# netapp-rickhuang-ai/spark-rapids-ml-nai

Measured on AMD Instinct MI355X. Metric: fit-time speedup vs Spark-ML CPU (geomean over reference headline workloads, 1Mx3000 fp32), higher is better.
Workload: dtype fp32

## Files before the change

### spark_rapids_ml_nai_amd/models/logistic.py

```python
from __future__ import annotations

import os

from typing import Any, Dict, List, Optional, Tuple

import numpy as np
import torch

from .. import ops
from ..parallel.context import WorkerContext
from .qn import QNProblem, minimize


def _problem(n: int, m_total: int, stats: Dict[str, Any], reg: float, l1_ratio: float, fit_intercept: bool,
             standardization: bool, max_iter: int, tol: float, K: int) -> Tuple[QNProblem, np.ndarray, np.ndarray]:
    sigma = stats["sigma"]
    inv_sigma = np.where(sigma > 0, 1.0 / np.where(sigma > 0, sigma, 1.0), 0.0)
    q1 = sigma if standardization else np.ones(n)
    q2 = sigma * sigma if standardization else np.ones(n)
    pen_l2 = reg * (1.0 - l1_ratio) * np.where(sigma > 0, q2 / np.where(sigma > 0, sigma * sigma, 1.0), 0.0)
    pen_l1 = reg * l1_ratio * np.where(sigma > 0, q1 / np.where(sigma > 0, sigma, 1.0), 0.0)
    nb = K if fit_intercept else 0
    theta0 = np.zeros(K * n + nb)
    if fit_intercept:
        counts = stats["class_counts"]
        if K == 1:
            p1 = counts[1] / max(counts.sum(), 1.0) if len(counts) > 1 else 0.5
            p1 = min(max(p1, 1e-12), 1 - 1e-12)
            theta0[K * n] = np.log(p1 / (1 - p1))
        else:
            lc = np.log(np.maximum(counts[:K], 1.0))
            theta0[K * n:] = lc - lc.mean()
    P = QNProblem(n=n, K=K, fit_intercept=fit_intercept, m_total=float(m_total),
                  l2=np.concatenate([np.tile(pen_l2, K), np.zeros(nb)]),
                  l1=np.concatenate([np.tile(pen_l1 if l1_ratio > 0 and reg > 0 else np.zeros(n), K), np.zeros(nb)]),
                  inv_sigma=inv_sigma, max_iter=max(0, int(max_iter)), tol=float(tol), M=10)
    return P, theta0, inv_sigma


def _result(res: Dict[str, Any], base: Dict[str, Any], ctx: WorkerContext, n: int, K: int, fit_intercept: bool,
            inv_sigma: np.ndarray, path: str) -> Dict[str, Any]:
    theta = res["theta"]
    if ctx.world_size > 1:
        th = torch.from_numpy(theta).to(ctx.device)
        ctx.comm.broadcast(th, 0)
        theta = th.cpu().numpy()
    W = theta[: K * n].reshape(K, n) * inv_sigma
    b = theta[K * n:] if fit_intercept else np.zeros(K)
    if fit_intercept and K > 1:
        b = b - b.mean()
    out = dict(base)
    out.update(coef_=W.tolist(), intercept_=[float(v) for v in b], num_iters=int(res["iter"]),
               objective=float(res["f"]))
    out["_solver"] = {"n_evals": int(res["n_evals"]), "status": res["status"], "path": path}
    if res.get("n_margin_only"):
        out["_solver"]["n_margin_only"] = int(res["n_margin_only"])
    return out


def _one_class(classes: list, base: Dict[str, Any], n: int) -> Dict[str, Any]:
    cv = classes[0]
    if cv not in (0.0, 1.0):
        raise RuntimeError("class value must be either 1. or 0. when dataset has one label")
    out = dict(base)
    out.update(coef_=[[0.0] * n], intercept_=[float("inf") if cv == 1.0 else float("-inf")], num_iters=0,
               objective=0.0)
    return out


def logistic_fit(X: Any, y: torch.Tensor, m_total: int, ctx: WorkerContext, reg: float, l1_ratio: float,
                 fit_intercept: bool, standardization: bool, max_iter: int, tol: float,
                 n_classes: Optional[int] = None, sparse: bool = False,
                 stats: Optional[Dict[str, Any]] = None) -> Dict[str, Any]:
    n = X.shape[1]
    if stats is None:
        stats = logistic_stats(X, y, m_total, ctx, sparse)
    classes = stats["classes"]
    C = n_classes if n_classes is not None else stats["num_classes"]
    K = 1 if C <= 2 else C
    dtype = "float32" if (X.dtype if not sparse else X.data.dtype) == torch.float32 else "float64"
    base = {"classes_": [float(c) for c in classes], "n_cols": int(n), "dtype": dtype}
    if len(classes) == 1 and fit_intercept:
        return _one_class(classes, base, n)
    P, theta0, inv_sigma = _problem(n, m_total, stats, reg, l1_ratio, fit_intercept, standardization, max_iter, tol, K)
    y32 = y if y.dtype == torch.float32 else y.to(torch.float32)
    y32 = y32.contiguous()

    ws = ops.logreg_workspace(X) if not sparse and K == 1 else None

    def evaluate(w: torch.Tensor, b: torch.Tensor, flag: Optional[torch.Tensor], out: torch.Tensor,
                 zc: Optional[tuple] = None) -> None:
        ops.logistic_loss_grad(X, y32, w, b, K, out, flag, ws=ws, zcache=zc)

    allreduce = ctx.comm.allreduce if ctx.distributed else None
    path = ops.logistic_path(X, K)
    fold = evaluate_partials = None
    if ws is not None and allreduce is None and path == "fused_binary_f32":
        parts, wst = ops.logreg_fold_layout(X)
        fold = (ws, parts, wst)
        _scratch = ops.zeros(K * n + 2, dtype=torch.float64, device=X.device)

        def evaluate_partials(w: torch.Tensor, b: torch.Tensor, flag: Optional[torch.Tensor],
                              zc: Optional[tuple] = None) -> None:
            ops.logistic_loss_grad(X, y32, w, b, K, _scratch, flag, ws=ws, leave_partials=True, zcache=zc)
    graph_safe = (path in ("fused_binary_f32", "fused_multinomial_f32", "csr_binary", "two_pass_multinomial_f32",
                           "two_pass_binary_f32") or path.startswith("lds_binary")) and _eval_bytes(X) <= GRAPH_MAX_BYTES
    zok = ((path == "fused_binary_f32" and (X.shape[0] == 0 or ops.logreg_zcache_ok(X)))
           or (path == "two_pass_multinomial_f32" and ops.XW_MFMA_MIN_K <= K <= 16))
    if allreduce is not None:
        flag_t = torch.tensor([1.0 if zok else 0.0], dtype=torch.float64, device=X.device)
        ctx.comm.allreduce(flag_t, op="min")
        zok = bool(flag_t.item() > 0)
    zbuf = ops.zeros(2 * X.shape[0] * K, dtype=torch.float64, device=X.device) if zok else None
    res = minimize(P, theta0, evaluate, allreduce, y.device, batch=8 if not path.startswith("torch") else 2,
                   graph_safe=graph_safe, fold=fold, evaluate_partials=evaluate_partials, zcache=zbuf)
    return _result(res, base, ctx, n, K, fit_intercept, inv_sigma, path)


GRAPH_MAX_BYTES = int(os.environ.get("SRML_QN_GRAPH_MAX_MB", "64")) << 20


def _eval_bytes(X: Any) -> int:
    if hasattr(X, "data") and hasattr(X, "indices") and not isinstance(X, torch.Tensor):
        return int(X.data.numel() * X.data.element_size() + X.indices.numel() * X.indices.element_size())
    return int(X.numel() * X.element_size())


MAX_BATCH = 12


def logistic_fit_multi(X: Any, y: torch.Tensor, m_total: int, ctx: WorkerContext, settings: List[Dict[str, Any]],
                       sparse: bool = False, stats: Optional[Dict[str, Any]] = None) -> List[Dict[str, Any]]:
    n = X.shape[1]
    if stats is None:
        stats = logistic_stats(X, y, m_total, ctx, sparse)
    K = 1 if stats["num_classes"] <= 2 else stats["num_classes"]
    if sparse or K != 1 or len(settings) < 2 or not ops.mbin_supported(X, min(len(settings), MAX_BATCH)):
        return [logistic_fit(X, y, m_total, ctx, s["reg"], s["l1_ratio"], s["fit_intercept"], s["standardization"],
                             s["max_iter"], s["tol"], sparse=sparse, stats=stats) for s in settings]
    from .qn import minimize_batch

    classes = stats["classes"]
    base = {"classes_": [float(c) for c in classes], "n_cols": int(n), "dtype": "float32"}
    y32 = (y if y.dtype == torch.float32 else y.to(torch.float32)).contiguous()
    allreduce = ctx.comm.allreduce if ctx.distributed else None
    out: List[Optional[Dict[str, Any]]] = [None] * len(settings)
    todo = []
    for i, s in enumerate(settings):
        if len(classes) == 1 and s["fit_intercept"]:
            out[i] = _one_class(classes, base, n)
        else:
            todo.append(i)
    for g0 in range(0, len(todo), MAX_BATCH):
        grp = todo[g0: g0 + MAX_BATCH]
        probs = [_problem(n, m_total, stats, settings[i]["reg"], settings[i]["l1_ratio"], settings[i]["fit_intercept"],
                          settings[i]["standardization"], settings[i]["max_iter"], settings[i]["tol"], 1) for i in grp]

        def evaluate(WB: torch.Tensor, OUT: torch.Tensor) -> None:
            ops.logistic_loss_grad_multi(X, y32, WB, OUT)

        res = minimize_batch([p[0] for p in probs], [p[1] for p in probs], evaluate, allreduce, y.device)
        for i, (P, _, inv_sigma), r in zip(grp, probs, res):
            out[i] = _result(r, base, ctx, n, 1, P.fit_intercept, inv_sigma, "batched_binary_f32")
    return [o for o in out if o is not None]


def logistic_stats(X: Any, y: torch.Tensor, m_total: int, ctx: WorkerContext, sparse: bool) -> Dict[str, Any]:
    n = X.shape[1]
    if sparse:
        s, q = ops.csr_col_moments(X)
    else:
        s, q = ops.col_moments(X)
    yl = y.long()
    if torch.any(y < 0) or torch.any(y != torch.floor(y)):
        bad = y[(y < 0) | (y != torch.floor(y))][0].item()
        if bad < 0:
            raise RuntimeError(f"Labels MUST be in [0, 2147483647), but got {bad}")
        raise RuntimeError(f"Labels MUST be Integers, but got {bad}")
    mx = torch.tensor([float(yl.max().item()) if yl.numel() else 0.0], dtype=torch.float64, device=y.device)
    ctx.comm.allreduce(mx, op="max")
    ncls = int(mx.item()) + 1
    hist = ops.label_counts(yl, ncls).double()
    buf = torch.cat([s, q, hist])
    ctx.comm.allreduce(buf)
    s, q, hist = buf[:n], buf[n: 2 * n], buf[2 * n:]
    mean = (s / m_total).cpu().numpy()
    var = np.maximum((q / m_total).cpu().numpy() - mean * mean, 0.0)
    var = var * m_total / max(m_total - 1, 1)
    counts = hist.cpu().numpy()
    classes = [float(c) for c in np.nonzero(counts > 0)[0]]
    return {"sigma": np.sqrt(var), "mean": mean, "class_counts": counts, "classes": classes,
            "num_classes": max(2, ncls)}


def logistic_scores(X: torch.Tensor, coef: torch.Tensor, intercept: torch.Tensor) -> torch.Tensor:
    return ops.xw(X, coef.T.contiguous(), intercept)
```

### spark_rapids_ml_nai_amd/models/qn.py

```python
from __future__ import annotations

import ctypes
import os
from dataclasses import dataclass
from typing import Callable, List, Optional

import numpy as np
import torch

from .. import ops

QN_GRAPH = os.environ.get("SRML_QN_GRAPH", "1") != "0"
QN_GRAPH_COMM = os.environ.get("SRML_QN_GRAPH_COMM", "1") != "0"
QN_STEP = os.environ.get("SRML_QN_STEP", "mb")
if QN_STEP not in ("mb", "single"):
    raise ValueError("SRML_QN_STEP must be 'mb' or 'single', not %r" % QN_STEP)
QN_MB = QN_STEP == "mb"
GRAPH_STATS = {"captures": 0, "replays": 0}
STATUS = {0: "running", 1: "converged (gradient)", 2: "converged (objective change)", 3: "max iterations",
          4: "line search failed"}
F_DONE, F_STATUS, F_ITER, F_NEVAL, F_LS, F_COUNT, F_HEAD, F_STARTED, F_BRACKET, F_ZMODE, F_ZSEL, F_NCHEAP, F_ZC = \
    range(13)
SC_F, SC_ALPHA, SC_DGINIT, SC_GAMMA, SC_GINF, SC_ALPHA1, SC_BETA = range(7)
QN_ZCACHE = os.environ.get("SRML_QN_ZCACHE", "1") != "0"


@dataclass
class QNProblem:
    n: int
    K: int
    fit_intercept: bool
    m_total: float
    l2: np.ndarray
    l1: np.ndarray
    inv_sigma: np.ndarray
    max_iter: int
    tol: float
    M: int = 10
    max_ls: int = 20
    past: int = 10
    c1: float = 1e-4
    c2: float = 0.9
    wolfe: bool = False
    delta: Optional[float] = None

    @property
    def Kn(self) -> int:
        return self.K * self.n

    @property
    def N(self) -> int:
        return self.Kn + (self.K if self.fit_intercept else 0)

    @property
    def use_l1(self) -> bool:
        return bool(np.any(self.l1 > 0))

    @property
    def delta_(self) -> float:
        return 0.01 * self.tol if self.delta is None else float(self.delta)

    @property
    def out_len(self) -> int:
        return self.Kn + self.K + 1


def _interp_width(f0: float, ft: float, dgtest: float) -> float:
    den = 2.0 * (ft - f0 - dgtest)
    w = -dgtest / den if den > 0 else 0.5
    if not np.isfinite(w):
        return 0.5
    return float(min(0.5, max(0.1, w)))


class HostQN:

    def __init__(self, P: QNProblem, theta0: np.ndarray) -> None:
        self.P = P
        N = P.N
        self.x = np.zeros(N)
        self.g = np.zeros(N)
        self.pg = np.zeros(N)
        self.d = np.zeros(N)
        self.xt = np.asarray(theta0, dtype=np.float64).copy()
        self.S: list = []
        self.Y: list = []
        self.f = 0.0
        self.alpha = 0.0
        self.dginit = 0.0
        self.gamma = 1.0
        self.iter = 0
        self.n_evals = 0
        self.ls = 0
        self.bracket = False
        self.started = False
        self.done = False
        self.status = 0
        self.fh = np.zeros(max(P.past, 1))
        self._isg_full = np.tile(P.inv_sigma, P.K)

    def wb(self) -> np.ndarray:
        P = self.P
        out = np.zeros(P.Kn + P.K)
        out[: P.Kn] = self.xt[: P.Kn] * self._isg_full
        if P.fit_intercept:
            out[P.Kn:] = self.xt[P.Kn:]
        return out

    @staticmethod
    def _pseudo(x: np.ndarray, g: np.ndarray, c: np.ndarray) -> np.ndarray:
        pg = g.copy()
        pos, neg, zero = x > 0, x < 0, x == 0
        pg[pos] += c[pos]
        pg[neg] -= c[neg]
        gp, gm = g + c, g - c
        z = zero & (c > 0)
        pz = np.where(gp < 0, gp, np.where(gm > 0, gm, 0.0))
        pg[z] = pz[z]
        return pg

    def _set_trial(self) -> None:
        P = self.P
        t = self.x + self.alpha * self.d
        if P.use_l1:
            orth = np.where(self.x != 0, np.sign(self.x), -np.sign(self.pg))
            mask = (P.l1 > 0) & (t * orth <= 0)
            t[mask] = 0.0
        self.xt = t

    def step(self, out: np.ndarray) -> None:
        P = self.P
        if self.done:
            return
        out = np.asarray(out, dtype=np.float64)
        Kn, N = P.Kn, P.N
        xt = self.xt
        gt = np.empty(N)
        gt[:Kn] = out[:Kn] / P.m_total * self._isg_full + P.l2[:Kn] * xt[:Kn]
        gt[Kn:] = out[Kn:N] / P.m_total
        ft = out[Kn + P.K] / P.m_total + 0.5 * float(np.sum(P.l2 * xt * xt)) + float(np.sum(P.l1 * np.abs(xt)))
        self.n_evals += 1
        if self.started:
            accept, width = True, 1.0
            if not np.isfinite(ft):
                accept, width = False, 0.5
            else:
                dgtest = float(self.pg @ (xt - self.x)) if P.use_l1 else self.alpha * self.dginit
                if ft > self.f + P.c1 * dgtest:
                    accept, width = False, _interp_width(self.f, ft, dgtest)
                elif P.wolfe and not P.use_l1 and not self.bracket and float(gt @ self.d) < P.c2 * self.dginit:
                    accept, width = False, 2.1
            if not accept:
                self.ls += 1
                if self.ls >= P.max_ls:
                    self.status, self.done = 4, True
                    return
                if width < 1.0:
                    self.bracket = True
                self.alpha *= width
                self._set_trial()
                return
        pg = self._pseudo(xt, gt, P.l1 if P.use_l1 else np.zeros(N))
        if self.started:
            s, y = xt - self.x, gt - self.g
            ys, yy = float(s @ y), float(y @ y)
            if yy > 0 and ys > 1e-10 * yy:
                self.S.append(s)
                self.Y.append(y)
                if len(self.S) > P.M:
                    self.S.pop(0)
                    self.Y.pop(0)
                self.gamma = ys / yy
            self.iter += 1
        self.x, self.g, self.f, self.pg = xt.copy(), gt, ft, pg
        self.ls, self.bracket = 0, False
        status = 0
        fmag = max(abs(ft), P.tol)
        if np.max(np.abs(pg)) <= P.tol * fmag if N else True:
            status = 1
        if P.past > 0:
            k = self.iter
            if status == 0 and self.started and k >= P.past and abs(self.fh[k % P.past] - ft) <= P.delta_ * fmag:
                status = 2
            self.fh[k % P.past] = ft
        if status == 0 and self.iter >= P.max_iter:
            status = 3
        self.started = True
        if status:
            self.status, self.done = status, True
            return
        d = -self._h_times(pg)
        if P.use_l1:
            d[(P.l1 > 0) & (d * pg >= 0)] = 0.0
        dg = float(pg @ d)
        if not dg < 0:
            d = -pg
            dg = -float(pg @ pg)
            self.S, self.Y, self.gamma = [], [], 1.0
        self.d = d
        self.dginit = dg
        self.alpha = 1.0 / max(np.sqrt(float(d @ d)), 1e-300) if not self.S else 1.0
        self._set_trial()

    def _h_times(self, v: np.ndarray) -> np.ndarray:
        if not self.S:
            return v.copy()
        S = np.stack(self.S)
        Y = np.stack(self.Y)
        g = self.gamma
        SY = S @ Y.T
        R = np.triu(SY)
        Dg = np.diag(np.diag(SY))
        p1, p2 = S @ v, Y @ v
        from scipy.linalg import solve_triangular

        t = solve_triangular(R, p1, lower=False)
        a = solve_triangular(R.T, (Dg + g * (Y @ Y.T)) @ t - g * p2, lower=True)
        return g * v + S.T @ a - g * (Y.T @ t)

    def theta(self) -> np.ndarray:
        return self.x.copy()


class _QnArgs(ctypes.Structure):
    _fields_ = [("N", ctypes.c_long), ("Kn", ctypes.c_long), ("n", ctypes.c_int), ("K", ctypes.c_int),
                ("M", ctypes.c_int), ("past", ctypes.c_int), ("max_iter", ctypes.c_int), ("max_ls", ctypes.c_int),
                ("l1", ctypes.c_int), ("wolfe", ctypes.c_int), ("tol", ctypes.c_double), ("delta", ctypes.c_double),
                ("inv_m", ctypes.c_double), ("c1", ctypes.c_double), ("c2", ctypes.c_double)] + \
               [(nm, ctypes.c_void_p) for nm in ("x", "g", "pg", "d", "xt", "gt", "S", "Y", "SY", "YY", "fh", "sc",
                                                 "l2", "l1c", "isg", "fl", "wb", "out", "probe")]


class DeviceQN:

    def __init__(self, P: QNProblem, theta0: np.ndarray, device: torch.device, wb: Optional[torch.Tensor] = None,
                 out: Optional[torch.Tensor] = None, flags: Optional[torch.Tensor] = None) -> None:
        from ..ops import native

        self.P = P
        self.device = device
        N, M = P.N, P.M
        if M > int(native.lib().srml_qn_max_history()):
            raise ValueError("L-BFGS memory %d exceeds the kernel's capacity" % M)
        f64 = dict(dtype=torch.float64, device=device)
        self.vec = ops.zeros((6 + 2 * M) * N, **f64)
        v = self.vec
        self.x, self.g, self.pg, self.d, self.xt, self.gt = (v[i * N:(i + 1) * N] for i in range(6))
        self.S = v[6 * N: (6 + M) * N]
        self.Y = v[(6 + M) * N:]
        self.small = ops.zeros(2 * M * M + max(P.past, 1) + 8, **f64)
        self.coef = torch.from_numpy(np.concatenate([P.l2, P.l1, P.inv_sigma]).astype(np.float64)).to(device)
        self.flags = flags if flags is not None else ops.zeros(16, dtype=torch.int32, device=device)
        self.wb = wb if wb is not None else ops.zeros(P.Kn + P.K, **f64)
        self.out = out if out is not None else ops.zeros(P.out_len, **f64)
        assert self.wb.numel() == P.Kn + P.K and self.out.numel() == P.out_len and self.flags.numel() == 16
        th = torch.from_numpy(np.asarray(theta0, dtype=np.float64)).to(device)
        self.xt.copy_(th)
        isg = torch.from_numpy(np.tile(P.inv_sigma, P.K)).to(device)
        self.wb[: P.Kn] = th[: P.Kn] * isg
        if P.fit_intercept:
            self.wb[P.Kn:] = th[P.Kn:]
        a = _QnArgs()
        a.N, a.Kn, a.n, a.K, a.M, a.past = N, P.Kn, P.n, P.K, M, P.past
        a.max_iter, a.max_ls, a.l1, a.wolfe = int(P.max_iter), int(P.max_ls), int(P.use_l1), int(P.wolfe)
        a.tol, a.delta, a.inv_m, a.c1, a.c2 = float(P.tol), P.delta_, 1.0 / float(P.m_total), P.c1, P.c2
        sm = self.small
        MM = M * M
        ptrs = dict(x=self.x, g=self.g, pg=self.pg, d=self.d, xt=self.xt, gt=self.gt, S=self.S, Y=self.Y,
                    SY=sm[:MM], YY=sm[MM: 2 * MM], fh=sm[2 * MM: 2 * MM + max(P.past, 1)],
                    sc=sm[2 * MM + max(P.past, 1):], l2=self.coef[:N], l1c=self.coef[N: 2 * N],
                    isg=self.coef[2 * N:], fl=self.flags, wb=self.wb, out=self.out)
        for k, t in ptrs.items():
            setattr(a, k, t.data_ptr())

        if os.environ.get("SRML_QN_PROBE") == "1":
            self.probe = ops.zeros(16, dtype=torch.int64, device=device)
            a.probe = self.probe.data_ptr()
        self._args = a
        self._keep = ptrs
        self._mb = None
        self.fold: Optional[tuple] = None
        if QN_MB and N <= 16384 and os.environ.get("SRML_QN_PROBE") != "1":
            self._mb = ops.zeros(int(native.lib().srml_qn_mb_scratch()), **f64)
        assert ctypes.sizeof(_QnArgs) == int(native.lib().srml_qn_args_size()), "QnArgs layout mismatch"

    @property
    def w_dev(self) -> torch.Tensor:
        return self.wb[: self.P.Kn]

    @property
    def b_dev(self) -> torch.Tensor:
        return self.wb[self.P.Kn:]

    def step(self) -> None:
        from ..ops import native

        if self._mb is not None and self.fold is not None:
            ws, parts, wst = self.fold
            native.call("srml_qn_step_mbf", ctypes.addressof(self._args), self._mb.data_ptr(), ws.data_ptr(),
                        int(parts), int(wst), native.stream(self.device))
        elif self._mb is not None:
            native.call("srml_qn_step_mb", ctypes.addressof(self._args), self._mb.data_ptr(), native.stream(self.device))
        else:
            native.call("srml_qn_step", ctypes.addressof(self._args), native.stream(self.device))

    def theta(self) -> np.ndarray:
        return self.x.cpu().numpy().copy()

    def zcache_supported(self) -> bool:
        return not self.P.use_l1 and not self.P.wolfe

    def enable_zcache(self, zbuf: torch.Tensor) -> tuple:
        self.flags[F_ZC] = 1
        return (self.flags, zbuf, self._keep["sc"])

    def info(self) -> dict:
        fl = self.flags.cpu().numpy()
        sc = self._keep["sc"].cpu().numpy()
        return {"iter": int(fl[F_ITER]), "n_evals": int(fl[F_NEVAL]), "status": STATUS.get(int(fl[F_STATUS]), "?"),
                "f": float(sc[SC_F]), "done": bool(fl[F_DONE]), "n_margin_only": int(fl[F_NCHEAP])}


def _graph_capturable(allreduce: Callable) -> bool:
    comm = getattr(allreduce, "__self__", None)
    if comm is None or getattr(comm, "backend", "none") != "nccl":
        return False
    from ..parallel import oneshot

    return oneshot.comm_mode() == "rccl"


def _comm_poll(allreduce: Optional[Callable]) -> Optional[Callable[[], None]]:
    return getattr(getattr(allreduce, "__self__", None), "poll", None)


def minimize(P: QNProblem, theta0: np.ndarray, evaluate: Callable[[torch.Tensor, torch.Tensor, Optional[torch.Tensor],
                                                                   torch.Tensor], None],
             allreduce: Optional[Callable[[torch.Tensor], None]], device: torch.device,
             batch: int = 8, graph_safe: bool = False, fold: Optional[tuple] = None,
             evaluate_partials: Optional[Callable] = None, zcache: Optional[torch.Tensor] = None) -> dict:
    if device.type != "cuda":
        st = HostQN(P, theta0)
        out = ops.zeros(P.out_len, dtype=torch.float64, device=device)
        cap = max(1, P.max_iter) * (P.max_ls + 1) + 2
        while not st.done and st.n_evals < cap:
            wb = torch.from_numpy(st.wb()).to(device)
            out.zero_()
            evaluate(wb[: P.Kn], wb[P.Kn:], None, out)
            if allreduce is not None:
                allreduce(out)
            st.step(out.cpu().numpy())
        return {"theta": st.theta(), "f": st.f, "iter": st.iter, "n_evals": st.n_evals,
                "status": STATUS[st.status if st.done else 3]}
    q = DeviceQN(P, theta0, device)
    zc = None
    if zcache is not None and QN_ZCACHE and q.zcache_supported():
        zc = q.enable_zcache(zcache)
    if fold is not None and evaluate_partials is not None and allreduce is None and q._mb is not None:
        q.fold = fold
        evaluate = lambda w, b, flag, out, **kw: evaluate_partials(w, b, flag, **kw)
    zkw = {"zc": zc} if zc is not None else {}
    poll = _comm_poll(allreduce)
    flag = q.flags[F_DONE: F_DONE + 1]
    host_flag = ops.zeros(2, dtype=torch.int32, pin_memory=True)
    events: list = []
    cap = max(1, P.max_iter) * (P.max_ls + (2 if zc is not None else 1)) + 2
    evals = 0
    stream = torch.cuda.current_stream(device)
    j = 0

    def run_batch() -> None:
        for _ in range(batch):
            evaluate(q.w_dev, q.b_dev, flag, q.out, **zkw)
            if allreduce is not None:
                allreduce(q.out)
            q.step()

    graph = None
    use_graph = graph_safe and QN_GRAPH and (allreduce is None or (QN_GRAPH_COMM and _graph_capturable(allreduce)))
    while evals < cap:
        if graph is not None:
            graph.replay()
            GRAPH_STATS["replays"] += 1
        else:
            run_batch()
            if use_graph and evals + batch < cap:
                graph = torch.cuda.CUDAGraph()
                side = torch.cuda.Stream(device)
                side.wait_stream(stream)
                try:
                    with torch.cuda.stream(side):
                        graph.capture_begin()
                        try:
                            run_batch()
                        finally:
                            graph.capture_end()
                    GRAPH_STATS["captures"] += 1
                except RuntimeError:
                    if allreduce is None:
                        raise
                    graph, use_graph = None, False
                    GRAPH_STATS["comm_capture_failed"] = GRAPH_STATS.get("comm_capture_failed", 0) + 1
                stream.wait_stream(side)
        evals += batch
        slot = host_flag[j % 2: j % 2 + 1]
        slot.copy_(flag, non_blocking=True)
        ev = torch.cuda.Event()
        ev.record(stream)
        events.append((ev, slot))
        j += 1
        if poll is not None:
            poll()
        if len(events) >= 2:
            ev0, s0 = events.pop(0)
            ev0.synchronize()
            if int(s0.item()):
                break
    torch.cuda.synchronize(device)
    res = q.info()
    res["theta"] = q.theta()
    if not res["done"]:
        res["status"] = "evaluation cap"
    return res


def minimize_batch(Ps: List[QNProblem], theta0s: List[np.ndarray],
                   evaluate: Callable[[torch.Tensor, torch.Tensor], None],
                   allreduce: Optional[Callable[[torch.Tensor], None]], device: torch.device,
                   batch: int = 8) -> List[dict]:
    from ..ops import native

    B = len(Ps)
    n = Ps[0].n
    assert all(P.K == 1 and P.n == n for P in Ps), "batched QN needs binary problems of one width"
    f64 = dict(dtype=torch.float64, device=device)
    WB = ops.zeros((B, n + 1), **f64)
    OUT = ops.zeros((B, n + 2), **f64)
    FL = ops.zeros((B, 16), dtype=torch.int32, device=device)
    qs = [DeviceQN(P, th, device, wb=WB[j], out=OUT[j], flags=FL[j]) for j, (P, th) in enumerate(zip(Ps, theta0s))]
    raw = b"".join(bytes(q._args) for q in qs)
    args_dev = torch.frombuffer(bytearray(raw), dtype=torch.uint8).to(device)
    st = native.stream(device)
    host = ops.zeros(2, dtype=torch.int32, pin_memory=True)
    cap = max(max(1, P.max_iter) * (P.max_ls + 1) + 2 for P in Ps)
    evals, j = 0, 0
    events: list = []
    stream = torch.cuda.current_stream(device)
    poll = _comm_poll(allreduce)
    while evals < cap:
        for _ in range(batch):
            evaluate(WB, OUT)
            if allreduce is not None:
                allreduce(OUT)
            native.call("srml_qn_step_batch", args_dev.data_ptr(), B, st)
        evals += batch
        slot = host[j % 2: j % 2 + 1]
        slot.copy_(FL[:, F_DONE].min().view(1), non_blocking=True)
        ev = torch.cuda.Event()
        ev.record(stream)
        events.append((ev, slot))
        j += 1
        if poll is not None:
            poll()
        if len(events) >= 2:
            ev0, s0 = events.pop(0)
            ev0.synchronize()
            if int(s0.item()):
                break
    torch.cuda.synchronize(device)
    out = []
    for q in qs:
        r = q.info()
        r["theta"] = q.theta()
        if not r["done"]:
            r["status"] = "evaluation cap"
        out.append(r)
    return out
```

### spark_rapids_ml_nai_amd/ops/__init__.py

```python
from __future__ import annotations

import math
import os
from typing import Any, Callable, Dict, Iterator, Optional, Tuple

import numpy as np
import torch

from . import native
from ..utils.determinism import deterministic

__all__ = ["col_moments", "gram", "xw", "dgemm", "sign_flip", "is_native", "xtv", "row_sqnorm",
           "logreg_binary_loss_grad", "nearest_centroid", "cluster_sums", "csr_logreg_binary_loss_grad",
           "csr_spmm", "csr_spmtm", "csr_col_moments", "logistic_loss_grad", "svc_path", "svc_loss_grad"]


def is_native(t: torch.Tensor) -> bool:
    return t.is_cuda


def _c(t: torch.Tensor) -> torch.Tensor:
    return t if t.is_contiguous() else t.contiguous()


# ... 138 lines not shown
        a = A.double().T if ta else A.double()
        b = B.double().T if tb else B.double()
        res = alpha * (a @ b)
        if beta != 0.0:
            res = res + beta * out
        out.copy_(res)
        return out
    A = _c(A.double())
    B = _c(B.double())
    if out.stride(1) != 1:
        raise ValueError("dgemm: out must have unit column stride")
    st = native.stream(A.device)
    tiles = ((M + 63) // 64) * ((N + 63) // 64)
    splits = _dgemm_splits(M, N, K, tiles)
    if splits > 1:
        ws = torch.empty(splits * M * N, dtype=torch.float64, device=A.device)
        native.call("srml_dgemm_splitk", int(ta), int(tb), M, N, K, float(alpha), A.data_ptr(), A.stride(0),
                    B.data_ptr(), B.stride(0), float(beta), out.data_ptr(), out.stride(0), splits, ws.data_ptr(), st)
        return out
    native.call("srml_dgemm", int(ta), int(tb), M, N, K, float(alpha), A.data_ptr(), A.stride(0), B.data_ptr(),
                B.stride(0), float(beta), out.data_ptr(), out.stride(0), st)
    return out


def _dgemm_splits(M: int, N: int, K: int, tiles: int) -> int:
    if tiles >= 512 or K < 128:
        return 1
    want = (1024 + tiles - 1) // tiles
    by_k = K // 64
    by_mem = max(1, (256 << 20) // max(1, 8 * M * N))
    return max(1, min(want, by_k, by_mem))


def sign_flip(U: torch.Tensor) -> torch.Tensor:
    rows, cols = U.shape
    if not U.is_cuda or U.dtype != torch.float64 or not U.is_contiguous():
        idx = U.abs().argmax(0)
        s = torch.sign(U[idx, torch.arange(cols, device=U.device)])
        s[s == 0] = 1
        U.mul_(s)
        return U
    native.call("srml_sign_flip_f64", U.data_ptr(), rows, cols, U.stride(0), native.stream(U.device))
    return U


def xtv(X: torch.Tensor, V: torch.Tensor, out: Optional[torch.Tensor] = None) -> torch.Tensor:
    m, n = X.shape
    V2 = V.reshape(m, -1)
    k = V2.shape[1]
    if out is None:
        out = zeros((n, k), dtype=torch.float64, device=X.device)
    if not X.is_cuda:
        out += X.double().T @ V2.double()
        return out
    if X.dtype == torch.float64:
        dgemm(_c(X), _c(V2.to(torch.float64)), ta=True, beta=1.0, out=out)
        return out
    if X.dtype != torch.float32:
        raise TypeError("xtv supports fp32/fp64 inputs, got %s" % X.dtype)
    X = _c(X)
    if k >= XTV_MFMA_MIN_K:
        for c0 in range(0, k, 16):
            kk = min(16, k - c0)
            Vc = _c(V2[:, c0: c0 + kk].to(torch.float32))
            oc = out[:, c0: c0 + kk]
            native.call("srml_xtv_mfma_f32", X.data_ptr(), m, n, X.stride(0), Vc.data_ptr(), kk, Vc.stride(0),
                        oc.data_ptr(), oc.stride(0), oc.stride(1), None, native.stream(X.device))
        return out
    if k <= 4 and out.is_contiguous() and out.dtype == torch.float64:
        Vc = _c(V2.to(torch.float32))
        native.call("srml_xtv_f32", X.data_ptr(), m, n, X.stride(0), Vc.data_ptr(), k, Vc.stride(0), out.data_ptr(),
                    native.stream(X.device))
        return out
    for c0 in range(0, k, 4):
        kk = min(4, k - c0)
        Vc = _c(V2[:, c0: c0 + kk].to(torch.float32))
        tmp = zeros((n, kk), dtype=torch.float64, device=X.device)
        native.call("srml_xtv_f32", X.data_ptr(), m, n, X.stride(0), Vc.data_ptr(), kk, Vc.stride(0), tmp.data_ptr(),
                    native.stream(X.device))
        out[:, c0: c0 + kk] += tmp
    return out


def row_sqnorm(X: torch.Tensor, mu: Optional[torch.Tensor] = None) -> torch.Tensor:
    m, n = X.shape
    if mu is not None:
        muf = _c(mu.float().view(-1))
        if not X.is_cuda or X.dtype != torch.float32:
            return ((X.float() - muf) ** 2).sum(1)
        X = _c(X)
        out = torch.empty(m, dtype=torch.float32, device=X.device)
        native.call("srml_row_sqnorm_centered_f32", X.data_ptr(), m, n, X.stride(0), muf.data_ptr(), out.data_ptr(),
                    native.stream(X.device))
        return out
    if X.is_cuda and X.dtype == torch.float64:
        X = _c(X)
        out = torch.empty(m, dtype=torch.float64, device=X.device)
        native.call("srml_row_sqnorm_f64", X.data_ptr(), m, n, X.stride(0), out.data_ptr(), native.stream(X.device))
        return out
    if not X.is_cuda or X.dtype != torch.float32:
        return (X.float() * X.float()).sum(1)
    X = _c(X)
    out = torch.empty(m, dtype=torch.float32, device=X.device)
    native.call("srml_row_sqnorm_f32", X.data_ptr(), m, n, X.stride(0), out.data_ptr(), native.stream(X.device))
    return out


def _softplus(z: torch.Tensor) -> torch.Tensor:
    return torch.clamp(z, min=0) + torch.log1p(torch.exp(-z.abs()))


def logreg_binary_loss_grad(X: torch.Tensor, y: torch.Tensor, w: torch.Tensor, b: float,
                            out: Optional[torch.Tensor] = None) -> torch.Tensor:
    m, n = X.shape
    if not X.is_cuda or X.dtype != torch.float32 or n > 4096:
        Xd = X.double()
        z = Xd @ w.double().to(X.device) + b
        yd = y.double()
        p = torch.sigmoid(z)
        r = p - yd
        loss = _softplus(z).sum() - (yd * z).sum()
        return torch.cat([Xd.T @ r, r.sum().view(1), loss.view(1)])
    X = _c(X)
    out = zeros(n + 2, dtype=torch.float64, device=X.device) if out is None else zero_(out)
    wf = _c(w.to(device=X.device, dtype=torch.float64))
    yf = _c(y.to(torch.float32))
    ws = logreg_workspace(X)
    native.call("srml_logreg_binary_f32", X.data_ptr(), m, n, X.stride(0), yf.data_ptr(), wf.data_ptr(), float(b),
                None, None, out.data_ptr(), ws.data_ptr() if ws is not None else None, 0, None, None, None,
                native.stream(X.device))
    return out


def logreg_fold_layout(X: Any) -> Tuple[int, int]:
    m, n = X.shape
    return int(native.lib().srml_logreg_fold_parts(m)), ((n + 3) & ~3) + 4


def logreg_workspace(X: Any) -> Optional[torch.Tensor]:
    if _is_csr(X) or not X.is_cuda or X.dtype != torch.float32:
        return None
    m, n = X.shape
    ptr, ld = (X.data_ptr(), X.stride(0)) if X.is_contiguous() else (0, n)
    nf = int(native.lib().srml_logreg_fold_ws(m, n, ld, ptr))
    return torch.empty(nf, dtype=torch.float32, device=X.device) if nf > 0 else None


def logreg_zcache_ok(X: Any) -> bool:
    if _is_csr(X) or not X.is_cuda or X.dtype != torch.float32 or deterministic():
        return False
    m, n = X.shape
    ptr, ld = (X.data_ptr(), X.stride(0)) if X.is_contiguous() else (0, n)
    return bool(int(native.lib().srml_logreg_zcache_ok(m, n, ld, ptr)))


def nearest_centroid(X: torch.Tensor, C: torch.Tensor, xnorm: Optional[torch.Tensor] = None,
                     cnorm: Optional[torch.Tensor] = None) -> Tuple[torch.Tensor, torch.Tensor]:
    m, n = X.shape
    k = C.shape[0]
    if X.is_cuda and X.dtype == torch.float64:
        X = _c(X)
        Cd = _c(C.to(device=X.device, dtype=torch.float64))
        cn = (Cd * Cd).sum(1) if cnorm is None or cnorm.dtype != torch.float64 else _c(cnorm)
        xn = xnorm if xnorm is not None and xnorm.dtype == torch.float64 else row_sqnorm(X)
        labels = torch.empty(m, dtype=torch.int32, device=X.device)
        dist = torch.empty(m, dtype=torch.float32, device=X.device)
        native.call("srml_nearest_centroid_f64", X.data_ptr(), m, n, X.stride(0), Cd.data_ptr(), k, Cd.stride(0),
                    cn.data_ptr(), _c(xn).data_ptr(), labels.data_ptr(), dist.data_ptr(), None,
                    native.stream(X.device))
        return labels, dist
    if cnorm is None:
        cnorm = (C.float() * C.float()).sum(1)
    if not X.is_cuda or X.dtype != torch.float32:
        labels = torch.empty(m, dtype=torch.int32, device=X.device)
        dist = torch.empty(m, dtype=torch.float32, device=X.device)
        bs = max(1, (1 << 24) // max(k, 1))
        for s in range(0, m, bs):
            xb = X[s: s + bs].float()
            d = cnorm.view(1, -1) - 2.0 * (xb @ C.float().T)
            v, i = d.min(1)
            xn = (xb * xb).sum(1) if xnorm is None else xnorm[s: s + bs]
            labels[s: s + bs] = i.int()
            dist[s: s + bs] = (v + xn).clamp_min(0)
        return labels, dist
    X = _c(X)
    C = _c(C.to(torch.float32))
    cn = _c(cnorm.to(torch.float32))
    if lloyd_small_ok(X, k, search_only=True):
        return kmeans_lloyd_small(X, C, cn, with_sums=False)[:2]
    best = torch.full((m,), -1, dtype=torch.int64, device=X.device)
    st = native.stream(X.device)
    native.call("srml_nearest_centroid_f32", X.data_ptr(), m, n, X.stride(0), C.data_ptr(), k, C.stride(0),
                cn.data_ptr(), best.data_ptr(), st)
    if xnorm is None:
        xnorm = row_sqnorm(X)
    labels = torch.empty(m, dtype=torch.int32, device=X.device)
    dist = torch.empty(m, dtype=torch.float32, device=X.device)
    native.call("srml_nn_finalize", best.data_ptr(), m, xnorm.data_ptr(), labels.data_ptr(), dist.data_ptr(), st)
    return labels, dist


def split_bf16x3(X: torch.Tensor, row_multiple: int = 128, tiled: bool = False,
                 mu: Optional[torch.Tensor] = None) -> torch.Tensor:
    m, n = X.shape
    kp = (n + 15) // 16 * 16
    if tiled and X.is_cuda and X.dtype == torch.float32:
        rows_pad = max(256, (m + 255) // 256 * 256)
        X = X if X.stride(1) == 1 else X.contiguous()
        P = torch.empty((3, rows_pad // 256, kp // 16, 256, 16), dtype=torch.bfloat16, device=X.device)
        if mu is not None:
            muf = _c(mu.float().view(-1))
            native.call("srml_split_bf16x3_tiled_centered", X.data_ptr(), m, n, X.stride(0), muf.data_ptr(), kp,
                        rows_pad, P.data_ptr(), native.stream(X.device))
        else:
            native.call("srml_split_bf16x3_tiled", X.data_ptr(), m, n, X.stride(0), kp, rows_pad, P.data_ptr(),
                        native.stream(X.device))
        return P
    if mu is not None:
        X = X.float() - mu.float().view(1, -1)
    rows_pad = max(row_multiple, (m + row_multiple - 1) // row_multiple * row_multiple)
    if not X.is_cuda or X.dtype != torch.float32:
        P = zeros((3, rows_pad, kp), dtype=torch.bfloat16, device=X.device)
        r = X.float()
        for p in range(3):
            P[p, :m, :n] = r.to(torch.bfloat16)
            r = r - P[p, :m, :n].float()
        return P
    X = X if X.stride(1) == 1 else X.contiguous()
    P = torch.empty((3, rows_pad, kp), dtype=torch.bfloat16, device=X.device)
    native.call("srml_split_bf16x3", X.data_ptr(), m, n, X.stride(0), kp, rows_pad, P.data_ptr(),
                native.stream(X.device))
    return P


CERTIFY_TAU = 2.0 ** -13


def split_bf16x3_rows(X: torch.Tensor, rows: torch.Tensor, mu: Optional[torch.Tensor]) -> torch.Tensor:
    m, n = int(rows.shape[0]), X.shape[1]
    if not X.is_cuda or X.dtype != torch.float32 or X.stride(1) != 1:
        return split_bf16x3(X.index_select(0, rows.long()), tiled=True, mu=mu)
    kp = (n + 15) // 16 * 16
    rows_pad = max(256, (m + 255) // 256 * 256)
    P = torch.empty((3, rows_pad // 256, kp // 16, 256, 16), dtype=torch.bfloat16, device=X.device)
    muf = _c(mu.float().view(-1)) if mu is not None else None
    ri = _c(rows.to(torch.int32))
    native.call("srml_split_bf16x3_tiled_centered_rows", X.data_ptr(), X.stride(0), ri.data_ptr(), m, n,
                muf.data_ptr() if muf is not None else None, kp, rows_pad, P.data_ptr(), native.stream(X.device))
    return P


def certify_tau(n: int) -> float:
    return CERTIFY_TAU + 2.0 * float(n) * 2.0 ** -24


def _nearest_centroid_certified(XP: torch.Tensor, X: torch.Tensor, m: int, k: int, CP: torch.Tensor,
                                cn: torch.Tensor, xnorm: torch.Tensor, st: int, mu: Optional[torch.Tensor]
                                ) -> Tuple[torch.Tensor, torch.Tensor]:
    dev = XP.device
    nslot = int(native.lib().srml_nearest_centroid_split_top2_nslot(k))
    keys = torch.empty(m * nslot, dtype=torch.int64, device=dev)
    lob = torch.empty(m * nslot, dtype=torch.float32, device=dev)
    xrows, kp, crows = XP.shape[1] * 256, XP.shape[2] * 16, CP.shape[1] * 256
    xn = _c(xnorm.float())
    tau = certify_tau(int(X.shape[1]) if X is not None else kp)
    cg = (2.0 * tau) * cn.clamp_min(0).sqrt()
    native.call("srml_nearest_centroid_split_top2", XP.data_ptr(), m, xrows, kp, CP.data_ptr(), k, crows,
                cn.data_ptr(), cg.data_ptr(), xn.data_ptr(), keys.data_ptr(), lob.data_ptr(), st)
    labels = torch.empty(m, dtype=torch.int32, device=dev)
    dist = torch.empty(m, dtype=torch.float32, device=dev)
    flagged = torch.empty(m, dtype=torch.int32, device=dev)
    cnt = zeros(1, dtype=torch.int32, device=dev)
    native.call("srml_split_top2_select", keys.data_ptr(), lob.data_ptr(), m, nslot, xn.data_ptr(), cg.data_ptr(),
                labels.data_ptr(), dist.data_ptr(), flagged.data_ptr(), cnt.data_ptr(), st)
    del keys, lob
    nf = int(cnt.item())
    _CERTIFY_STATS["rows"] += m
    _CERTIFY_STATS["refined"] += nf
    if nf:
        rows = flagged[:nf]
        XPr = split_bf16x3_rows(X, rows, mu)
        best = torch.full((nf,), -1, dtype=torch.int64, device=dev)
        native.call("srml_nearest_centroid_split_tiled_np", XPr.data_ptr(), nf, XPr.shape[1] * 256, kp,
                    CP.data_ptr(), k, crows, cn.data_ptr(), best.data_ptr(), 6, st)
        native.call("srml_split_scatter_refined", best.data_ptr(), rows.data_ptr(), nf, xn.data_ptr(),
                    labels.data_ptr(), dist.data_ptr(), st)
    return labels, dist


_CERTIFY_STATS = {"rows": 0, "refined": 0}


F16_U = 2.0 ** -11
F16_A = 2.0 ** -14


def certify_tau16(n: int) -> float:
    return 1.01 * (2.0 * F16_U + F16_U * F16_U + 1.01 * float(n) * 2.0 ** -24)


def f16_radius_terms(n: int, scale: float, tau: float) -> Tuple[float, float, float]:
    a = F16_A / scale
    z = 2.02 * a * math.sqrt(n) * (1.0 + F16_U)
    z2 = 2.02 * float(n) * a * a
    wmax = math.sqrt(n) * 32768.0 / scale
    return (z + 2.0 ** -24 * wmax) / (2.0 * tau), z, z2
# ... 2912 lines not shown
    n = X.shape[1]
    f32 = X.dtype == torch.float32
    if deterministic() and f32:
        return det
    if f32 and n <= 4096:
        return "fused_%s_f32" % tag
    if X.dtype in (torch.float32, torch.float64) and n <= 16384:
        return "lds_%s_%s" % (tag, "f32" if f32 else "f64")
    return "two_pass_%s_%s" % (tag, "f32" if f32 else "f64")


def logistic_path(X, K: int) -> str:
    if K == 1:
        return _binary_path(X, "binary", "two_pass_deterministic_f32")
    if _is_csr(X):
        if not X.data.is_cuda:
            return "torch-cpu"
        return "csr_spmm" if K <= 16 else "csr_wide"
    if not X.is_cuda:
        return "torch-cpu"
    n = X.shape[1]
    if deterministic() and X.dtype == torch.float32 and K <= 16:
        return "two_pass_deterministic_f32"
    if X.dtype == torch.float32 and K <= 16:
        fused = os.environ.get("SRML_LOGREG_FUSED", "0") == "1" and int(native.lib().srml_mlogit_supported(n, K))
        return "fused_multinomial_f32" if fused else "two_pass_multinomial_f32"
    if X.dtype == torch.float32:
        return "two_pass_wide_f32"
    return "two_pass_multinomial_f64"


def _glm_wide(X, y32: torch.Tensor, W: torch.Tensor, b: torch.Tensor, out: torch.Tensor,
              flag: Optional[torch.Tensor]) -> None:
    csr = _is_csr(X)
    m, n = X.shape
    K = W.shape[0]
    dev = X.data.device if csr else X.device
    st = native.stream(dev)
    fp = flag.data_ptr() if flag is not None else None
    Wf = W.to(torch.float32)
    if csr:
        Z = csr_spmm(X, Wf.t())
    else:
        Z = torch.empty((m, K), dtype=torch.float32, device=dev)
        for c0 in range(0, K, 32):
            xw_t(X, _c(Wf[c0: c0 + 32]), out=Z[:, c0: c0 + 32])
    R = zeros((m, K), dtype=torch.float32, device=dev)
    Kn = K * n
    native.call("srml_logit_residual_wide_f32", Z.data_ptr(), m, K, K, _c(y32).data_ptr(), _c(b).data_ptr(), 1,
                R.data_ptr(), K, out[Kn + K:].data_ptr(), fp, st)
    del Z
    gb, _ = col_moments(R, need_sq=False)
    out[Kn: Kn + K] += gb
    if csr:
        out[: K * n] += csr_spmtm(X, R).t().reshape(-1)
        return
    for c0 in range(0, K, 16):
        kk = min(16, K - c0)
        native.call("srml_xtv_mfma_f32", X.data_ptr(), m, n, X.stride(0), R[:, c0:].data_ptr(), kk, K,
                    out[c0 * n:].data_ptr(), 1, n, fp, st)


def mbin_supported(X, M: int) -> bool:
    return (not _is_csr(X)) and X.is_cuda and X.dtype == torch.float32 and M >= 1


def _glm_two_pass(X: torch.Tensor, y32: torch.Tensor, W: torch.Tensor, b: torch.Tensor, sb: int, mode: int,
                  grad: torch.Tensor, so_c: int, so_k: int, gb: torch.Tensor, sgb: int, loss: torch.Tensor, sl: int,
                  flag: Optional[torch.Tensor], zc: Optional[tuple] = None, family: str = "logit",
                  kind: Tuple[int, ...] = ()) -> None:
    m, n = X.shape
    K = W.shape[0]
    st = native.stream(X.device)
    fp = flag.data_ptr() if flag is not None else None
    yp = _c(y32).data_ptr()
    if zc is not None:
        zfl, zb, zsc = zc
        skip = zfl[13:14]
        Wt = W.to(torch.float32).contiguous()
        Z = torch.empty((m, K), dtype=torch.float32, device=X.device)
        X = _c(X)
        native.call("srml_xw_t_f32_skip", X.data_ptr(), m, n, X.stride(0), Wt.data_ptr(), K, Wt.stride(0), None,
                    Z.data_ptr(), Z.stride(0), skip.data_ptr(), st)
        R = torch.empty((m, K), dtype=torch.float32, device=X.device)
        native.call("srml_logit_residual_zc_f32", Z.data_ptr(), m, K, Z.stride(0), yp, b.data_ptr(), sb, mode,
                    R.data_ptr(), K, gb.data_ptr(), sgb, loss.data_ptr(), sl, fp, zfl.data_ptr(), zb.data_ptr(),
                    zsc.data_ptr(), st)
        fn = "srml_xtv_mfma_f32" if K >= XTV_MFMA_MIN_K else "srml_xtv2_f32"
        native.call(fn, X.data_ptr(), m, n, X.stride(0), R.data_ptr(), K, K, grad.data_ptr(), so_c, so_k,
                    skip.data_ptr(), st)
        return
    Z = xw_t(X, W.to(torch.float32).contiguous()) if K >= XW_MFMA_MIN_K else xw(X, W.t().float().contiguous())
    R = torch.empty((m, K), dtype=torch.float32, device=X.device)
    if deterministic():
        L = native.lib()
        ws = torch.empty(max(int(L.srml_logit_residual_ws(m, K)), int(L.srml_xtv_mfma_ws(m, n, K)), 1),
                         dtype=torch.float64, device=X.device)
        native.call("srml_%s_residual_det_f32" % family, Z.data_ptr(), m, K, Z.stride(0), yp, b.data_ptr(), sb, mode,
                    R.data_ptr(), K, gb.data_ptr(), sgb, loss.data_ptr(), sl, fp, ws.data_ptr(), *kind, st)
        native.call("srml_xtv_mfma_det_f32", X.data_ptr(), m, n, X.stride(0), R.data_ptr(), K, K, grad.data_ptr(),
                    so_c, so_k, fp, ws.data_ptr(), st)
        return
    native.call("srml_%s_residual_f32" % family, Z.data_ptr(), m, K, Z.stride(0), yp, b.data_ptr(), sb,
                mode, R.data_ptr(), K, gb.data_ptr(), sgb, loss.data_ptr(), sl, fp, *kind, st)
    fn = "srml_xtv_mfma_f32" if K >= XTV_MFMA_MIN_K else "srml_xtv2_f32"
    native.call(fn, X.data_ptr(), m, n, X.stride(0), R.data_ptr(), K, K, grad.data_ptr(), so_c, so_k, fp, st)


def _binary_two_pass(X: torch.Tensor, y32: torch.Tensor, w: torch.Tensor, b: torch.Tensor, out: torch.Tensor,
                     flag: Optional[torch.Tensor], family: str = "logit", kind: Tuple[int, ...] = ()) -> None:
    m, n = X.shape
    if X.dtype == torch.float32:
        _glm_two_pass(X, y32, w.view(1, n), b, 1, 1, out, 1, n, out[n:], 1, out[n + 1:], 1, flag, family=family,
                      kind=kind)
        return
    z = dgemm(X, w.view(n, 1))
    r = zeros((m, 1), dtype=torch.float64, device=X.device)
    native.call("srml_%s_residual_f64" % family, z.data_ptr(), m, 1, 1, _c(y32).data_ptr(), b.data_ptr(), 1, 1,
                r.data_ptr(), 1, out[n:].data_ptr(), 1, out[n + 1:].data_ptr(), 1,
                flag.data_ptr() if flag is not None else None, *kind, native.stream(X.device))
    dgemm(X, r, ta=True, beta=1.0, out=out[:n].view(n, 1))


def logistic_loss_grad_multi(X: torch.Tensor, y32: torch.Tensor, WB: torch.Tensor, out: torch.Tensor) -> torch.Tensor:
    m, n = X.shape
    M = WB.shape[0]
    if mbin_supported(X, M) and WB.stride(1) == 1 and out.stride(1) == 1 and M > 16:
        for j0 in range(0, M, 16):
            logistic_loss_grad_multi(X, y32, WB[j0: j0 + 16], out[j0: j0 + 16])
        return out
    if mbin_supported(X, M) and WB.stride(1) == 1 and out.stride(1) == 1:
        X = _c(X)
        if (os.environ.get("SRML_LOGREG_FUSED", "0") == "1" and not deterministic()
                and int(native.lib().srml_mlogit_supported(n, max(2, M)))):
            native.call("srml_mbin_f32", X.data_ptr(), m, n, X.stride(0), _c(y32).data_ptr(), WB.data_ptr(),
                        WB.stride(0), M, out.data_ptr(), out.stride(0), native.stream(X.device))
            return out
        ld = out.stride(0)
        _glm_two_pass(X, y32, WB[:, :n], WB[:, n:], WB.stride(0), 1, out, 1, ld, out[:, n:], ld, out[:, n + 1:], ld,
                      None)
        return out
    Xd = X.double()
    yd = y32.double()
    Z = Xd @ WB[:, :n].double().t() + WB[:, n].double().view(1, M)
    R = torch.sigmoid(Z) - yd.view(-1, 1)
    out[:, :n] += (R.t() @ Xd)
    out[:, n] += R.sum(0)
    out[:, n + 1] += (_softplus(Z) - yd.view(-1, 1) * Z).sum(0)
    return out


def logistic_loss_grad(X, y32: torch.Tensor, w: torch.Tensor, b: torch.Tensor, K: int, out: torch.Tensor,
                       flag: Optional[torch.Tensor] = None, ws: Optional[torch.Tensor] = None,
                       leave_partials: bool = False, zcache: Optional[tuple] = None) -> torch.Tensor:
    path = logistic_path(X, K)
    if _is_csr(X):
        m, n = X.shape
        dev = X.data.device
    else:
        X = _c(X)
        m, n = X.shape
        dev = X.device
    if path.startswith("torch"):
        if _is_csr(X):
            Xs = _csr_torch(X)
            Xs = Xs.to(torch.float64) if Xs.dtype != torch.float64 else Xs
            W = w.double().view(K, n)
            Z = (Xs @ W.t()) + b.double().view(1, K)
        else:
            Xd = X.double()
            W = w.double().view(K, n)
            Z = Xd @ W.t() + b.double().view(1, K)
        yd = y32.double()
        if K == 1:
            z = Z.view(-1)
            r = (torch.sigmoid(z) - yd).view(-1, 1)
            loss = (_softplus(z) - yd * z).sum()
        else:
            lse = torch.logsumexp(Z, 1)
            Y = torch.nn.functional.one_hot(yd.long(), K).double()
            r = torch.exp(Z - lse.view(-1, 1)) - Y
            loss = (lse - (Z * Y).sum(1)).sum()
        if _is_csr(X):
            G = (Xs.t() @ r).t()
        else:
            G = r.t() @ Xd
        out[: K * n] += G.reshape(-1)
        out[K * n: K * n + K] += r.sum(0)
        out[K * n + K] += loss
        return out
    st = native.stream(dev)
    fp = flag.data_ptr() if flag is not None else None
    assert w.dtype == torch.float64 and b.dtype == torch.float64 and out.dtype == torch.float64
    assert w.numel() == K * n and b.numel() == K and out.numel() == K * n + K + 1
    if path == "csr_binary":
        _csr_check(X)
        native.call("srml_csr_logreg_binary_" + _sfx(X), X.indptr.data_ptr(), X.indices.data_ptr(), X.data.data_ptr(),
                    m, n, X.data.numel(), y32.data_ptr(), w.data_ptr(), 0.0, b.data_ptr(), fp, out.data_ptr(), st)
    elif path == "csr_spmm":
        Z = csr_spmm(X, w.view(K, n).t())
        R = zeros((m, K), dtype=torch.float32, device=dev)
        native.call("srml_logit_residual_f32", Z.data_ptr(), m, K, K, _c(y32).data_ptr(), b.data_ptr(), 1, 0,
                    R.data_ptr(), K, out[K * n:].data_ptr(), 1, out[K * n + K:].data_ptr(), 0, fp, st)
        out[: K * n] += csr_spmtm(X, R).t().reshape(-1)
    elif path in ("csr_wide", "two_pass_wide_f32"):
        _glm_wide(X, y32, w.view(K, n), b, out, flag)
    elif path in ("two_pass_binary_f32", "two_pass_binary_f64") or (path == "two_pass_deterministic_f32" and K == 1):
        _binary_two_pass(X, y32, w, b, out, flag)
    elif path == "two_pass_multinomial_f64":
        Z = dgemm(X, w.view(K, n), tb=True)
        R = zeros((m, K), dtype=torch.float64, device=dev)
        if K <= 16:
            native.call("srml_logit_residual_f64", Z.data_ptr(), m, K, K, _c(y32).data_ptr(), b.data_ptr(), 1, 0,
                        R.data_ptr(), K, out[K * n:].data_ptr(), 1, out[K * n + K:].data_ptr(), 0, fp, st)
        else:
            native.call("srml_logit_residual_wide_f64", Z.data_ptr(), m, K, K, _c(y32).data_ptr(), b.data_ptr(), 1,
                        R.data_ptr(), K, out[K * n + K:].data_ptr(), fp, st)
            del Z
            out[K * n: K * n + K] += col_moments(R, need_sq=False)[0]
        dgemm(R, X, ta=True, beta=1.0, out=out[: K * n].view(K, n))
    elif path == "fused_binary_f32":
        zc = [t.data_ptr() for t in zcache] if zcache is not None else [None, None, None]
        native.call("srml_logreg_binary_f32", X.data_ptr(), m, n, X.stride(0), y32.data_ptr(), w.data_ptr(), 0.0,
                    b.data_ptr(), fp, out.data_ptr(), ws.data_ptr() if ws is not None else None,
                    int(bool(leave_partials and ws is not None)), *zc, st)
    elif path.startswith("lds_binary"):
        native.call("srml_logreg_binary_lds_" + path[-3:], X.data_ptr(), m, n, X.stride(0), y32.data_ptr(),
                    w.data_ptr(), 0.0, b.data_ptr(), fp, out.data_ptr(), st)
    elif path == "fused_multinomial_f32":
        native.call("srml_mlogit_f32", X.data_ptr(), m, n, X.stride(0), y32.data_ptr(), w.data_ptr(), b.data_ptr(),
                    fp, K, out.data_ptr(), st)
    elif path in ("two_pass_multinomial_f32", "two_pass_deterministic_f32"):
        _glm_two_pass(X, y32, w.view(K, n), b, 1, 0, out, 1, n, out[K * n:], 1, out[K * n + K:], 0, flag,
                      zc=zcache if path == "two_pass_multinomial_f32" else None)
    else:
        raise AssertionError(path)
    return out


SVC_LOSSES = {"hinge": 0, "squared_hinge": 1}


def svc_path(X) -> str:
    return _binary_path(X, "svc", "two_pass_deterministic_svc_f32")


def exact_sum(T: torch.Tensor, bound: Any, dim: int = 0) -> torch.Tensor:
    bound = torch.as_tensor(bound, dtype=torch.float64, device=T.device).clamp_min(2.0 ** -900)
    grid = torch.ldexp(torch.ones_like(bound), torch.frexp(bound).exponent - 52)
    return (torch.round(T / grid) * grid).sum(dim)


def _svc_exact_cpu(Xd: torch.Tensor, y32: torch.Tensor, w: torch.Tensor, b: torch.Tensor, out: torch.Tensor, kind: int,
                   xmax: torch.Tensor, m_total: float) -> torch.Tensor:
    n = Xd.shape[1]
    wd, b0 = w.double().view(-1), float(b.double().view(-1)[0])
    bz = math.fsum((xmax * wd.abs()).tolist())
    z = exact_sum(Xd * wd.view(1, n), bz, 1) + b0
    s = 2.0 * y32.double() - 1.0
    h = 1.0 - s * z
    act = (h > 0).double()
    hb = 2.0 + bz + abs(b0)
    r = -2.0 * s * h * act if kind else -s * act
    rb = 2.0 * hb if kind else 1.0
    out[:n] += exact_sum(Xd * r.view(-1, 1), m_total * rb * xmax)
    out[n] += exact_sum(r, m_total * rb)
    out[n + 1] += exact_sum(h * h * act if kind else h * act, m_total * (hb * hb if kind else hb))
    return out


def svc_loss_grad(X, y32: torch.Tensor, w: torch.Tensor, b: torch.Tensor, out: torch.Tensor,
                  flag: Optional[torch.Tensor] = None, loss: str = "hinge", ws: Optional[torch.Tensor] = None,
                  leave_partials: bool = False, exact: Optional[tuple] = None) -> torch.Tensor:
    if loss not in SVC_LOSSES:
        raise ValueError(f"loss must be 'hinge' or 'squared_hinge', got {loss!r}")
    kind = SVC_LOSSES[loss]
    path = svc_path(X)
    csr = _is_csr(X)
    if csr:
        m, n = X.shape
        dev = X.data.device
    else:
        if not (X.dim() == 2 and X.stride(1) == 1 and X.stride(0) >= X.shape[1] and ws is None
                and (path == "fused_svc_f32" or path.startswith("lds_svc"))):
            X = _c(X)
        m, n = X.shape
        dev = X.device
    if path == "torch-cpu":
        wd = w.double().view(n, 1)
        if csr:
            Xd = _csr_torch(X)
            Xd = Xd.to(torch.float64) if Xd.dtype != torch.float64 else Xd
        else:
            Xd = X.double()
        if exact is not None:
            return _svc_exact_cpu(Xd.to_dense() if csr else Xd, y32, w, b, out, kind, exact[0], float(exact[1]))
        z = (Xd @ wd).view(-1) + b.double().view(-1)[0]
        s = 2.0 * y32.double() - 1.0
        h = 1.0 - s * z
        act = (h > 0).double()
        r = -2.0 * s * h * act if kind else -s * act
        lsum = (h * h * act).sum() if kind else (h * act).sum()
        out[:n] += (Xd.t() @ r.view(-1, 1)).view(-1)
        out[n] += r.sum()
        out[n + 1] += lsum
        return out
    st = native.stream(dev)
    fp = flag.data_ptr() if flag is not None else None
    assert w.dtype == torch.float64 and b.dtype == torch.float64 and out.dtype == torch.float64
    assert w.numel() == n and b.numel() == 1 and out.numel() == n + 2 and y32.dtype == torch.float32
    if path == "csr_svc":
        _csr_check(X)
        native.call("srml_csr_svc_loss_grad_" + _sfx(X), X.indptr.data_ptr(), X.indices.data_ptr(), X.data.data_ptr(),
                    m, n, X.data.numel(), y32.data_ptr(), w.data_ptr(), 0.0, b.data_ptr(), fp, out.data_ptr(), kind, st)
    elif path == "fused_svc_f32":
        native.call("srml_svc_loss_grad_f32", X.data_ptr(), m, n, X.stride(0), y32.data_ptr(), w.data_ptr(), 0.0,
                    b.data_ptr(), fp, out.data_ptr(), ws.data_ptr() if ws is not None else None,
                    int(bool(leave_partials and ws is not None)), kind, st)
    elif path.startswith("lds_svc"):
        native.call("srml_svc_loss_grad_lds_" + path[-3:], X.data_ptr(), m, n, X.stride(0), y32.data_ptr(),
                    w.data_ptr(), 0.0, b.data_ptr(), fp, out.data_ptr(), kind, st)
    elif path in ("two_pass_svc_f32", "two_pass_svc_f64", "two_pass_deterministic_svc_f32"):
        _binary_two_pass(X, y32, w, b, out, flag, family="svc", kind=(kind,))
    else:
        raise AssertionError(path)
    return out


def h2d_async(dst: torch.Tensor, src: torch.Tensor) -> None:
    if not dst.is_cuda:
        dst.copy_(src)
        return
    assert src.is_pinned() and dst.is_contiguous() and src.is_contiguous() and dst.nbytes == src.nbytes
    native.call("srml_memcpy_h2d_async", dst.data_ptr(), src.data_ptr(), dst.nbytes, native.stream(dst.device))


def d2h_sync(dst: torch.Tensor, src: torch.Tensor) -> None:
    if not src.is_cuda:
        dst.copy_(src)
        return
    assert dst.is_pinned() and dst.is_contiguous() and src.is_contiguous() and dst.nbytes == src.nbytes
    native.call("srml_memcpy_d2h_sync", dst.data_ptr(), src.data_ptr(), src.nbytes, native.stream(src.device))


def zero_(t: torch.Tensor) -> torch.Tensor:
    if not t.is_cuda:
        return t.zero_()
    assert t.is_contiguous()
    if t.numel():
        native.call("srml_memset_async", t.data_ptr(), 0, t.nbytes, native.stream(t.device))
    return t


def zeros(*size: Any, **kw: Any) -> torch.Tensor:
    return zero_(torch.empty(*size, **kw))


_KIND = {torch.float64: 0, torch.float32: 1, torch.int64: 2, torch.int32: 3}


def _kind(t: torch.Tensor) -> Tuple[torch.Tensor, int]:
    t = _c(t)
    if t.dtype not in _KIND:
        t = t.double()
    return t, _KIND[t.dtype]


CONFUSION_MAX_CLASSES = 4096


def confusion_counts(y: torch.Tensor, pred: torch.Tensor, C: int) -> Optional[np.ndarray]:
    if C > CONFUSION_MAX_CLASSES:
        return None
    m = int(y.shape[0])
    if not y.is_cuda:
        yy, pp = y.double().cpu().numpy(), pred.double().cpu().numpy()
        ok = (yy >= 0) & (yy < C) & (yy == np.floor(yy)) & (pp >= 0) & (pp < C) & (pp == np.floor(pp))
        if not ok.all():
# ... 42 lines not shown
```

### spark_rapids_ml_nai_amd/ops/csrc/glm.hip

```cpp
#include "common.h"
#include <stdlib.h>

template <int K>
__global__ __launch_bounds__(256) void xtv_kernel(const float* __restrict__ X, long m, int n, long ld,
                                                  const float* __restrict__ V, long ldv, double* __restrict__ out,
                                                  long rows_per_block) {
  const int c0 = (blockIdx.x * 256 + threadIdx.x) * 4;
  const long r0 = (long)blockIdx.y * rows_per_block;
  const long r1 = min(m, r0 + rows_per_block);
  if (c0 >= n) return;
  double acc[K][4];
  float facc[K][4];
#pragma unroll
  for (int k = 0; k < K; ++k)
#pragma unroll
    for (int j = 0; j < 4; ++j) { acc[k][j] = 0.0; facc[k][j] = 0.f; }
  const bool full = (c0 + 3 < n) && ((ld & 3) == 0);
  int cnt = 0;
  for (long r = r0; r < r1; ++r) {
    floatx4 x;
    if (full) {
      x = *reinterpret_cast<const floatx4*>(X + r * ld + c0);
    } else {
#pragma unroll
      for (int j = 0; j < 4; ++j) x[j] = (c0 + j < n) ? X[r * ld + c0 + j] : 0.f;
    }
#pragma unroll
    for (int k = 0; k < K; ++k) {
      const float v = V[r * ldv + k];
#pragma unroll
      for (int j = 0; j < 4; ++j) facc[k][j] = fmaf(x[j], v, facc[k][j]);
    }
    if (++cnt == 256) {
#pragma unroll
      for (int k = 0; k < K; ++k)
#pragma unroll
        for (int j = 0; j < 4; ++j) { acc[k][j] += facc[k][j]; facc[k][j] = 0.f; }
      cnt = 0;
    }
  }
#pragma unroll
  for (int k = 0; k < K; ++k)
#pragma unroll
    for (int j = 0; j < 4; ++j) {
      acc[k][j] += facc[k][j];
      if (c0 + j < n) atomicAdd(&out[(long)(c0 + j) * K + k], acc[k][j]);
    }
}

SRML_API int srml_xtv_f32(const float* X, long m, int n, long ld, const float* V, int k, long ldv, double* out,
                          hipStream_t stream) {
  if (m <= 0 || n <= 0) return 0;
  unsigned gx = ceil_div(n, 1024);
  long gy = (2048 + gx - 1) / gx;
  long rpb = (m + gy - 1) / gy;
  if (rpb < 64) rpb = 64;
  gy = (m + rpb - 1) / rpb;
  dim3 grid(gx, (unsigned)gy);
  switch (k) {
    case 1: hipLaunchKernelGGL(xtv_kernel<1>, grid, dim3(256), 0, stream, X, m, n, ld, V, ldv, out, rpb); break;
    case 2: hipLaunchKernelGGL(xtv_kernel<2>, grid, dim3(256), 0, stream, X, m, n, ld, V, ldv, out, rpb); break;
    case 3: hipLaunchKernelGGL(xtv_kernel<3>, grid, dim3(256), 0, stream, X, m, n, ld, V, ldv, out, rpb); break;
    case 4: hipLaunchKernelGGL(xtv_kernel<4>, grid, dim3(256), 0, stream, X, m, n, ld, V, ldv, out, rpb); break;
    default: return -1;
  }
  return srml_status();
}

template <int K>
__global__ __launch_bounds__(256) void xtv2_kernel(const float* __restrict__ X, long m, int n, long ld,
                                                   const float* __restrict__ V, long ldv, double* __restrict__ out,
                                                   long so_c, long so_k, long rows_per_block, int kk,
                                                   const int* __restrict__ flag) {
  if (flag && *flag) return;
  const int c0 = (blockIdx.x * 256 + threadIdx.x) * 4;
  const long r0 = (long)blockIdx.y * rows_per_block;
  const long r1 = min(m, r0 + rows_per_block);
  if (c0 >= n) return;
  double acc[K][4];
  float facc[K][4];
#pragma unroll
  for (int k = 0; k < K; ++k)
#pragma unroll
    for (int j = 0; j < 4; ++j) { acc[k][j] = 0.0; facc[k][j] = 0.f; }
  const bool full = (c0 + 3 < n) && ((ld & 3) == 0);
  int cnt = 0;
  for (long r = r0; r < r1; ++r) {
    floatx4 x;
    if (full) {
      x = __builtin_nontemporal_load(reinterpret_cast<const floatx4*>(X + r * ld + c0));
    } else {
#pragma unroll
      for (int j = 0; j < 4; ++j) x[j] = (c0 + j < n) ? X[r * ld + c0 + j] : 0.f;
    }
#pragma unroll
    for (int k = 0; k < K; ++k) {
      const float v = k < kk ? V[r * ldv + k] : 0.f;
#pragma unroll
      for (int j = 0; j < 4; ++j) facc[k][j] = fmaf(x[j], v, facc[k][j]);
    }
    if (++cnt == 256) {
#pragma unroll
      for (int k = 0; k < K; ++k)
#pragma unroll
        for (int j = 0; j < 4; ++j) { acc[k][j] += facc[k][j]; facc[k][j] = 0.f; }
      cnt = 0;
    }
  }
#pragma unroll
  for (int k = 0; k < K; ++k)
#pragma unroll
    for (int j = 0; j < 4; ++j) {
      acc[k][j] += facc[k][j];
      if (k < kk && c0 + j < n) atomicAdd(&out[(long)(c0 + j) * so_c + (long)k * so_k], acc[k][j]);
    }
}

SRML_API int srml_xtv2_f32(const float* X, long m, int n, long ld, const float* V, int k, long ldv, double* out,
                           long so_c, long so_k, const int* flag, hipStream_t stream) {
  if (m <= 0 || n <= 0) return 0;
  unsigned gx = ceil_div(n, 1024);
  long gy = (2048 + gx - 1) / gx;
  long rpb = (m + gy - 1) / gy;
  if (rpb < 64) rpb = 64;
  gy = (m + rpb - 1) / rpb;
  dim3 grid(gx, (unsigned)gy);
#define SRML_XTV2(KK)                                                                                            \
  hipLaunchKernelGGL(xtv2_kernel<KK>, grid, dim3(256), 0, stream, X, m, n, ld, V, ldv, out, so_c, so_k, rpb, k, flag)
  if (k <= 1) SRML_XTV2(1);
  else if (k <= 2) SRML_XTV2(2);
  else if (k <= 4) SRML_XTV2(4);
  else if (k <= 8) SRML_XTV2(8);
  else if (k <= 12) SRML_XTV2(12);
  else if (k <= 16) SRML_XTV2(16);
  else return -1;
#undef SRML_XTV2
  return srml_status();
}

template <int WPB>
__global__ __launch_bounds__(64 * WPB) void xtv_mfma_kernel(const float* __restrict__ X, long m, int n, long ld,
                                                       const float* __restrict__ V, int K, long ldv,
                                                       double* __restrict__ out, long so_c, long so_k,
                                                       long rows_per_block, int vec, const int* __restrict__ flag,
                                                       double* __restrict__ ws) {
  if (flag && *flag) return;
  const int lane = threadIdx.x & 63, g = lane >> 4, li = lane & 15;
  const int c0 = (blockIdx.x * WPB + (threadIdx.x >> 6)) * 64;
  if (c0 >= n) return;
  const long r0 = (long)blockIdx.y * rows_per_block;
  const long r1 = min(m, r0 + rows_per_block);
  const int cl = c0 + 4 * li;
  const bool cfull = vec && (c0 + 63 < n);
// ... 156 lines not shown
SRML_API int srml_fold_partials_f64(const double* ws, long parts, long pstride, long width, long inner, double* out,
                                    long so_outer, long so_inner, const int* flag, hipStream_t stream) {
  if (width <= 0 || parts <= 0) return 0;
  if (inner < 1) return -2;
  hipLaunchKernelGGL(fold_partials_kernel, dim3(ceil_div(width, 256)), dim3(256), 0, stream, ws, parts, pstride, width,
                     inner, out, so_outer, so_inner, flag);
  return srml_status();
}

__global__ __launch_bounds__(256) void row_sqnorm_kernel(const float* __restrict__ X, long m, int n, long ld,
                                                         float* __restrict__ out, const float* __restrict__ mu,
                                                         unsigned* __restrict__ amax = nullptr) {
  const int lane = threadIdx.x & 63;
  const long wave = (long)blockIdx.x * 4 + (threadIdx.x >> 6);
  const long nw = (long)gridDim.x * 4;
  const bool vec = ((ld & 3) == 0) && ((n & 3) == 0);
  float mx = 0.f;
  for (long r = wave; r < m; r += nw) {
    const float* row = X + r * ld;
    float s = 0.f;
    if (vec) {
      for (int d = lane * 4; d < n; d += 256) {
        floatx4 v = *reinterpret_cast<const floatx4*>(row + d);
        if (mu) {
          const floatx4 c = *reinterpret_cast<const floatx4*>(mu + d);
          v[0] -= c[0]; v[1] -= c[1]; v[2] -= c[2]; v[3] -= c[3];
        }
        s = fmaf(v[0], v[0], fmaf(v[1], v[1], fmaf(v[2], v[2], fmaf(v[3], v[3], s))));
        if (amax) mx = fmaxf(mx, fmaxf(fmaxf(fabsf(v[0]), fabsf(v[1])), fmaxf(fabsf(v[2]), fabsf(v[3]))));
      }
    } else {
      for (int d = lane; d < n; d += 64) {
        const float v = mu ? row[d] - mu[d] : row[d];
        s = fmaf(v, v, s);
        mx = fmaxf(mx, fabsf(v));
      }
    }
    s = wave_sum(s);
    if (lane == 0) out[r] = s;
  }
  if (amax) {
    mx = wave_max(mx);
    if (lane == 0) atomicMax(amax, __float_as_uint(mx));
  }
}

SRML_API int srml_row_sqnorm_f32(const float* X, long m, int n, long ld, float* out, hipStream_t stream) {
  if (m <= 0) return 0;
  long blocks = (m + 3) / 4;
  if (blocks > 8192) blocks = 8192;
  hipLaunchKernelGGL(row_sqnorm_kernel, dim3((unsigned)blocks), dim3(256), 0, stream, X, m, n, ld, out,
                     (const float*)nullptr);
  return srml_status();
}

SRML_API int srml_row_sqnorm_centered_f32(const float* X, long m, int n, long ld, const float* mu, float* out,
                                          hipStream_t stream) {
  if (m <= 0) return 0;
  if (reinterpret_cast<uintptr_t>(mu) & 15) return -5;
  long blocks = (m + 3) / 4;
  if (blocks > 8192) blocks = 8192;
  hipLaunchKernelGGL(row_sqnorm_kernel, dim3((unsigned)blocks), dim3(256), 0, stream, X, m, n, ld, out, mu);
  return srml_status();
}

SRML_API int srml_row_sqnorm_centered_amax_f32(const float* X, long m, int n, long ld, const float* mu, float* out,
                                               unsigned* amax, hipStream_t stream) {
  if (m <= 0) return 0;
  if (reinterpret_cast<uintptr_t>(mu) & 15) return -5;
  long blocks = (m + 3) / 4;
  if (blocks > 8192) blocks = 8192;
  hipLaunchKernelGGL(row_sqnorm_kernel, dim3((unsigned)blocks), dim3(256), 0, stream, X, m, n, ld, out, mu, amax);
  return srml_status();
}

__device__ __forceinline__ float softplus_f(float z) {
  return z > 0.f ? z + log1pf(__expf(-z)) : log1pf(__expf(z));
}

template <int V, int LOSS = GLM_LOGISTIC>
__global__ __launch_bounds__(256) void logreg_binary_kernel(const float* __restrict__ X, long m, int n, long ld,
                                                            const float* __restrict__ y, const double* __restrict__ w,
                                                            double b_in, const double* __restrict__ bptr,
                                                            const int* __restrict__ flag, double* __restrict__ out,
                                                            long rows_per_block) {
  if (flag && *flag) return;
  const double b = bptr ? *bptr : b_in;
  extern __shared__ __attribute__((aligned(16))) double ldsd[];
  double* ws = ldsd;
  float* gs = reinterpret_cast<float*>(ldsd + 256 * V);
  const int NV = 256 * V;
  for (int i = threadIdx.x; i < NV; i += 256) {
    ws[i] = (i < n) ? w[i] : 0.0;
    gs[i] = 0.f;
  }
  __syncthreads();
  const int lane = threadIdx.x & 63;
  const int wid = threadIdx.x >> 6;
  const long r0 = (long)blockIdx.x * rows_per_block;
  const long r1 = min(m, r0 + rows_per_block);

  floatx4 g[V];
#pragma unroll
  for (int v = 0; v < V; ++v) g[v] = floatx4{0.f, 0.f, 0.f, 0.f};
  double gb = 0.0, loss = 0.0;
  const bool vec = ((ld & 3) == 0);
  for (long r = r0 + wid; r < r1; r += 4) {
    const float* row = X + r * ld;
    floatx4 x[V];
    double dot = 0.0;
#pragma unroll
    for (int v = 0; v < V; ++v) {
      const int c = (v * 64 + lane) * 4;
      floatx4& xv = x[v];
      if (vec && c + 3 < n) {
        xv = *reinterpret_cast<const floatx4*>(row + c);
      } else {
#pragma unroll
        for (int q = 0; q < 4; ++q) xv[q] = (c + q < n) ? row[c + q] : 0.f;
      }
      const double2 w01 = *reinterpret_cast<const double2*>(&ws[c]);
      const double2 w23 = *reinterpret_cast<const double2*>(&ws[c + 2]);
      dot = fma((double)xv[0], w01.x, fma((double)xv[1], w01.y, fma((double)xv[2], w23.x,
                fma((double)xv[3], w23.y, dot))));
    }
    dot = wave_sum(dot);
    const double z = dot + b;
    const double yr = (double)y[r];
    double res, lt;
    binary_terms<LOSS>(z, yr, res, lt);
    if (lane == 0) {
      loss += lt;
      gb += res;
    }
    const float rf = (float)res;
#pragma unroll
    for (int v = 0; v < V; ++v)
#pragma unroll
      for (int q = 0; q < 4; ++q) g[v][q] = fmaf(rf, x[v][q], g[v][q]);
  }
#pragma unroll
  for (int v = 0; v < V; ++v)
#pragma unroll
    for (int q = 0; q < 4; ++q) atomicAdd(&gs[(v * 64 + lane) * 4 + q], g[v][q]);
  __syncthreads();
  for (int i = threadIdx.x; i < n; i += 256) atomicAdd(&out[i], (double)gs[i]);
  if (lane == 0) {
    atomicAdd(&out[n], gb);
    atomicAdd(&out[n + 1], loss);
  }
}


constexpr int LR_F_ZMODE = 9, LR_F_ZSEL = 10, LR_SC_BETA = 6;

__device__ __forceinline__ void lr_margin_only(long m, int n, const float* __restrict__ y, double* __restrict__ out,
                                               float* __restrict__ ws, const double* __restrict__ zb,
                                               const double* __restrict__ zsc, int zsel, long q0, long rows) {
  __shared__ double mred[2][4];
  const int lane = threadIdx.x & 63, wid = threadIdx.x >> 6;
  const double beta = zsc[LR_SC_BETA];
  const double* z0 = zb + (long)zsel * m;
  const double* z1 = zb + (long)(1 - zsel) * m;
  const long q1 = min(m, q0 + rows);
  double gbc = 0.0, lossc = 0.0;
  for (long r = q0 + threadIdx.x; r < q1; r += blockDim.x) {
    const double a = z0[r];
    double res, lt;
    logistic_terms(a + beta * (z1[r] - a), (double)y[r], res, lt);
    gbc += res;
    lossc += lt;
  }
  gbc = wave_sum(gbc);
  lossc = wave_sum(lossc);
  if (lane == 0) {
    mred[0][wid] = gbc;
    mred[1][wid] = lossc;
  }
  __syncthreads();
  gbc = (mred[0][0] + mred[0][1]) + (mred[0][2] + mred[0][3]);
  lossc = (mred[1][0] + mred[1][1]) + (mred[1][2] + mred[1][3]);
  if (ws == nullptr) {
    if (threadIdx.x == 0) {
      if (gbc != 0.0) atomicAdd(&out[n], gbc);
      if (lossc != 0.0) atomicAdd(&out[n + 1], lossc);
    }
    return;
  }
  const long wsc = (long)((n + 3) & ~3) + 4;
  float* mine = ws + (long)blockIdx.x * wsc;
  for (int c = 4 * threadIdx.x; c < n; c += 4 * blockDim.x)
    *reinterpret_cast<floatx4*>(mine + c) = floatx4{0.f, 0.f, 0.f, 0.f};
  if (threadIdx.x == 0) {
    double* md = reinterpret_cast<double*>(mine + wsc - 4);
    md[0] = gbc;
    md[1] = lossc;
  }
}

constexpr int LR_PF_R = 1;
constexpr int LR_PF_D = 3;
constexpr bool LR_PF_NT = true;

template <int V, int LOSS = GLM_LOGISTIC>
__global__ __launch_bounds__(256, 2) void logreg_binary_pf_kernel(const float* __restrict__ X, long m, int n, long ld,
                                                                  const float* __restrict__ y,
                                                                  const double* __restrict__ w, double b_in,
                                                                  const double* __restrict__ bptr,
                                                                  const int* __restrict__ flag,
                                                                  double* __restrict__ out, long rows_per_block,
                                                                  float* __restrict__ ws, const int* __restrict__ zfl,
                                                                  double* __restrict__ zb,
                                                                  const double* __restrict__ zsc) {
  constexpr int R = LR_PF_R, D = LR_PF_D;
  if (flag && *flag) return;
  const double b = bptr ? *bptr : b_in;
  __shared__ double part[2][R][4];
  const int lane = threadIdx.x & 63;
  const int wid = threadIdx.x >> 6;
  const int zmode = (LOSS == GLM_LOGISTIC && zfl) ? zfl[LR_F_ZMODE] : 0;
  const int zsel = (LOSS == GLM_LOGISTIC && zfl) ? zfl[LR_F_ZSEL] : 0;
  if (zmode == 1) {
    lr_margin_only(m, n, y, out, ws, zb, zsc, zsel, (long)blockIdx.x * rows_per_block, rows_per_block);
    return;
  }
  double* zw = (LOSS == GLM_LOGISTIC && zfl) ? zb + (long)(1 - zsel) * m : nullptr;
  const int cbase = wid * 256 * V;
  double wreg[V][4];
  int coff[V];
#pragma unroll
  for (int v = 0; v < V; ++v) {
    const int c = cbase + (v * 64 + lane) * 4;
    coff[v] = (c + 3 < n) ? c : 0;
#pragma unroll
    for (int q = 0; q < 4; ++q) wreg[v][q] = (c + 3 < n) ? w[c + q] : 0.0;
  }
  floatx4 g[V];
#pragma unroll
  for (int v = 0; v < V; ++v) g[v] = floatx4{0.f, 0.f, 0.f, 0.f};
  double gb = 0.0, loss = 0.0;
  const long r0 = (long)blockIdx.x * rows_per_block;
  const long r1 = min(m, r0 + rows_per_block);
  if (r0 >= r1 && ws == nullptr) return;

  auto load = [&](long rb, floatx4 (&x)[R][V]) {
#pragma unroll
    for (int i = 0; i < R; ++i) {
      const long r = rb + i < r1 ? rb + i : r1 - 1;
      const float* row = X + r * ld;
#pragma unroll
      for (int v = 0; v < V; ++v)
        x[i][v] = LR_PF_NT ? __builtin_nontemporal_load(reinterpret_cast<const floatx4*>(row + coff[v]))
                           : *reinterpret_cast<const floatx4*>(row + coff[v]);
    }
  };
  int buf = 0;
  auto process = [&](long rb, const floatx4 (&x)[R][V]) {
#pragma unroll
    for (int i = 0; i < R; ++i) {
      double dot = 0.0;
#pragma unroll
      for (int v = 0; v < V; ++v)
        dot = fma((double)x[i][v][0], wreg[v][0], fma((double)x[i][v][1], wreg[v][1],
              fma((double)x[i][v][2], wreg[v][2], fma((double)x[i][v][3], wreg[v][3], dot))));
      dot = wave_sum(dot);
      if (lane == 0) part[buf][i][wid] = dot;
    }
    __syncthreads();
#pragma unroll
    for (int i = 0; i < R; ++i) {
      const long r = rb + i;
      if (r < r1) {
        const double z = part[buf][i][0] + part[buf][i][1] + part[buf][i][2] + part[buf][i][3] + b;
        double res, lt;
        binary_terms<LOSS>(z, (double)y[r], res, lt);
        if (wid == 0 && lane == 0) {
          loss += lt;
          gb += res;
          if (zw) zw[r] = z;
        }
        const float rf = (float)res;
#pragma unroll
        for (int v = 0; v < V; ++v)
#pragma unroll
          for (int q = 0; q < 4; ++q) g[v][q] = fmaf(rf, x[i][v][q], g[v][q]);
      }
    }
    buf ^= 1;
  };
  floatx4 x[D + 1][R][V];
#pragma unroll
  for (int d = 0; d < D; ++d)
    if (r0 + d * R < r1) load(r0 + d * R, x[d]);
  for (long rb = r0; rb < r1; rb += (D + 1) * R) {
#pragma unroll
    for (int ph = 0; ph <= D; ++ph) {
      const long cur = rb + ph * R;
      if (cur < r1) {
        const long nxt = cur + D * R;
        if (nxt < r1) load(nxt, x[(ph + D) % (D + 1)]);
        process(cur, x[ph]);
      }
    }
  }
  if (ws == nullptr) {
#pragma unroll
    for (int v = 0; v < V; ++v)
#pragma unroll
      for (int q = 0; q < 4; ++q) {
        const int c = cbase + (v * 64 + lane) * 4 + q;
        if (cbase + (v * 64 + lane) * 4 + 3 < n) atomicAdd(&out[c], (double)g[v][q]);
      }
    if (wid == 0 && lane == 0) {
      atomicAdd(&out[n], gb);
      atomicAdd(&out[n + 1], loss);
    }
    return;
  }
  const long wst = (long)((n + 3) & ~3) + 4;
  float* mine = ws + (long)blockIdx.x * wst;
#pragma unroll
  for (int v = 0; v < V; ++v) {
    const int c = cbase + (v * 64 + lane) * 4;
    if (c + 3 < n) *reinterpret_cast<floatx4*>(mine + c) = g[v];
  }
  if (wid == 0 && lane == 0) {
    double* md = reinterpret_cast<double*>(mine + wst - 4);
    md[0] = gb;
    md[1] = loss;
  }
}

template <int G, int D, int LOSS = GLM_LOGISTIC, int WPE = 1>
__global__ __launch_bounds__(256, WPE) void logreg_binary_narrow_kernel(const float* __restrict__ X, long m, int n, long ld,
                                                                   const float* __restrict__ y,
                                                                   const double* __restrict__ w, double b_in,
                                                                   const double* __restrict__ bptr,
                                                                   const int* __restrict__ flag,
                                                                   double* __restrict__ out, long rows_per_block,
                                                                   const int* __restrict__ zfl,
                                                                   double* __restrict__ zb,
                                                                   const double* __restrict__ zsc) {
  if (flag && *flag) return;
  const int zmode = (LOSS == GLM_LOGISTIC && zfl) ? zfl[LR_F_ZMODE] : 0;
  const int zsel = (LOSS == GLM_LOGISTIC && zfl) ? zfl[LR_F_ZSEL] : 0;
  if (zmode == 1) {
    lr_margin_only(m, n, y, out, nullptr, zb, zsc, zsel, (long)blockIdx.x * rows_per_block, rows_per_block);
    return;
  }
  double* zw = (LOSS == GLM_LOGISTIC && zfl) ? zb + (long)(1 - zsel) * m : nullptr;
  __shared__ float gsum[4][64 * G];
  __shared__ double red[2][4];
  const double b = bptr ? *bptr : b_in;
  const int lane = threadIdx.x & 63, wid = threadIdx.x >> 6;
  const int sub = lane & 15, grp = lane >> 4;
  double wr[G][4];
  bool cok[G];
#pragma unroll
  for (int k = 0; k < G; ++k) {
    const int c = (k * 16 + sub) * 4;
    cok[k] = c + 3 < n;
#pragma unroll
    for (int q = 0; q < 4; ++q) wr[k][q] = cok[k] ? w[c + q] : 0.0;
  }
  floatx4 g[G];
#pragma unroll
  for (int k = 0; k < G; ++k) g[k] = floatx4{0.f, 0.f, 0.f, 0.f};
  double gb = 0.0, loss = 0.0;
  const long r0 = (long)blockIdx.x * rows_per_block;
  const long r1 = min(m, r0 + rows_per_block);
  const int roff = wid * 4 + grp;
  auto load = [&](long base, floatx4 (&x)[G]) {
    long r = base + roff;
    if (r >= r1) r = r1 - 1;
    const float* row = X + r * ld;
#pragma unroll
    for (int k = 0; k < G; ++k)
      x[k] = cok[k] ? __builtin_nontemporal_load(reinterpret_cast<const floatx4*>(row + (k * 16 + sub) * 4))
                    : floatx4{0.f, 0.f, 0.f, 0.f};
  };
  auto process = [&](long base, const floatx4 (&x)[G]) {
    const long r = base + roff;
    double dot = 0.0;
#pragma unroll
    for (int k = 0; k < G; ++k)
      dot = fma((double)x[k][0], wr[k][0], fma((double)x[k][1], wr[k][1],
            fma((double)x[k][2], wr[k][2], fma((double)x[k][3], wr[k][3], dot))));
    dot += dpp_d<0xb1>(dot);
    dot += dpp_d<0x4e>(dot);
    dot += dpp_d<0x141>(dot);
    dot += dpp_d<0x140>(dot);
    if (r < r1) {
      double res, lt;
      binary_terms<LOSS>(dot + b, (double)y[r], res, lt);
      if (sub == 0) {
        loss += lt;
        gb += res;
        if (zw) zw[r] = dot + b;
      }
      const float rf = (float)res;
#pragma unroll
      for (int k = 0; k < G; ++k)
#pragma unroll
        for (int q = 0; q < 4; ++q) g[k][q] = fmaf(rf, x[k][q], g[k][q]);
    }
  };
  floatx4 xs[D + 1][G];
#pragma unroll
  for (int d = 0; d < D; ++d)
    if (r0 + d * 16 < r1) load(r0 + d * 16, xs[d]);
  for (long rb = r0; rb < r1; rb += (D + 1) * 16) {
#pragma unroll
    for (int ph = 0; ph <= D; ++ph) {
      const long cur = rb + ph * 16;
      if (cur < r1) {
        const long nxt = cur + D * 16;
        if (nxt < r1) load(nxt, xs[(ph + D) % (D + 1)]);
        process(cur, xs[ph]);
      }
    }
  }
#pragma unroll
  for (int k = 0; k < G; ++k)
#pragma unroll
    for (int q = 0; q < 4; ++q) {
      float v = g[k][q];
      v += __shfl_xor(v, 16, 64);
      v += __shfl_xor(v, 32, 64);
      if (grp == 0) gsum[wid][(k * 16 + sub) * 4 + q] = v;
    }
  loss = wave_sum(loss);
  gb = wave_sum(gb);
  if (lane == 0) {
    red[0][wid] = gb;
    red[1][wid] = loss;
  }
  __syncthreads();
  for (int c = threadIdx.x; c < n; c += 256) {
    const float v = (gsum[0][c] + gsum[1][c]) + (gsum[2][c] + gsum[3][c]);
    if (v != 0.f) atomicAdd(&out[c], (double)v);
  }
  if (threadIdx.x == 0) {
    atomicAdd(&out[n], (red[0][0] + red[0][1]) + (red[0][2] + red[0][3]));
    atomicAdd(&out[n + 1], (red[1][0] + red[1][1]) + (red[1][2] + red[1][3]));
  }
}

__global__ __launch_bounds__(256) void fold_rows_kernel(const float* __restrict__ ws, int parts, long wst, int n,
                                                        double* __restrict__ out, const int* __restrict__ flag) {
  if (flag && *flag) return;
  __shared__ double red[16][65];
  const int t = threadIdx.x;
  const int q = t & 15, rg = t >> 4;
  const int ncb = (n + 63) / 64;
  if ((int)blockIdx.x < ncb) {
    const int c = (int)blockIdx.x * 64 + 4 * q;
    double a0 = 0.0, a1 = 0.0, a2 = 0.0, a3 = 0.0;
    if (c < n) {
      int p = rg;
      for (; p + 48 < parts; p += 64) {
        floatx4 v[4];
#pragma unroll
        for (int j = 0; j < 4; ++j)
          v[j] = __builtin_nontemporal_load(reinterpret_cast<const floatx4*>(ws + (long)(p + 16 * j) * wst + c));
#pragma unroll
        for (int j = 0; j < 4; ++j) { a0 += v[j][0]; a1 += v[j][1]; a2 += v[j][2]; a3 += v[j][3]; }
      }
      for (; p < parts; p += 16) {
        const floatx4 v = __builtin_nontemporal_load(reinterpret_cast<const floatx4*>(ws + (long)p * wst + c));
        a0 += v[0]; a1 += v[1]; a2 += v[2]; a3 += v[3];
      }
    }
    red[rg][4 * q] = a0;
    red[rg][4 * q + 1] = a1;
    red[rg][4 * q + 2] = a2;
    red[rg][4 * q + 3] = a3;
    __syncthreads();
    if (t < 64) {
      const int cc = (int)blockIdx.x * 64 + t;
      double sum = 0.0;
#pragma unroll
      for (int g = 0; g < 16; ++g) sum += red[g][t];
      if (cc < n) out[cc] += sum;
    }
    return;
  }
  double gb = 0.0, loss = 0.0;
  for (int p = t; p < parts; p += 256) {
    const double* pd = reinterpret_cast<const double*>(ws + (long)p * wst + wst - 4);
    gb += pd[0];
    loss += pd[1];
  }
  gb = wave_sum(gb);
  loss = wave_sum(loss);
  if ((t & 63) == 0) {
    red[0][t >> 6] = gb;
    red[1][t >> 6] = loss;
  }
  __syncthreads();
  if (t == 0) {
    out[n] += (red[0][0] + red[0][1]) + (red[0][2] + red[0][3]);
    out[n + 1] += (red[1][0] + red[1][1]) + (red[1][2] + red[1][3]);
  }
}

static long logreg_grid(long m) {
  static const long blocks_env = getenv("SRML_LOGREG_BLOCKS") ? atol(getenv("SRML_LOGREG_BLOCKS")) : 0;
  long blocks = blocks_env;
  if (blocks <= 0) {
    blocks = m / 163;
    if (blocks > 2048) blocks = 2048;
    if (blocks < 512) blocks = 512;
  }
  long rpb = (m + blocks - 1) / blocks;
  if (rpb < 16) rpb = 16;
  return (m + rpb - 1) / rpb;
}

static bool logreg_pf_eligible(int n, long ld, const void* X) {
  return n > 1024 && n <= 4096 && (n & 3) == 0 && (ld & 3) == 0 && (reinterpret_cast<uintptr_t>(X) & 15) == 0;
}

static bool logreg_narrow_eligible(int n, long ld, const void* X) {
  static const int narrow = getenv("SRML_LOGREG_NARROW") ? atoi(getenv("SRML_LOGREG_NARROW")) : 1;
  return narrow && n <= 512 && (n & 3) == 0 && (ld & 3) == 0 && (reinterpret_cast<uintptr_t>(X) & 15) == 0;
}

static bool logreg_fold_enabled() {
  static const int fold = getenv("SRML_LOGREG_FOLD") ? atoi(getenv("SRML_LOGREG_FOLD")) : 1;
  return fold != 0;
}

SRML_API long srml_logreg_fold_ws(long m, int n, long ld, const void* X) {
  if (m <= 0 || !logreg_fold_enabled() || !logreg_pf_eligible(n, ld, X)) return 0;
  return logreg_grid(m) * (((n + 3) & ~3) + 4);
}

SRML_API long srml_logreg_fold_parts(long m) { return m <= 0 ? 0 : logreg_grid(m); }

SRML_API int srml_logreg_zcache_ok(long m, int n, long ld, const void* X) {
  return m > 0 && (logreg_narrow_eligible(n, ld, X) || logreg_pf_eligible(n, ld, X)) ? 1 : 0;
}

template <int LOSS>
static int logreg_binary_launch(const float* X, long m, int n, long ld, const float* y, const double* w, double b,
                                const double* bptr, const int* flag, double* out, float* fold_ws, int leave,
                                const int* zfl, double* zb, const double* zsc, hipStream_t stream) {
  if (m <= 0) return 0;
  if (LOSS != GLM_LOGISTIC && zfl) return -2;
  if (zfl && !logreg_pf_eligible(n, ld, X) && !logreg_narrow_eligible(n, ld, X)) return -2;
  if (logreg_narrow_eligible(n, ld, X)) {
    long nb = m / 256;
    if (nb > 4096) nb = 4096;
    if (nb < 1) nb = 1;
    long rpb = (m + nb - 1) / nb;
    rpb = (rpb + 15) / 16 * 16;
    const long blocks = (m + rpb - 1) / rpb;
    const int G = (n + 63) / 64;
#define SRML_LR_NARROW(GG, DD)                                                                                       \
  hipLaunchKernelGGL((logreg_binary_narrow_kernel<GG, DD, LOSS>), dim3((unsigned)blocks), dim3(256), 0, stream, X, m, n, ld, \
                     y, w, b, bptr, flag, out, rpb, zfl, zb, zsc)
    if constexpr (LOSS != GLM_LOGISTIC) {
      if (G > 2 && G <= 4) {
        hipLaunchKernelGGL((logreg_binary_narrow_kernel<4, 1, LOSS, 4>), dim3((unsigned)blocks), dim3(256), 0, stream,
                           X, m, n, ld, y, w, b, bptr, flag, out, rpb, zfl, zb, zsc);
        return srml_status();
      }
    }
    if (G <= 1) SRML_LR_NARROW(1, 3);
    else if (G <= 2) SRML_LR_NARROW(2, 3);
    else if (G <= 4) SRML_LR_NARROW(4, 3);
    else SRML_LR_NARROW(8, 2);
#undef SRML_LR_NARROW
    return srml_status();
  }
  const long blocks = logreg_grid(m);
  long rpb = (m + blocks - 1) / blocks;
  if (rpb < 16) rpb = 16;
  dim3 grid((unsigned)blocks), blk(256);
  if (logreg_pf_eligible(n, ld, X)) {
    const int VS = (n + 1023) / 1024;
    const long wst = ((n + 3) & ~3) + 4;
    float* fws = logreg_fold_enabled() ? fold_ws : nullptr;
#define SRML_LR_PF(VV)                                                                                       \
  hipLaunchKernelGGL((logreg_binary_pf_kernel<VV, LOSS>), grid, blk, 0, stream, X, m, n, ld, y, w, b, bptr, flag, out, \
                     rpb, fws, zfl, zb, zsc)
    if (VS == 2) SRML_LR_PF(2);
    else if (VS == 3) SRML_LR_PF(3);
    else SRML_LR_PF(4);
#undef SRML_LR_PF
    if (fws && !leave)
      hipLaunchKernelGGL(fold_rows_kernel, dim3(ceil_div(n, 64) + 1), dim3(256), 0, stream, fws, (int)blocks, wst, n,
                         out, flag);
    return srml_status();
  }
  const int V = (n + 255) / 256;
  const size_t vpad = V <= 1 ? 1 : V <= 2 ? 2 : V <= 4 ? 4 : V <= 8 ? 8 : V <= 12 ? 12 : 16;
  const size_t lds = 256 * vpad * (sizeof(double) + sizeof(float));
#define SRML_LR_LAUNCH(VV)                                                                                        \
  hipLaunchKernelGGL((logreg_binary_kernel<VV, LOSS>), grid, blk, lds, stream, X, m, n, ld, y, w, b, bptr, flag, out, rpb)
  if (V <= 1) SRML_LR_LAUNCH(1);
  else if (V <= 2) SRML_LR_LAUNCH(2);
  else if (V <= 4) SRML_LR_LAUNCH(4);
  else if (V <= 8) SRML_LR_LAUNCH(8);
  else if (V <= 12) SRML_LR_LAUNCH(12);
  else if (V <= 16) SRML_LR_LAUNCH(16);
  else return -2;
#undef SRML_LR_LAUNCH
  return srml_status();
}

SRML_API int srml_logreg_binary_f32(const float* X, long m, int n, long ld, const float* y, const double* w, double b,
                                    const double* bptr, const int* flag, double* out, float* fold_ws, int leave,
                                    const int* zfl, double* zb, const double* zsc, hipStream_t stream) {
  return logreg_binary_launch<GLM_LOGISTIC>(X, m, n, ld, y, w, b, bptr, flag, out, fold_ws, leave, zfl, zb, zsc, stream);
}

SRML_API int srml_svc_loss_grad_f32(const float* X, long m, int n, long ld, const float* y, const double* w, double b,
                                    const double* bptr, const int* flag, double* out, float* fold_ws, int leave,
                                    int loss, hipStream_t stream) {
  if (loss == 0)
    return logreg_binary_launch<GLM_HINGE>(X, m, n, ld, y, w, b, bptr, flag, out, fold_ws, leave, nullptr, nullptr,
                                           nullptr, stream);
  if (loss == 1)
    return logreg_binary_launch<GLM_SQ_HINGE>(X, m, n, ld, y, w, b, bptr, flag, out, fold_ws, leave, nullptr, nullptr,
                                              nullptr, stream);
  return -2;
}
```

### spark_rapids_ml_nai_amd/ops/csrc/qn.hip

```cpp
#include "common.h"

namespace {

constexpr int QN_T = 512;
constexpr int QN_NW = QN_T / 64;
constexpr int QN_MMAX = 12;
constexpr int QN_NV = 6 + 5 * QN_MMAX;

enum { F_DONE = 0, F_STATUS, F_ITER, F_NEVAL, F_LS, F_COUNT, F_HEAD, F_STARTED, F_BRACKET, F_ZMODE, F_ZSEL,
       F_NCHEAP, F_ZC, F_SKIPX };
enum { ST_RUNNING = 0, ST_CONV_GRAD = 1, ST_CONV_F = 2, ST_MAXITER = 3, ST_LS_FAIL = 4 };
enum { SC_F = 0, SC_ALPHA, SC_DGINIT, SC_GAMMA, SC_GINF, SC_ALPHA1, SC_BETA };

}

struct QnArgs {
  long N;
  long Kn;
  int n, K, M, past, max_iter, max_ls, l1, wolfe;
  double tol, delta, inv_m, c1, c2;
  double *x, *g, *pg, *d, *xt, *gt;
  double *S, *Y;
  double *SY, *YY;
  double *fh;
  double *sc;
  const double *l2, *l1c;
  const double *isg;
  int *fl;
  double *wb;
  double *out;
  long long *probe;
};


template <int NW, int NV>
__device__ __forceinline__ void qn_block_sum(const double (&v)[NV], double* red, double* tot) {
  const int lane = threadIdx.x & 63, wid = threadIdx.x >> 6;
#pragma unroll
  for (int i = 0; i < NV; ++i) {
    const double t = wave_sum(v[i]);
    if (lane == 0) red[i * NW + wid] = t;
    __builtin_amdgcn_sched_barrier(0);
  }
  __syncthreads();
  if (threadIdx.x < NV) {
    double s = 0.0;
#pragma unroll
    for (int w = 0; w < NW; ++w) s += red[threadIdx.x * NW + w];
    tot[threadIdx.x] = s;
  }
  __syncthreads();
}

__device__ __forceinline__ double pseudo_grad(double x, double g, double c) {
  if (c <= 0.0) return g;
  if (x > 0.0) return g + c;
  if (x < 0.0) return g - c;
  if (g + c < 0.0) return g + c;
  if (g - c > 0.0) return g - c;
  return 0.0;
}

__device__ __forceinline__ double qn_trial_value(double xv, double dv, double pv, double cv, double alpha) {
  double t = xv + alpha * dv;
  if (cv > 0.0) {
    const double orth = xv != 0.0 ? (xv > 0.0 ? 1.0 : -1.0) : (pv < 0.0 ? 1.0 : (pv > 0.0 ? -1.0 : 0.0));
    if (t * orth <= 0.0) t = 0.0;
  }
  return t;
}

__device__ __forceinline__ double qn_p0_terms(const QnArgs& A, double ov, double isg, double l2v, double l1v,
                                              double xv, double dv, double pv, double xo, double (&t)[4]) {
  const double gi = ov * A.inv_m * isg + l2v * xv;
  t[0] = l2v * xv * xv;
  t[1] = l1v * fabs(xv);
  t[2] = gi * dv;
  t[3] = pv * (xv - xo);
  return gi;
}

struct QnPair {
  double sx, yx, pgi;
};

__device__ __forceinline__ QnPair qn_p1_terms(bool started, double xv, double gv, double xo, double go, double cv,
                                              double (&t)[6]) {
  const double sx = started ? xv - xo : 0.0;
  const double yx = started ? gv - go : 0.0;
  const double pgi = pseudo_grad(xv, gv, cv);
  t[0] = sx * yx;
  t[1] = yx * yx;
  t[2] = sx * pgi;
  t[3] = yx * pgi;
  t[4] = pgi * pgi;
  t[5] = fabs(pgi);
  return {sx, yx, pgi};
}

__device__ __forceinline__ void qn_p1_slot_terms(double sx, double yx, double pgi, double Sj, double Yj,
                                                 double (&t)[5]) {
  t[0] = sx * Yj;
  t[1] = Sj * yx;
  t[2] = yx * Yj;
  t[3] = Sj * pgi;
  t[4] = Yj * pgi;
}

struct QnLs {
  bool accept;
  double width;
};

__device__ __forceinline__ QnLs qn_ls_decide(const QnArgs& A, double ft, double f, double alpha, double dginit,
                                             double p02, double p03, bool bracket, bool zc, int zmode) {
  bool accept = true;
  double width = 1.0;
  if (zc && zmode == 2 && isfinite(ft)) {
  } else if (!isfinite(ft)) {
    accept = false;
    width = 0.5;
  } else {
    const double dgtest = A.l1 ? p03 : alpha * dginit;
    if (ft > f + A.c1 * dgtest) {
      accept = false;
      const double den = 2.0 * (ft - f - dgtest);
      width = den > 0.0 ? -dgtest / den : 0.5;
      width = isfinite(width) ? fmin(0.5, fmax(0.1, width)) : 0.5;
    } else if (A.wolfe && !A.l1 && !bracket && p02 < A.c2 * dginit) {
      accept = false;
      width = 2.1;
    }
  }
  return {accept, width};
}

__device__ __forceinline__ void qn_commit_done(int* fl, int status) {
  fl[F_STATUS] = status;
  fl[F_DONE] = 1;
  fl[F_SKIPX] = 1;
}

__device__ __forceinline__ void qn_commit_zmode(int* fl, int zmode) {
  fl[F_ZMODE] = zmode;
  fl[F_SKIPX] = zmode == 1 ? 1 : 0;
}

__device__ __forceinline__ void qn_commit_reject(const QnArgs& A, int ls, int neval, double width, double alpha_tried,
                                                 double alpha, double ft, bool zc, int zmode, double alpha1) {
  int* fl = A.fl;
  fl[F_LS] = ls;
  fl[F_NEVAL] = neval;
  if (ls >= A.max_ls) {
    qn_commit_done(fl, ST_LS_FAIL);
    return;
  }
  if (width < 1.0) fl[F_BRACKET] = 1;
  A.sc[SC_ALPHA] = alpha;
  if (zc && isfinite(ft)) {
    const double a1 = zmode == 0 ? alpha_tried : alpha1;
    A.sc[SC_ALPHA1] = a1;
    A.sc[SC_BETA] = alpha / a1;
    qn_commit_zmode(fl, 1);
  } else if (zc) {
    qn_commit_zmode(fl, 0);
  }
}

__device__ __forceinline__ void qn_commit_margins_accept(int* fl, int neval) {
  fl[F_NEVAL] = neval;
  qn_commit_zmode(fl, 2);
}

__device__ __forceinline__ void qn_commit_margins_point(int* fl) {
  fl[F_ZSEL] ^= 1;
  qn_commit_zmode(fl, 0);
}

struct QnHist {
  double sy[QN_MMAX * QN_MMAX], yy[QN_MMAX * QN_MMAX];
  double p1[QN_MMAX], p2[QN_MMAX];
  double cf_a[QN_MMAX], cf_t[QN_MMAX];
  int sl[QN_MMAX];
};

struct QnUpd {
  int status, newp, cnt, hd, iter;
  double gamma;
};

__device__ __forceinline__ QnUpd qn_history_update(const QnArgs& A, QnHist& H, const double* tot, double ginf,
                                                   double fn, bool started, int count, int head, int pre_iter,
                                                   double pre_gamma, double fh_next) {
  const int M = A.M;
  int cnt = count, hd = head, status = ST_RUNNING;
  double gamma = started ? pre_gamma : 1.0;
  for (int j = 0; j < M; ++j) {
    H.p1[j] = tot[6 + 3 * QN_MMAX + j];
    H.p2[j] = tot[6 + 4 * QN_MMAX + j];
  }
  const double ys = tot[0], yy = tot[1];
  const bool newp = started && yy > 0.0 && ys > 1e-10 * yy;
  if (newp) {
    const int h = hd;
    for (int j = 0; j < M; ++j) {
      if (j == h) continue;
      H.sy[h * M + j] = tot[6 + j];
      H.sy[j * M + h] = tot[6 + QN_MMAX + j];
      H.yy[h * M + j] = tot[6 + 2 * QN_MMAX + j];
      H.yy[j * M + h] = tot[6 + 2 * QN_MMAX + j];
    }
    H.sy[h * M + h] = ys;
    H.yy[h * M + h] = yy;
    H.p1[h] = tot[2];
    H.p2[h] = tot[3];
    hd = (h + 1) % M;
    cnt = cnt < M ? cnt + 1 : M;
    gamma = ys / yy;
  }
  const int iter = pre_iter + (started ? 1 : 0);
  const double fmag = fmax(fabs(fn), A.tol);
  if (ginf <= A.tol * fmag) status = ST_CONV_GRAD;
  if (A.past > 0 && status == ST_RUNNING && started && iter >= A.past && fabs(fh_next - fn) <= A.delta * fmag)
    status = ST_CONV_F;
  if (status == ST_RUNNING && iter >= A.max_iter) status = ST_MAXITER;
  for (int c = 0; c < cnt; ++c) H.sl[c] = (hd - cnt + c + 2 * M) % M;
  return {status, newp ? 1 : 0, cnt, hd, iter, gamma};
}

__device__ __forceinline__ void qn_compact_solve(QnHist& H, int M, int cnt, double gamma) {
  const int c = threadIdx.x;
  const bool act = c < cnt;
  const int slc = act ? H.sl[c] : 0;
  double Rrow[QN_MMAX], Rcol[QN_MMAX], Yrow[QN_MMAX], tv[QN_MMAX];
#pragma unroll
  for (int e = 0; e < QN_MMAX; ++e) {
    const bool ok = act && e < cnt;
    const int sle = ok ? H.sl[e] : 0;
    Rrow[e] = ok ? H.sy[slc * M + sle] : 0.0;
    Rcol[e] = ok ? H.sy[sle * M + slc] : 0.0;
    Yrow[e] = ok ? H.yy[slc * M + sle] : 0.0;
    tv[e] = 0.0;
  }
  const double diag = act ? H.sy[slc * M + slc] : 1.0;
  double acc = act ? H.p1[slc] : 0.0;
  double tmine = 0.0;
#pragma unroll
  for (int e = QN_MMAX - 1; e >= 0; --e) {
    if (e < cnt) {
      const double te = __shfl(acc / diag, e, 64);
      tv[e] = te;
      if (c == e) tmine = te;
      if (c < e) acc -= Rrow[e] * te;
    }
  }
  acc = diag * tmine - gamma * (act ? H.p2[slc] : 0.0);
#pragma unroll
  for (int e = 0; e < QN_MMAX; ++e) acc += gamma * Yrow[e] * tv[e];
  double amine = 0.0;
#pragma unroll
  for (int e = 0; e < QN_MMAX; ++e) {
    if (e < cnt) {
      const double ae = __shfl(acc / diag, e, 64);
      if (c == e) amine = ae;
      if (c > e) acc -= Rcol[e] * ae;
    }
  }
  if (c < QN_MMAX) {
    H.cf_a[c] = 0.0;
    H.cf_t[c] = 0.0;
  }
  __builtin_amdgcn_wave_barrier();
  if (act) {
    H.cf_a[slc] = amine;
    H.cf_t[slc] = gamma * tmine;
  }
}


template <int NV>
__device__ __forceinline__ void qn_sum_all(double (&v)[NV], double* red) {
  qn_block_sum<QN_NW>(v, red, red + NV * QN_NW);
#pragma unroll
  for (int i = 0; i < NV; ++i) v[i] = red[NV * QN_NW + i];
}

__device__ __forceinline__ double qn_max_all(double v, double* red) {
  v = wave_max(v);
  const int lane = threadIdx.x & 63, wid = threadIdx.x >> 6;
  if (lane == 0) red[wid] = v;
  __syncthreads();
  double r = red[0];
#pragma unroll
  for (int w = 1; w < QN_NW; ++w) r = fmax(r, red[w]);
  __syncthreads();
  return r;
}

constexpr int QN_U = 4;
#define QN_BATCH(i0) for (long i0 = threadIdx.x; i0 < A.N; i0 += (long)QN_T * QN_U)
#define QN_LANE(u, i0) const long i_##u = (i0) + (long)(u) * QN_T

__device__ void qn_set_trial(const QnArgs& A, double alpha) {
  QN_BATCH(i0) {
    double xv[QN_U], dv[QN_U], pv[QN_U], cv[QN_U], sv[QN_U];
#pragma unroll
    for (int u = 0; u < QN_U; ++u) {
      const long i = i0 + (long)u * QN_T;
      const bool ok = i < A.N;
      xv[u] = ok ? A.x[i] : 0.0;
      dv[u] = ok ? A.d[i] : 0.0;
      pv[u] = (ok && A.l1) ? A.pg[i] : 0.0;
      cv[u] = (ok && A.l1) ? A.l1c[i] : 0.0;
      sv[u] = (ok && i < A.Kn) ? A.isg[i % A.n] : 1.0;
    }
#pragma unroll
    for (int u = 0; u < QN_U; ++u) {
      const long i = i0 + (long)u * QN_T;
      if (i < A.N) {
        const double t = qn_trial_value(xv[u], dv[u], pv[u], cv[u], alpha);
        A.xt[i] = t;
        A.wb[i] = t * sv[u];
      }
    }
  }
}

#define QN_PROBE(k) \
  do { if (A.probe && threadIdx.x == 0) A.probe[k] = wall_clock64(); } while (0)
// ... 163 lines not shown
        }
      }
    }
  }

  QN_PROBE(3);
  if (tid == 0) {
    const QnUpd u = qn_history_update(A, H, s_v, ginf, ft, started, count, head, pre_iter, pre_gamma, pre_fh_next);
    s_u = u;
    if (A.past > 0) A.fh[u.iter % A.past] = ft;
    fl[F_ITER] = u.iter;
    fl[F_HEAD] = u.hd;
    fl[F_COUNT] = u.cnt;
    fl[F_NEVAL] = pre_neval + 1;
    fl[F_LS] = 0;
    fl[F_BRACKET] = 0;
    fl[F_STARTED] = 1;
    A.sc[SC_F] = ft;
    A.sc[SC_GAMMA] = u.gamma;
    A.sc[SC_GINF] = ginf;
  }
  __syncthreads();
  if (tid < 64) qn_compact_solve(H, M, s_u.cnt, s_u.gamma);
  __syncthreads();
  if (s_u.newp) {
    for (int i = tid; i < M * M; i += QN_T) {
      A.SY[i] = H.sy[i];
      A.YY[i] = H.yy[i];
    }
  }
  __syncthreads();
  const int status = s_u.status;
  const bool newp = s_u.newp != 0;
  const int cnt = s_u.cnt;
  const double gamma = s_u.gamma;
  QN_PROBE(4);

  double p2v[2] = {0.0, 0.0};
  QN_BATCH(i0) {
    double xv[QN_U], gv[QN_U], sv[QN_U], yv[QN_U], pv[QN_U], cv[QN_U];
#pragma unroll
    for (int u = 0; u < QN_U; ++u) {
      const long i = i0 + (long)u * QN_T;
      const bool ok = i < N;
      xv[u] = ok ? A.xt[i] : 0.0;
      gv[u] = ok ? A.gt[i] : 0.0;
      sv[u] = ok ? A.d[i] : 0.0;
      yv[u] = ok ? A.wb[i] : 0.0;
      pv[u] = ok ? A.pg[i] : 0.0;
      cv[u] = (ok && A.l1) ? A.l1c[i] : 0.0;
    }
#pragma unroll
    for (int u = 0; u < QN_U; ++u) {
      const long i = i0 + (long)u * QN_T;
      if (i < N) {
        if (newp) {
          A.S[(long)head * N + i] = sv[u];
          A.Y[(long)head * N + i] = yv[u];
        }
        A.x[i] = xv[u];
        A.g[i] = gv[u];
      }
    }
    if (status == ST_RUNNING) {
      double hg[QN_U];
#pragma unroll
      for (int u = 0; u < QN_U; ++u) hg[u] = gamma * pv[u];
      constexpr int QN_G = 4;
      for (int c0 = 0; c0 < cnt; c0 += QN_G) {
        double Sv[QN_G][QN_U], Yv[QN_G][QN_U], ca[QN_G], ct[QN_G];
#pragma unroll
        for (int q = 0; q < QN_G; ++q) {
          const bool okq = c0 + q < cnt;
          const int j = okq ? H.sl[c0 + q] : 0;
          ca[q] = okq ? H.cf_a[j] : 0.0;
          ct[q] = okq ? H.cf_t[j] : 0.0;
#pragma unroll
          for (int u = 0; u < QN_U; ++u) {
            const long i = i0 + (long)u * QN_T;
            const bool ok = okq && i < N;
            Sv[q][u] = ok ? A.S[(long)j * N + i] : 0.0;
            Yv[q][u] = ok ? A.Y[(long)j * N + i] : 0.0;
          }
        }
#pragma unroll
        for (int q = 0; q < QN_G; ++q)
#pragma unroll
          for (int u = 0; u < QN_U; ++u) hg[u] += ca[q] * Sv[q][u] - ct[q] * Yv[q][u];
      }
#pragma unroll
      for (int u = 0; u < QN_U; ++u) {
        const long i = i0 + (long)u * QN_T;
        if (i < N) {
          double di = -hg[u];
          if (cv[u] > 0.0 && di * pv[u] >= 0.0) di = 0.0;
          A.d[i] = di;
          p2v[0] += pv[u] * di;
          p2v[1] += di * di;
        }
      }
    }
  }
  if (status != ST_RUNNING) {
    if (tid == 0) qn_commit_done(fl, status);
    return;
  }
  QN_PROBE(5);
  qn_sum_all(p2v, red);
  double dg = p2v[0], dd = p2v[1];
  int cnt2 = cnt;
  if (!(dg < 0.0)) {
    for (long i = tid; i < N; i += QN_T) A.d[i] = -A.pg[i];
    dg = -s_v[4];
    dd = s_v[4];
    cnt2 = 0;
    __syncthreads();
  }
  alpha = cnt2 == 0 ? 1.0 / fmax(sqrt(dd), 1e-300) : 1.0;
  QN_PROBE(6);
  qn_set_trial(A, alpha);
  QN_PROBE(7);
  if (tid == 0) {
    if (cnt2 == 0) {
      fl[F_COUNT] = 0;
      A.sc[SC_GAMMA] = 1.0;
    }
    A.sc[SC_ALPHA] = alpha;
    A.sc[SC_DGINIT] = dg;
  }
}

__global__ __launch_bounds__(QN_T) void qn_step_kernel(QnArgs A) { qn_step_body(A); }

__global__ __launch_bounds__(QN_T) void qn_step_batch_kernel(const QnArgs* __restrict__ args) {
  const QnArgs A = args[blockIdx.x];
  qn_step_body(A);
}

SRML_API int srml_qn_step_batch(const QnArgs* args_dev, int count, hipStream_t stream) {
  if (count <= 0) return 0;
  hipLaunchKernelGGL(qn_step_batch_kernel, dim3((unsigned)count), dim3(QN_T), 0, stream, args_dev);
  return srml_status();
}

SRML_API int srml_qn_step(const QnArgs* a, hipStream_t stream) {
  if (a->M < 1 || a->M > QN_MMAX || a->N <= 0) return (int)hipErrorInvalidValue;
  hipLaunchKernelGGL(qn_step_kernel, dim3(1), dim3(QN_T), 0, stream, *a);
  return srml_status();
}

SRML_API int srml_qn_max_history() { return QN_MMAX; }
SRML_API long srml_qn_args_size() { return (long)sizeof(QnArgs); }

namespace {

constexpr int MB_T = 256;
constexpr int MB_NW = MB_T / 64;
constexpr int MB_GMAX = 64;
constexpr int MBF_E = 32;
constexpr int MB_GAMAX = 512;
constexpr int MB_PW = 6 + 5 * QN_MMAX + 1;
enum {
  S_STARTED = 0, S_ITER, S_COUNT, S_HEAD, S_LS, S_NEVAL, S_BRACKET, S_F, S_ALPHA, S_DGINIT, S_GAMMA, S_FHN, S_LOSS,
  S_ZMODE, S_ZC, S_ALPHA1,
  S_PHASE = 16, S_STATUS, S_NEWP, S_CNT, S_HD, S_GAM, S_FT, S_GINF, S_ITERN, S_FN,
  S_CF = 32,
  S_SL = S_CF + 2 * QN_MMAX,
  S_SY = S_SL + QN_MMAX,
  S_PA = S_SY + 2 * QN_MMAX * QN_MMAX,
  S_PB = S_PA + 4 * MB_GAMAX,
  S_PC = S_PB + MB_PW * MB_GMAX,
  S_END = S_PC + 2 * MB_GMAX
};

__device__ __forceinline__ void mb_grid_sum(const double* part, int G, int width, double* tot, bool max_last) {
  __shared__ double gs[MB_T];
  const int t = threadIdx.x, S = MB_T / width;
  const int j = t % width, sl = t / width;
  const bool mx = max_last && j == width - 1;
  double a[8] = {0.0, 0.0, 0.0, 0.0, 0.0, 0.0, 0.0, 0.0};
  if (sl < S) {
    int b = sl;
    for (; b + 7 * S < G; b += 8 * S) {
      double v[8];
#pragma unroll
      for (int k = 0; k < 8; ++k) v[k] = part[(long)(b + k * S) * width + j];
#pragma unroll
      for (int k = 0; k < 8; ++k) a[k] = mx ? fmax(a[k], v[k]) : a[k] + v[k];
    }
    for (; b < G; b += S) {
      const double v = part[(long)b * width + j];
      a[0] = mx ? fmax(a[0], v) : a[0] + v;
    }
  }
  gs[t] = mx ? fmax(fmax(fmax(a[0], a[1]), fmax(a[2], a[3])), fmax(fmax(a[4], a[5]), fmax(a[6], a[7])))
             : ((a[0] + a[1]) + (a[2] + a[3])) + ((a[4] + a[5]) + (a[6] + a[7]));
  __syncthreads();
  if (t < width) {
    double x = gs[t];
    for (int q = 1; q < S; ++q) x = mx ? fmax(x, gs[q * width + t]) : x + gs[q * width + t];
    tot[t] = x;
  }
  __syncthreads();
}

}


struct MbSnap {
  int started, iter, count, head, ls, neval, bracket, zmode, zc;
  double f, alpha, dginit, gamma, alpha1;
};

__device__ __forceinline__ MbSnap mb_snap_load(const QnArgs& A) {
  const int* fl = A.fl;
  MbSnap q;
  q.started = fl[F_STARTED];
  q.iter = fl[F_ITER];
  q.count = fl[F_COUNT];
  q.head = fl[F_HEAD];
  q.ls = fl[F_LS];
  q.neval = fl[F_NEVAL];
  q.bracket = fl[F_BRACKET];
  q.f = A.sc[SC_F];
  q.alpha = A.sc[SC_ALPHA];
  q.dginit = A.sc[SC_DGINIT];
  q.gamma = A.sc[SC_GAMMA];
  q.zc = fl[F_ZC];
  q.zmode = q.zc ? fl[F_ZMODE] : 0;
  q.alpha1 = A.sc[SC_ALPHA1];
  return q;
}

__device__ __forceinline__ void mb_snap_store(const QnArgs& A, const MbSnap& q, double* scr) {
  scr[S_STARTED] = q.started ? 1.0 : 0.0;
  scr[S_ITER] = q.iter;
  scr[S_COUNT] = q.count;
  scr[S_HEAD] = q.head;
  scr[S_LS] = q.ls;
  scr[S_NEVAL] = q.neval;
  scr[S_BRACKET] = q.bracket;
  scr[S_F] = q.f;
  scr[S_ALPHA] = q.alpha;
  scr[S_DGINIT] = q.dginit;
  scr[S_GAMMA] = q.gamma;
  scr[S_FHN] = (A.past > 0 && q.started) ? A.fh[(q.iter + 1) % A.past] : 0.0;
  scr[S_ZMODE] = q.zmode;
  scr[S_ZC] = q.zc;
  scr[S_ALPHA1] = q.alpha1;
  scr[S_PHASE] = 0.0;
}

struct MbP0In {
  double xv, l2v, l1v, dv, pgv, xo, isg;
};

__device__ __forceinline__ MbP0In mb_p0_load(const QnArgs& A, long i, bool own) {
  MbP0In e{0.0, 0.0, 0.0, 0.0, 0.0, 0.0, 1.0};
  if (own) {
    e.xv = A.xt[i];
    e.l2v = A.l2[i];
    e.l1v = A.l1c[i];
    e.dv = A.d[i];
    e.pgv = A.pg[i];
    e.xo = A.x[i];
    if (i < A.Kn) e.isg = A.isg[i % A.n];
  }
  return e;
}

__device__ __forceinline__ void mb_p0(const QnArgs& A, long i, bool own, const MbP0In& e, double ov, double (&p0)[4]) {
  if (own) A.gt[i] = qn_p0_terms(A, ov, e.isg, e.l2v, e.l1v, e.xv, e.dv, e.pgv, e.xo, p0);
}

__global__ __launch_bounds__(MB_T) void qn_mb1_kernel(QnArgs A, double* __restrict__ scr) {
  __shared__ double red[4 * MB_NW], tot[4];
  const bool first = blockIdx.x == 0 && threadIdx.x == 0;
  const long i = (long)blockIdx.x * MB_T + threadIdx.x;
  const bool own = i < A.N;
  const int done = A.fl[F_DONE];
  MbSnap q{};
  double loss = 0.0;
  if (first) {
    q = mb_snap_load(A);
    loss = A.out[A.Kn + A.K];
  }
  const MbP0In e = mb_p0_load(A, i, own);
  const double ov = own ? A.out[i] : 0.0;
  if (done) {
    if (first) scr[S_PHASE] = 0.0;
    return;
  }
  if (first) {
    mb_snap_store(A, q, scr);
    scr[S_LOSS] = loss;
  }
  double p0[4] = {0.0, 0.0, 0.0, 0.0};
  mb_p0(A, i, own, e, ov, p0);
  if (own && i < A.Kn + A.K) A.out[i] = 0.0;
  qn_block_sum<MB_NW>(p0, red, tot);
  if (threadIdx.x < 4) scr[S_PA + blockIdx.x * 4 + threadIdx.x] = tot[threadIdx.x];
}

__device__ __forceinline__ void mb_trial(const QnArgs& A, long i, double xv, double dv, double pv, double cv,
                                         double isg, double alpha) {
  const double t = qn_trial_value(xv, dv, pv, A.l1 ? cv : 0.0, alpha);
  A.xt[i] = t;
  A.wb[i] = t * isg;
}

__global__ __launch_bounds__(MB_T) void qn_mb2_kernel(QnArgs A, double* __restrict__ scr, int ga) {
  __shared__ double red[MB_PW * MB_NW], p0[4];
  int* fl = A.fl;
  const int M = A.M;
  const long N = A.N;
  const long i = (long)blockIdx.x * MB_T + threadIdx.x;
  const bool own = i < N;
  const bool first = blockIdx.x == 0 && threadIdx.x == 0;
  const int done = fl[F_DONE];
  const bool started = scr[S_STARTED] != 0.0;
  const double f = scr[S_F], dginit = scr[S_DGINIT], alpha0 = scr[S_ALPHA], loss = scr[S_LOSS];
  const bool bracket = scr[S_BRACKET] != 0.0;
  const int pre_ls = (int)scr[S_LS], pre_neval = (int)scr[S_NEVAL];
  const bool zc = scr[S_ZC] != 0.0;
  const int zmode = (int)scr[S_ZMODE];
  const double alpha1 = scr[S_ALPHA1];
  double xt = 0.0, gt = 0.0, xo = 0.0, go = 0.0, cv = 0.0, dv = 0.0, pv = 0.0, isg = 1.0;
  double Sv[QN_MMAX], Yv[QN_MMAX];
  if (own) {
    xt = A.xt[i];
    gt = A.gt[i];
    xo = A.x[i];
    go = A.g[i];
    cv = A.l1c[i];
    dv = A.d[i];
    pv = A.pg[i];
    if (i < A.Kn) isg = A.isg[i % A.n];
  }
#pragma unroll
  for (int j = 0; j < QN_MMAX; ++j) {
    Sv[j] = (own && j < M) ? A.S[(long)j * N + i] : 0.0;
    Yv[j] = (own && j < M) ? A.Y[(long)j * N + i] : 0.0;
  }
  if (done) return;
  mb_grid_sum(scr + S_PA, ga, 4, p0, false);
  double alpha = alpha0;
  const double ft = loss * A.inv_m + 0.5 * p0[0] + p0[1];
  if (first)
    for (long j = N; j < A.Kn + A.K + 1; ++j) A.out[j] = 0.0;
  if (first && zc && zmode == 1) fl[F_NCHEAP] += 1;
  if (started) {
    const QnLs d = qn_ls_decide(A, ft, f, alpha, dginit, p0[2], p0[3], bracket, zc, zmode);
    if (!d.accept) {
      const int ls = pre_ls + 1;
      alpha *= d.width;
      if (ls < A.max_ls && own) mb_trial(A, i, xo, dv, pv, cv, isg, alpha);
      if (first) qn_commit_reject(A, ls, pre_neval + 1, d.width, alpha0, alpha, ft, zc, zmode, alpha1);
      return;
    }
    if (zc && zmode == 1) {
      if (first) qn_commit_margins_accept(fl, pre_neval + 1);
      return;
    }
  }
  if (first) {
    scr[S_PHASE] = 1.0;
    scr[S_FT] = ft;
    if (zc) qn_commit_margins_point(fl);
  }
  double v[MB_PW];
#pragma unroll
  for (int j = 0; j < MB_PW; ++j) v[j] = 0.0;
  if (own) {
    double t[6];
    const QnPair e = qn_p1_terms(started, xt, gt, xo, go, A.l1 ? cv : 0.0, t);
    A.pg[i] = e.pgi;
    A.d[i] = e.sx;
    A.wb[i] = e.yx;
#pragma unroll
    for (int k = 0; k < 5; ++k) v[k] = t[k];
    v[MB_PW - 1] = t[5];
#pragma unroll
    for (int j = 0; j < QN_MMAX; ++j) {
      double h[5];
      qn_p1_slot_terms(e.sx, e.yx, e.pgi, Sv[j], Yv[j], h);
#pragma unroll
      for (int k = 0; k < 5; ++k) v[6 + k * QN_MMAX + j] = h[k];
    }
  }
  const int lane = threadIdx.x & 63, wid = threadIdx.x >> 6;
#pragma unroll
  for (int j = 0; j < MB_PW - 1; ++j) {
    const bool live = j < 6 || ((j - 6) % QN_MMAX) < M;
    const double t = live ? wave_sum(v[j]) : 0.0;
    if (lane == 0) red[j * MB_NW + wid] = t;
    __builtin_amdgcn_sched_barrier(0);
  }
  {
    const double mx = wave_max(v[MB_PW - 1]);
    if (lane == 0) red[(MB_PW - 1) * MB_NW + wid] = mx;
  }
  __syncthreads();
  if (threadIdx.x < MB_PW) {
    const int j = threadIdx.x;
    double s = 0.0;
    for (int w = 0; w < MB_NW; ++w)
      s = j == MB_PW - 1 ? fmax(s, red[j * MB_NW + w]) : s + red[j * MB_NW + w];
    scr[S_PB + (long)blockIdx.x * MB_PW + j] = s;
  }
}

__global__ __launch_bounds__(MB_T) void qn_mb3_kernel(QnArgs A, double* __restrict__ scr) {
  __shared__ double tot[MB_PW], red[2 * MB_NW], t2[2];
  __shared__ QnHist H;
  __shared__ QnUpd s_u;
  const int G = gridDim.x, M = A.M, tid = threadIdx.x;
  const long N = A.N;
  const long i = (long)blockIdx.x * MB_T + tid;
  const bool own = i < N;
  const double phase = scr[S_PHASE];
  const bool started = scr[S_STARTED] != 0.0;
  const int pre_count = (int)scr[S_COUNT], head = (int)scr[S_HEAD], pre_iter = (int)scr[S_ITER];
  const double pre_gamma = scr[S_GAMMA], fn = scr[S_FT], fhn = scr[S_FHN];
  const double sy0 = tid < M * M ? A.SY[tid] : 0.0, yy0 = tid < M * M ? A.YY[tid] : 0.0;
  double xt = 0.0, gt = 0.0, sv = 0.0, yv = 0.0, pv = 0.0, cv = 0.0;
  double Sv[QN_MMAX], Yv[QN_MMAX];
  if (own) {
    xt = A.xt[i];
    gt = A.gt[i];
    sv = A.d[i];
    yv = A.wb[i];
    pv = A.pg[i];
    cv = A.l1c[i];
  }
#pragma unroll
  for (int j = 0; j < QN_MMAX; ++j) {
    Sv[j] = (own && j < M) ? A.S[(long)j * N + i] : 0.0;
    Yv[j] = (own && j < M) ? A.Y[(long)j * N + i] : 0.0;
  }
  if (phase != 1.0) return;
  if (tid < M * M) {
    H.sy[tid] = sy0;
    H.yy[tid] = yy0;
  }
  mb_grid_sum(scr + S_PB, G, MB_PW, tot, true);
  if (tid == 0) {
    const double ginf = tot[MB_PW - 1];
    const QnUpd u = qn_history_update(A, H, tot, ginf, fn, started, pre_count, head, pre_iter, pre_gamma, fhn);
    s_u = u;
    if (blockIdx.x == 0) {
      scr[S_STATUS] = u.status;
      scr[S_NEWP] = u.newp ? 1.0 : 0.0;
      scr[S_CNT] = u.cnt;
      scr[S_HD] = u.hd;
      scr[S_GAM] = u.gamma;
      scr[S_GINF] = ginf;
      scr[S_ITERN] = u.iter;
      scr[S_FN] = fn;
    }
  }
  __syncthreads();
  if (tid < 64) qn_compact_solve(H, M, s_u.cnt, s_u.gamma);
  __syncthreads();
  const int status = s_u.status;
  const bool newp = s_u.newp != 0;
  const double gamma = s_u.gamma;
  if (blockIdx.x == 0 && newp)
    for (int k = tid; k < M * M; k += MB_T) {
      scr[S_SY + k] = H.sy[k];
      scr[S_SY + QN_MMAX * QN_MMAX + k] = H.yy[k];
    }
  double p2v[2] = {0.0, 0.0};
  if (own) {
    if (newp) {
      A.S[(long)head * N + i] = sv;
      A.Y[(long)head * N + i] = yv;
    }
    A.x[i] = xt;
    A.g[i] = gt;
    if (status == ST_RUNNING) {
      double hg = gamma * pv;
#pragma unroll
      for (int j = 0; j < QN_MMAX; ++j) {
        if (j < M) {
          const bool fresh = newp && j == head;
          hg += H.cf_a[j] * (fresh ? sv : Sv[j]) - H.cf_t[j] * (fresh ? yv : Yv[j]);
        }
      }
      double di = -hg;
      if (A.l1 && cv > 0.0 && di * pv >= 0.0) di = 0.0;
      A.d[i] = di;
      p2v[0] = pv * di;
      p2v[1] = di * di;
    }
  }
  qn_block_sum<MB_NW>(p2v, red, t2);
  if (tid < 2) scr[S_PC + blockIdx.x * 2 + tid] = t2[tid];
}

__global__ __launch_bounds__(MB_T) void qn_mb4_kernel(QnArgs A, double* __restrict__ scr) {
  __shared__ double p2[2], pbt[MB_PW];
  const int G = gridDim.x, M = A.M, tid = threadIdx.x;
  const bool first = blockIdx.x == 0 && tid == 0;
  const long i = (long)blockIdx.x * MB_T + tid;
  const bool own = i < A.N;
  int* fl = A.fl;
  const double phase = scr[S_PHASE];
  const int status = (int)scr[S_STATUS];
  const bool newp = scr[S_NEWP] != 0.0;
  const int cnt0 = (int)scr[S_CNT];
  double sy = 0.0, yy = 0.0;
  if (blockIdx.x == 0 && tid < M * M) {
    sy = scr[S_SY + tid];
    yy = scr[S_SY + QN_MMAX * QN_MMAX + tid];
  }
  double xv = 0.0, dv = 0.0, pv = 0.0, cv = 0.0, isg = 1.0;
  if (own) {
    xv = A.x[i];
    dv = A.d[i];
    pv = A.pg[i];
    cv = A.l1c[i];
    if (i < A.Kn) isg = A.isg[i % A.n];
  }
  if (phase != 1.0) return;
  if (blockIdx.x == 0) {
    if (newp && tid < M * M) {
      A.SY[tid] = sy;
      A.YY[tid] = yy;
    }
    if (tid == 0) {
      const int iter = (int)scr[S_ITERN];
      if (A.past > 0) A.fh[iter % A.past] = scr[S_FN];
      fl[F_ITER] = iter;
      fl[F_HEAD] = (int)scr[S_HD];
      fl[F_COUNT] = cnt0;
      fl[F_NEVAL] = (int)scr[S_NEVAL] + 1;
      fl[F_LS] = 0;
      fl[F_BRACKET] = 0;
      fl[F_STARTED] = 1;
      A.sc[SC_F] = scr[S_FN];
      A.sc[SC_GAMMA] = scr[S_GAM];
      A.sc[SC_GINF] = scr[S_GINF];
    }
  }
  if (status != ST_RUNNING) {
    if (first) qn_commit_done(fl, status);
    return;
  }
  mb_grid_sum(scr + S_PC, G, 2, p2, false);
  double dg = p2[0], dd = p2[1];
  int cnt2 = cnt0;
  if (!(dg < 0.0)) {
    mb_grid_sum(scr + S_PB, G, MB_PW, pbt, true);
    const double pp = pbt[4];
    dv = -pv;
    if (own) A.d[i] = dv;
    dg = -pp;
    dd = pp;
    cnt2 = 0;
  }
  const double alpha = cnt2 == 0 ? 1.0 / fmax(sqrt(dd), 1e-300) : 1.0;
  if (own) mb_trial(A, i, xv, dv, pv, cv, isg, alpha);
  if (first) {
    if (cnt2 == 0) {
      fl[F_COUNT] = 0;
      A.sc[SC_GAMMA] = 1.0;
    }
    A.sc[SC_ALPHA] = alpha;
    A.sc[SC_DGINIT] = dg;
  }
}

SRML_API long srml_qn_mb_scratch() { return (long)S_END; }

SRML_API int srml_qn_step_mb(const QnArgs* a, double* scratch, hipStream_t stream) {
  if (a->M < 1 || a->M > QN_MMAX || a->N <= 0 || !scratch) return (int)hipErrorInvalidValue;
  const long G = (a->N + MB_T - 1) / MB_T;
  if (G > MB_GMAX) return srml_qn_step(a, stream);
  const dim3 grid((unsigned)G), blk(MB_T);
  hipLaunchKernelGGL(qn_mb1_kernel, grid, blk, 0, stream, *a, scratch);
  hipLaunchKernelGGL(qn_mb2_kernel, grid, blk, 0, stream, *a, scratch, (int)G);
  hipLaunchKernelGGL(qn_mb3_kernel, grid, blk, 0, stream, *a, scratch);
  hipLaunchKernelGGL(qn_mb4_kernel, grid, blk, 0, stream, *a, scratch);
  return srml_status();
}

__device__ __forceinline__ void mbf_fold_block(const QnArgs& A, const float* __restrict__ fws, int parts, long wst,
                                              double (*fold)[33], double* red, bool own, long i, unsigned G,
                                              double& oval, double& lpart) {
  const int tid = threadIdx.x;
  const int q = tid & 7, rg = tid >> 3;
  const long c = (long)blockIdx.x * MBF_E + 4 * q;
  const bool has_bias = A.K == 1 && A.Kn < A.N && (long)blockIdx.x == A.Kn / MBF_E;
  const bool has_loss = blockIdx.x == G - 1;
  double gb = 0.0, ls = 0.0;
  if (has_bias || has_loss)
    for (int p = tid; p < parts; p += 4 * MB_T) {
      double t0[4], t1[4];
#pragma unroll
      for (int k = 0; k < 4; ++k) {
        const int pk = p + k * MB_T;
        const double* pd = reinterpret_cast<const double*>(fws + (long)(pk < parts ? pk : 0) * wst + wst - 4);
        t0[k] = pk < parts ? pd[0] : 0.0;
        t1[k] = pk < parts ? pd[1] : 0.0;
      }
#pragma unroll
      for (int k = 0; k < 4; ++k) {
        gb += t0[k];
        ls += t1[k];
      }
    }
  double a0 = 0.0, a1 = 0.0, a2 = 0.0, a3 = 0.0;
  if (c < A.Kn) {
    int p = rg;
    for (; p + 32 * 11 < parts; p += 32 * 12) {
      floatx4 v[12];
#pragma unroll
      for (int j = 0; j < 12; ++j)
        v[j] = __builtin_nontemporal_load(reinterpret_cast<const floatx4*>(fws + (long)(p + 32 * j) * wst + c));
#pragma unroll
      for (int j = 0; j < 12; ++j) { a0 += v[j][0]; a1 += v[j][1]; a2 += v[j][2]; a3 += v[j][3]; }
    }
    for (; p < parts; p += 32) {
      const floatx4 v = __builtin_nontemporal_load(reinterpret_cast<const floatx4*>(fws + (long)p * wst + c));
      a0 += v[0]; a1 += v[1]; a2 += v[2]; a3 += v[3];
    }
  }
  fold[rg][4 * q] = a0;
  fold[rg][4 * q + 1] = a1;
  fold[rg][4 * q + 2] = a2;
  fold[rg][4 * q + 3] = a3;
  const double sums[2] = {has_bias ? gb : 0.0, has_loss ? ls : 0.0};
  double tv2[2];
  {
    const int lane = tid & 63, wid = tid >> 6;
    for (int k = 0; k < 2; ++k) {
      const double t = wave_sum(sums[k]);
      if (lane == 0) red[k * MB_NW + wid] = t;
    }
  }
  __syncthreads();
  tv2[0] = (red[0] + red[1]) + (red[2] + red[3]);
  tv2[1] = (red[MB_NW] + red[MB_NW + 1]) + (red[MB_NW + 2] + red[MB_NW + 3]);
  if (own) {
    if (i < A.Kn) {
      double s = 0.0;
#pragma unroll
      for (int g2 = 0; g2 < 32; ++g2) s += fold[g2][tid];
      oval = s;
    } else {
      oval = tv2[0];
    }
  }
  lpart = tv2[1];
  __syncthreads();
}

__global__ __launch_bounds__(MB_T) void qn_mb1f_kernel(QnArgs A, double* __restrict__ scr,
                                                       const float* __restrict__ fws, int parts, long wst) {
  __shared__ double red[4 * MB_NW], tot[4], fold[32][33];
  const bool first = blockIdx.x == 0 && threadIdx.x == 0;
  const unsigned G = gridDim.x;
  const long i = (long)blockIdx.x * MBF_E + threadIdx.x;
  const bool own = threadIdx.x < MBF_E && i < A.N;
  const int done = A.fl[F_DONE];
  MbSnap q{};
  if (first) q = mb_snap_load(A);
  const MbP0In e = mb_p0_load(A, i, own);
  double oval = 0.0, lpart = 0.0;
  mbf_fold_block(A, fws, parts, wst, fold, red, own, i, G, oval, lpart);
  if (done) {
    if (first) scr[S_PHASE] = 0.0;
    return;
  }
  if (first) mb_snap_store(A, q, scr);
  if (blockIdx.x == G - 1 && threadIdx.x == 0) scr[S_LOSS] = lpart;
  double p0[4] = {0.0, 0.0, 0.0, 0.0};
  mb_p0(A, i, own, e, oval, p0);
  qn_block_sum<MB_NW>(p0, red, tot);
  if (threadIdx.x < 4) scr[S_PA + blockIdx.x * 4 + threadIdx.x] = tot[threadIdx.x];
}

SRML_API int srml_qn_step_mbf(const QnArgs* a, double* scratch, const float* fws, int parts, long wst,
                              hipStream_t stream) {
  if (a->M < 1 || a->M > QN_MMAX || a->N <= 0 || !scratch || !fws) return (int)hipErrorInvalidValue;
  if (a->K != 1 || (wst & 3) || parts <= 0) return (int)hipErrorInvalidValue;
  const long G = (a->N + MB_T - 1) / MB_T, G1 = (a->N + MBF_E - 1) / MBF_E;
  if (G > MB_GMAX || G1 > MB_GAMAX) return (int)hipErrorInvalidValue;
  const dim3 grid((unsigned)G), blk(MB_T);
  hipLaunchKernelGGL(qn_mb1f_kernel, dim3((unsigned)G1), blk, 0, stream, *a, scratch, fws, parts, wst);
  hipLaunchKernelGGL(qn_mb2_kernel, grid, blk, 0, stream, *a, scratch, (int)G1);
  hipLaunchKernelGGL(qn_mb3_kernel, grid, blk, 0, stream, *a, scratch);
  hipLaunchKernelGGL(qn_mb4_kernel, grid, blk, 0, stream, *a, scratch);
  return srml_status();
}
```

### spark_rapids_ml_nai_amd/ops/native.py

```python
from __future__ import annotations

import ctypes
import os
import threading
from typing import Any, Dict, Optional, Tuple

import torch

from . import build as _build

_P = ctypes.c_void_p
_I = ctypes.c_int
_L = ctypes.c_long
_D = ctypes.c_double
_F = ctypes.c_float

_LONG_RESULT = ("srml_rf_bootstrap_ws", "srml_logreg_fold_ws", "srml_qn_mb_scratch",
                "srml_logreg_fold_parts", "srml_qn_args_size", "srml_logit_residual_ws", "srml_xtv_mfma_ws",
                "srml_rf_partition_ws", "srml_dbscan_labels_ws", "srml_umap_categorical_ws",
                "srml_umap_epoch_sync_ws",
                "srml_label_sort_ws", "srml_radix_sort_ws", "srml_lloyd_moved_ws", "srml_sum_f32_ws", "srml_sum_sq_ws",
                "srml_cagra_lds_bytes")
SIGNATURES: Dict[str, Tuple[Any, ...]] = {
    "srml_col_moments_f32": (_P, _L, _I, _L, _P, _P, _P),
    "srml_col_moments_f64": (_P, _L, _I, _L, _P, _P, _P),
    "srml_standardize_f32": (_P, _L, _I, _L, _P, _P, _P),
    "srml_gram_f32": (_P, _L, _I, _L, _P, _P, _P),
    "srml_gram_f32_ex": (_P, _L, _I, _L, _P, _P, _P, _I, _P),
    "srml_mirror_upper_f64": (_P, _I, _P),
    "srml_xw_f32": (_P, _L, _I, _L, _P, _I, _P, _P, _L, _P),
    "srml_dgemm": (_I, _I, _I, _I, _I, _D, _P, _L, _P, _L, _D, _P, _L, _P),
    "srml_dgemm_splitk": (_I, _I, _I, _I, _I, _D, _P, _L, _P, _L, _D, _P, _L, _I, _P, _P),
    "srml_dgemm_syrk_lower": (_I, _I, _D, _P, _L, _D, _P, _L, _P),
    "srml_sign_flip_f64": (_P, _I, _I, _L, _P),
    "srml_xtv_f32": (_P, _L, _I, _L, _P, _I, _L, _P, _P),
    "srml_row_sqnorm_f32": (_P, _L, _I, _L, _P, _P),
    "srml_logreg_binary_f32": (_P, _L, _I, _L, _P, _P, _D, _P, _P, _P, _P, _I, _P, _P, _P, _P),
    "srml_logreg_fold_parts": (_L,),
    "srml_logreg_fold_ws": (_L, _I, _L, _P),
    "srml_logreg_zcache_ok": (_L, _I, _L, _P),
    "srml_logreg_binary_lds_f32": (_P, _L, _I, _L, _P, _P, _D, _P, _P, _P, _P),
    "srml_logreg_binary_lds_f64": (_P, _L, _I, _L, _P, _P, _D, _P, _P, _P, _P),
    "srml_xtv2_f32": (_P, _L, _I, _L, _P, _I, _L, _P, _L, _L, _P, _P),
    "srml_xtv_mfma_f32": (_P, _L, _I, _L, _P, _I, _L, _P, _L, _L, _P, _P),
    "srml_xtv_mfma_det_f32": (_P, _L, _I, _L, _P, _I, _L, _P, _L, _L, _P, _P, _P),
    "srml_fold_partials_f64": (_P, _L, _L, _L, _L, _P, _L, _L, _P, _P),
    "srml_xw_t_f32": (_P, _L, _I, _L, _P, _I, _L, _P, _P, _L, _P),
    "srml_xw_t_f32_skip": (_P, _L, _I, _L, _P, _I, _L, _P, _P, _L, _P, _P),
    "srml_xw_t_f32_variant": (_P, _L, _I, _L, _P, _I, _L, _P, _P, _L, _I, _P),
    "srml_logit_residual_f32": (_P, _L, _I, _L, _P, _P, _L, _I, _P, _L, _P, _L, _P, _L, _P, _P),
    "srml_logit_residual_zc_f32": (_P, _L, _I, _L, _P, _P, _L, _I, _P, _L, _P, _L, _P, _L, _P, _P, _P, _P, _P),
    "srml_logit_residual_f64": (_P, _L, _I, _L, _P, _P, _L, _I, _P, _L, _P, _L, _P, _L, _P, _P),
    "srml_logit_residual_det_f32": (_P, _L, _I, _L, _P, _P, _L, _I, _P, _L, _P, _L, _P, _L, _P, _P, _P),
    "srml_logit_residual_ws": (_L, _I),
    "srml_svc_loss_grad_f32": (_P, _L, _I, _L, _P, _P, _D, _P, _P, _P, _P, _I, _I, _P),
    "srml_svc_loss_grad_lds_f32": (_P, _L, _I, _L, _P, _P, _D, _P, _P, _P, _I, _P),
    "srml_svc_loss_grad_lds_f64": (_P, _L, _I, _L, _P, _P, _D, _P, _P, _P, _I, _P),
    "srml_csr_svc_loss_grad_f32": (_P, _P, _P, _L, _I, _L, _P, _P, _D, _P, _P, _P, _I, _P),
    "srml_csr_svc_loss_grad_f64": (_P, _P, _P, _L, _I, _L, _P, _P, _D, _P, _P, _P, _I, _P),
    "srml_svc_residual_f32": (_P, _L, _I, _L, _P, _P, _L, _I, _P, _L, _P, _L, _P, _L, _P, _I, _P),
    "srml_svc_residual_f64": (_P, _L, _I, _L, _P, _P, _L, _I, _P, _L, _P, _L, _P, _L, _P, _I, _P),
    "srml_svc_residual_det_f32": (_P, _L, _I, _L, _P, _P, _L, _I, _P, _L, _P, _L, _P, _L, _P, _P, _I, _P),
    "srml_xtv_mfma_ws": (_L, _I, _I),
    "srml_mbin_f32": (_P, _L, _I, _L, _P, _P, _L, _I, _P, _L, _P),
    "srml_qn_step_batch": (_P, _I, _P),
    "srml_mlogit_f32": (_P, _L, _I, _L, _P, _P, _P, _P, _I, _P, _P),
    "srml_mlogit_supported": (_I, _I),
    "srml_qn_step": (_P, _P),
    "srml_qn_step_mb": (_P, _P, _P),
    "srml_qn_step_mbf": (_P, _P, _P, _I, _L, _P),
    "srml_kmeans_lloyd_small": (_P, _L, _I, _L, _P, _I, _P, _P, _P, _P, _P, _P, _P),
    "srml_kmeans_lloyd_mfma": (_P, _L, _I, _L, _P, _I, _P, _P, _P, _P, _P, _P, _P, _P, _P),
    "srml_kmeans_small_update": (_P, _I, _I, _P, _P, _P, _D, _P, _P, _P, _P),
    "srml_qn_mb_scratch": (),
    "srml_kmeanspp_gram": (_P, _I, _L, _P, _I, _I, ctypes.c_ulonglong, _P, _P),
    "srml_qn_max_history": (),
    "srml_qn_args_size": (),
    "srml_nearest_centroid_f32": (_P, _L, _I, _L, _P, _I, _L, _P, _P, _P),
    "srml_nn_finalize": (_P, _L, _P, _P, _P, _P),
    "srml_split_bf16x3": (_P, _L, _I, _L, _I, _L, _P, _P),
    "srml_nearest_centroid_split": (_P, _L, _L, _I, _P, _I, _L, _P, _P, _P),
    "srml_split_bf16x3_tiled": (_P, _L, _I, _L, _I, _L, _P, _P),
    "srml_nearest_centroid_split_tiled": (_P, _L, _L, _I, _P, _I, _L, _P, _P, _P),
    "srml_nearest_centroid_split_tiled_np": (_P, _L, _L, _I, _P, _I, _L, _P, _P, _I, _P),
    "srml_nearest_centroid_split_top2": (_P, _L, _L, _I, _P, _I, _L, _P, _P, _P, _P, _P, _P),
    "srml_split_bf16x3_tiled_centered": (_P, _L, _I, _L, _P, _I, _L, _P, _P),
    "srml_split_bf16x3_tiled_centered_rows": (_P, _L, _P, _L, _I, _P, _I, _L, _P, _P),
    "srml_row_sqnorm_centered_f32": (_P, _L, _I, _L, _P, _P, _P),
    "srml_row_sqnorm_centered_amax_f32": (_P, _L, _I, _L, _P, _P, _P, _P),
    "srml_rf_sample_features_floyd": (_I, _I),
    "srml_rf_bootstrap_ws": (_I, _L),
    "srml_rf_bootstrap": (_I, _L, _D, ctypes.c_ulonglong, _P, _P, _P, _P, _P),
    "srml_split_f16_tiled_centered": (_P, _L, _I, _L, _P, _I, _L, _F, _P, _P, _P),
    "srml_nearest_centroid_f16_top2": (_P, _L, _L, _I, _P, _I, _L, _P, _P, _P, _F, _F, _P, _P, _P),
    "srml_nearest_centroid_f16_top2_nslot": (_I,),
    "srml_split_top2_select_f16": (_P, _P, _L, _I, _P, _P, _F, _F, _F, _P, _P, _P, _P, _P, _P),
    "srml_split_f16_tiled_centered_rows": (_P, _L, _P, _L, _I, _P, _I, _L, _F, _P, _P, _P),
    "srml_f16_plane_gather_rows": (_P, _L, _I, _P, _L, _L, _P, _P),
    "srml_nearest_f16_rowloop": (_P, _L, _L, _I, _P, _I, _L, _P, _F, _P, _P),
    "srml_f16_plane_gather_rows_ex": (_P, _L, _I, _P, _L, _L, _P, _P, _P, _P, _P),
    "srml_split_top2_select_f16_thr": (_P, _P, _L, _I, _P, _P, _F, _F, _F, _P, _P, _P, _P, _P, _P, _P),
    "srml_nearest_centroid_f16_cand": (_P, _L, _L, _I, _P, _I, _L, _P, _P, _P, _F, _F, _P, _P, _P, _I, _P),
    "srml_kmeans_cand_exact": (_P, _L, _P, _P, _L, _I, _I, _P, _I, _P, _P, _I, _P, _P, _P),
    "srml_nearest_centroid_split_top2_nslot": (_I,),
    "srml_split_top2_select": (_P, _P, _L, _I, _P, _P, _P, _P, _P, _P, _P),
    "srml_split_scatter_refined": (_P, _P, _I, _P, _P, _P, _P),
    "srml_kmeans_accumulate_f32": (_P, _L, _I, _L, _P, _I, _P, _P, _P, _P),
    "srml_kmeans_accumulate_sorted_f32": (_P, _L, _I, _L, _P, _P, _P, _P),
    "srml_kmeans_accumulate_sorted_rows_f32": (_P, _L, _I, _L, _P, _P, _P, _P, _P),
    "srml_lloyd_moved_ws": (_L,),
    "srml_lloyd_moved_count": (_P, _P, _L, _P, _P, _P),
    "srml_lloyd_moved_compact": (_P, _P, _L, _P, _L, _P, _P, _P, _P),
    "srml_counts_from_offsets": (_P, _I, _P, _P),
    "srml_sum_f32_ws": (),
    "srml_sum_f32_f64": (_P, _L, _P, _P, _P),
    "srml_lloyd_centre_update": (_P, _I, _I, _P, _P, _P, _P),
    "srml_kmeans_segment_sums_f32": (_P, _L, _I, _L, _P, _P, _I, _P, _I, _P, _P),
    "srml_kmeans_segment_sums_f64": (_P, _L, _I, _L, _P, _P, _I, _P, _I, _P, _P),
    "srml_nearest_centroid_f64": (_P, _L, _I, _L, _P, _I, _L, _P, _P, _P, _P, _P, _P),
    "srml_row_sqnorm_f64": (_P, _L, _I, _L, _P, _P),
    "srml_knn_dist_f32": (_P, _L, _I, _L, _P, _L, _L, _P, _P, _L, _P),
    "srml_pairdist_f32": (_P, _L, _I, _L, _P, _L, _L, _I, _F, _P, _L, _P),
    "srml_topk_rows_f32": (_P, _L, _L, _L, _I, _P, _L, ctypes.c_longlong, _I, _P, _P, _L, _L, _P),
    "srml_knn_f32": (_P, _L, _I, _L, _P, _L, _L, _P, _I, _I, _P, _P, ctypes.c_longlong, _P),
    "srml_ivf_search_f32": (_P, _L, _I, _L, _P, _I, _P, _P, _L, _P, _P, _I, _P, _P, _P),
    "srml_knn_lists_f32": (_P, _I, _L, _P, _P, _P, _I, _P, _P, _I, _I, _P, _P, _P),
    "srml_f16_centre_prep": (_P, _I, _I, _I, _P, _F, _I, _P, _P, _P, _P, _P),
    "srml_knn_lists_f16c": (_P, _I, _L, _P, _P, _P, _I, _P, _P, _I, _I, _P, _P, _P),
    "srml_knn_pairs_f16c": (_P, _I, _L, _P, _P, _P, _P, _P, _P, _P, _I, _I, _P, _P, _P, _P, _P, _P, _P),
    "srml_center_rows_f16": (_P, _I, _L, _P, _P, _I, _L, _P, _P, _P),
    "srml_dbscan_degree_f32": (_P, _L, _I, _L, _P, _F, _L, _L, _P, _P),
    "srml_dbscan_link_f32": (_P, _L, _I, _L, _P, _F, _L, _L, _P, _P, _P, _P),
    "srml_uf_unite_pairs": (_P, _L, _P, _P),
    "srml_uf_compress": (_P, _L, _P),
    "srml_dbscan_labels_ws": (_L,),
    "srml_umap_categorical_ws": (_L, _L),
    "srml_umap_categorical": (_P, _P, _P, _L, _P, _L, _D, _D, _D, _P, _P, _P),
    "srml_dbscan_labels": (_P, _P, _P, _L, _P, _P, _P),
    "srml_oneshot_alloc": (_L, _P, _P),
    "srml_oneshot_open": (_P, _P),
    "srml_oneshot_close": (_P,),
    "srml_oneshot_free": (_P,),
    "srml_oneshot_allreduce": (_P, _P, _L, _I, _P, _I, _I, ctypes.c_ulonglong, _L, ctypes.c_longlong, _P, _P),
    "srml_umap_smooth_knn": (_P, _P, _L, _I, _L, _D, _D, _I, _P, _I, _P, _P, _P, _P),
    "srml_umap_fuzzy_union_knn": (_P, _P, _L, _I, _L, ctypes.c_float, _P, _P, _P, _P),
    "srml_umap_epoch": (_P, _P, _L, _P, _P, _P, _P, _P, _P, _I, _I, _F, _F, _F, _F, _F, _I, _I, ctypes.c_uint, _P, _P,
                        _I, _P),
    "srml_umap_neg_table": (_P, _P, _L, _I, _P, _P),
    "srml_umap_epoch_sync_ws": (_L, _L, _I),
    "srml_umap_epoch_sync": (_P, _P, _L, _P, _P, _P, _P, _P, _P, _P, _L, _I, _I, _F, _F, _F, _F, _F, _I, _I,
                             ctypes.c_uint, _P, _P, _I, _P, _I, _P),
    "srml_syevj_f64": (_P, _I, _P, _P, _I, _D, _P),
    "srml_potrf_f64": (_P, _I, _L, _P, _P),
    "srml_potrs_f64": (_P, _I, _L, _P, _P),
    "srml_potrs_backward_f64": (_P, _I, _L, _P, _P),
    "srml_cd_gram_f64": (_P, _I, _L, _P, _P, _P, _P, _I, _D, _P, _P),
    "srml_potrf_f64_variant": (_P, _I, _L, _P, _I, _I, _I, _P),
    "srml_potrs_f64_variant": (_P, _I, _L, _P, _I, _P),
    "srml_cd_gram_f64_variant": (_P, _I, _L, _P, _P, _P, _P, _I, _D, _P, _I, _P),
    "srml_rf_quantize_u8": (_P, _L, _I, _L, _P, _I, _P, _P),
    "srml_rf_quantize_u8_ld": (_P, _L, _I, _L, _P, _I, _P, _L, _P),
    "srml_rf_pack_wy": (_P, _P, _P, _L, _P, _P),
    "srml_rf_quantiles_f32": (_P, _I, _I, _I, _P, _P),
    "srml_rf_hist": (_P, _L, _P, _P, _P, _I, _P, _I, _I, _I, _I, _D, _I, _P, _P, _I, _P),
    "srml_rf_interleave_u8": (_P, _L, _I, _I, _P, _P),
    "srml_rf_hist_fb": (_I, _I, _I),
    "srml_rf_hist_fb_max": (),
    "srml_rf_best_split": (_P, _P, _I, _I, _I, _I, _I, _I, _D, _D, _P, _P, _P),
    "srml_rf_node_split_ok": (_I, _I, _I),
    "srml_rf_transpose_u8": (_P, _L, _I, _P, _P),
    "srml_rf_node_split": (_P, _L, _P, _P, _P, _I, _P, _I, _I, _I, _I, _D, _D, _P, _P, _P),
    "srml_rf_route": (_P, _L, _P, _P, _L, _P, _P, _P, _P, _P),
    "srml_rf_route_segments": (_P, _L, _P, _L, _P, _I, _P, _P, _P, _P, _P),
    "srml_rf_node_stats": (_P, _P, _P, _L, _P, _I, _I, _I, _P, _P),
    "srml_rf_node_stats_det": (_P, _P, _P, _P, _I, _I, _I, _P, _P),
    "srml_label_sort": (_P, _L, _I, _P, _P, _P, _P, _P),
    "srml_label_sort_ws": (_L, _I),
    "srml_label_sort_kmax": (),
    "srml_radix_sort_ws": (_L,),
    "srml_knn_refine_sort_f32": (_P, _L, _I, _L, _P, _L, _P, _I, _L, _I, _P, _P, _P),
    "srml_radix_sort_u64": (_P, _P, _P, _P, _L, _I, _P, _P),
    "srml_label_counts": (_P, _L, _I, _P, _P),
    "srml_rf_hist_wide": (_P, _L, _P, _P, _P, _I, _P, _I, _I, _I, _I, _D, _I, _I, _I, _P, _P, _P),
    "srml_rf_hist_wide_fb": (_I, _I, _I),
    "srml_rf_hist_fixed": (_P, _L, _P, _P, _P, _I, _P, _I, _I, _D, _I, _P, _I, _P),
    "srml_rf_hist_fixed_finish": (_P, _L, _D, _P),
    "srml_csr_logreg_binary_f32": (_P, _P, _P, _L, _I, _L, _P, _P, _D, _P, _P, _P, _P),
    "srml_csr_logreg_binary_f64": (_P, _P, _P, _L, _I, _L, _P, _P, _D, _P, _P, _P, _P),
    "srml_csr_spmm_f32": (_P, _P, _P, _L, _L, _P, _I, _P, _P, _P),
    "srml_csr_spmm_f64": (_P, _P, _P, _L, _L, _P, _I, _P, _P, _P),
    "srml_csr_spmtm_f32": (_P, _P, _P, _L, _L, _P, _I, _P, _P),
    "srml_csr_spmtm_f64": (_P, _P, _P, _L, _L, _P, _I, _P, _P),
    "srml_csr_spmm_ld_f32": (_P, _P, _P, _L, _L, _P, _I, _L, _P, _P, _L, _P),
    "srml_csr_spmm_ld_f64": (_P, _P, _P, _L, _L, _P, _I, _L, _P, _P, _L, _P),
    "srml_csr_spmtm_ld_f32": (_P, _P, _P, _L, _L, _P, _I, _L, _P, _L, _P),
    "srml_csr_spmtm_ld_f64": (_P, _P, _P, _L, _L, _P, _I, _L, _P, _L, _P),
    "srml_csr_row_sums_f32": (_P, _P, _L, _P, _P),
    "srml_csr_knn_config": (_I,),
    "srml_csr_pairdist_f32": (_P, _P, _P, _P, _L, _P, _P, _P, _P, _L, _I, _I, _P, _L, _P),
    "srml_csr_refine_f32": (_P, _P, _P, _L, _P, _P, _P, _L, _P, _I, _L, _P, _L, _P),
    "srml_csr_nnd_config": (_I,),
    "srml_csr_nnd_join_f32": (_P, _P, _P, _P, _L, _L, _P, _P, _P, _P, _L, _P, _I, _P, _P, _I, _I, _I, _I, _I, _P, _P,
                              _P),
    "srml_confusion_counts": (_P, _I, _P, _I, _L, _I, _P, _P),
    "srml_logloss_sum": (_P, _I, _L, _I, _L, _P, _I, _D, _P, _P),
    "srml_reg_moments": (_P, _I, _P, _I, _L, _P, _P),
    "srml_csr_col_moments_f32": (_P, _P, _L, _P, _P, _P),
    "srml_csr_col_moments_f64": (_P, _P, _L, _P, _P, _P),
    "srml_memcpy_h2d_async": (_P, _P, _L, _P),
    "srml_memcpy_d2h_sync": (_P, _P, _L, _P),
    "srml_memset_async": (_P, _I, _L, _P),
    "srml_rf_predict_nodes2": (_P, _L, _L, _I, _P, _P, _I, _P, _I, _P, _P, _P),
    "srml_rf_predict": (_P, _L, _L, _P, _I, _P, _P, _P, _P, _P, _P, _I, _P, _P, _P),
    "srml_rf_left_totals": (_P, _I, _L, _I, _I, _I, _P, _P, _P),
    "srml_rf_gather_feature": (_P, _L, _P, _L, _P, _P),
    "srml_rf_decide": (_P, _P, _P, _L, _P, _P, _P, _P, _P, _P, _P, _I, _P, _P),
    "srml_rf_level_pack": (_P, _L, _P, _I, _I, _I, _P, _P, _P, _P),
    "srml_seg_lower_bound": (_P, _P, _P, _L, _P, _I, _P, _P),
    "srml_scatter_shift": (_P, _I, _P, _P, _P, _D, _P),
    "srml_sum_sq_ws": (),
    "srml_sum_sq": (_P, _I, _L, _P, _P, _P),
    "srml_lsq_prepare": (_P, _I, _P, _P, _P, _D, _D, _D, _D, _D, _I, _I, _I, _P, _P, _P),
    "srml_lsq_finish": (_P, _I, _P, _P, _D, _D, _I, _P, _P),
    "srml_rf_sample_features": (_I, _I, _I, ctypes.c_ulonglong, _P, _P),
    "srml_rf_partition": (_P, _L, _P, _I, _P, _P, _I, _P, _P, _P, _P, _P, _P, _P),
    "srml_rf_partition_ws": (_L, _I),
    "srml_ivf_candidate_max": (_P, _I, _P, _L, _P, _P, _P),
    "srml_ivf_candidates_f32": (_P, _L, _L, _I, _L, _P, _I, _P, _P, _P, _L, _P, _P, _P, _P, _L, _P),
    "srml_row_list": (_P, _I, _L, _P, _P),
    "srml_cd_sweep_global_f64": (_P, _I, _L, _P, _P, _P, _P, _P, _P, _P, _I, _P),
# ... 77 lines not shown
```

Before: 3510.

## Fuse L-BFGS line-search trial step into margin-only logistic evaluation kernel

```diff
diff --git a/spark_rapids_ml_nai_amd/models/logistic.py b/spark_rapids_ml_nai_amd/models/logistic.py
--- a/spark_rapids_ml_nai_amd/models/logistic.py
+++ b/spark_rapids_ml_nai_amd/models/logistic.py
@@ -89,8 +89,8 @@
     ws = ops.logreg_workspace(X) if not sparse and K == 1 else None
 
     def evaluate(w: torch.Tensor, b: torch.Tensor, flag: Optional[torch.Tensor], out: torch.Tensor,
-                 zc: Optional[tuple] = None) -> None:
-        ops.logistic_loss_grad(X, y32, w, b, K, out, flag, ws=ws, zcache=zc)
+                 zc: Optional[tuple] = None, zt: Optional[tuple] = None) -> None:
+        ops.logistic_loss_grad(X, y32, w, b, K, out, flag, ws=ws, zcache=zc, ztrial=zt)
 
     allreduce = ctx.comm.allreduce if ctx.distributed else None
     path = ops.logistic_path(X, K)
@@ -101,8 +101,8 @@
         _scratch = ops.zeros(K * n + 2, dtype=torch.float64, device=X.device)
 
         def evaluate_partials(w: torch.Tensor, b: torch.Tensor, flag: Optional[torch.Tensor],
-                              zc: Optional[tuple] = None) -> None:
-            ops.logistic_loss_grad(X, y32, w, b, K, _scratch, flag, ws=ws, leave_partials=True, zcache=zc)
+                              zc: Optional[tuple] = None, zt: Optional[tuple] = None) -> None:
+            ops.logistic_loss_grad(X, y32, w, b, K, _scratch, flag, ws=ws, leave_partials=True, zcache=zc, ztrial=zt)
     graph_safe = (path in ("fused_binary_f32", "fused_multinomial_f32", "csr_binary", "two_pass_multinomial_f32",
                            "two_pass_binary_f32") or path.startswith("lds_binary")) and _eval_bytes(X) <= GRAPH_MAX_BYTES
     zok = ((path == "fused_binary_f32" and (X.shape[0] == 0 or ops.logreg_zcache_ok(X)))
@@ -112,8 +112,10 @@
         ctx.comm.allreduce(flag_t, op="min")
         zok = bool(flag_t.item() > 0)
     zbuf = ops.zeros(2 * X.shape[0] * K, dtype=torch.float64, device=X.device) if zok else None
+    zblocks = ops.logreg_trial_blocks(X) if zok and allreduce is None and path == "fused_binary_f32" else 0
     res = minimize(P, theta0, evaluate, allreduce, y.device, batch=8 if not path.startswith("torch") else 2,
-                   graph_safe=graph_safe, fold=fold, evaluate_partials=evaluate_partials, zcache=zbuf)
+                   graph_safe=graph_safe, fold=fold, evaluate_partials=evaluate_partials, zcache=zbuf,
+                   ztrial_blocks=zblocks)
     return _result(res, base, ctx, n, K, fit_intercept, inv_sigma, path)
 
 
diff --git a/spark_rapids_ml_nai_amd/models/qn.py b/spark_rapids_ml_nai_amd/models/qn.py
--- a/spark_rapids_ml_nai_amd/models/qn.py
+++ b/spark_rapids_ml_nai_amd/models/qn.py
@@ -23,6 +23,9 @@
     range(13)
 SC_F, SC_ALPHA, SC_DGINIT, SC_GAMMA, SC_GINF, SC_ALPHA1, SC_BETA = range(7)
 QN_ZCACHE = os.environ.get("SRML_QN_ZCACHE", "1") != "0"
+QN_ZTRIAL = os.environ.get("SRML_QN_ZTRIAL", "launch")
+if QN_ZTRIAL not in ("launch", "step"):
+    raise ValueError("SRML_QN_ZTRIAL must be 'launch' or 'step', not %r" % QN_ZTRIAL)
 
 
 @dataclass
@@ -231,6 +234,11 @@
                                                  "l2", "l1c", "isg", "fl", "wb", "out", "probe")]
 
 
+class _QnTrial(ctypes.Structure):
+    _fields_ = [("A", _QnArgs), ("scr", ctypes.c_void_p), ("tab", ctypes.c_void_p), ("elems", ctypes.c_int),
+                ("pad", ctypes.c_int)]
+
+
 class DeviceQN:
 
     def __init__(self, P: QNProblem, theta0: np.ndarray, device: torch.device, wb: Optional[torch.Tensor] = None,
@@ -314,6 +322,22 @@
         self.flags[F_ZC] = 1
         return (self.flags, zbuf, self._keep["sc"])
 
+    def ztrial_supported(self) -> bool:
+        return self._mb is not None and self.P.K == 1 and self.zcache_supported()
+
+    def enable_ztrial(self, blocks: int) -> tuple:
+        from ..ops import native
+
+        assert self._mb is not None and blocks > 0
+        self._ztab = ops.zeros(int(native.lib().srml_qn_trial_tab(blocks)), dtype=torch.float64, device=self.device)
+        t = _QnTrial()
+        ctypes.memmove(ctypes.addressof(t), ctypes.addressof(self._args), ctypes.sizeof(_QnArgs))
+        t.scr, t.tab, t.elems = self._mb.data_ptr(), self._ztab.data_ptr(), 32 if self.fold is not None else 256
+        assert ctypes.sizeof(_QnTrial) == int(native.lib().srml_qn_trial_size()), "QnTrial layout mismatch"
+        native.call("srml_qn_trial_check", ctypes.addressof(t))
+        self._ztrial = torch.frombuffer(bytearray(bytes(t)), dtype=torch.uint8).to(self.device)
+        return (self._ztrial, int(blocks))
+
     def info(self) -> dict:
         fl = self.flags.cpu().numpy()
         sc = self._keep["sc"].cpu().numpy()
@@ -338,7 +362,8 @@
                                                                    torch.Tensor], None],
              allreduce: Optional[Callable[[torch.Tensor], None]], device: torch.device,
              batch: int = 8, graph_safe: bool = False, fold: Optional[tuple] = None,
-             evaluate_partials: Optional[Callable] = None, zcache: Optional[torch.Tensor] = None) -> dict:
+             evaluate_partials: Optional[Callable] = None, zcache: Optional[torch.Tensor] = None,
+             ztrial_blocks: int = 0) -> dict:
     if device.type != "cuda":
         st = HostQN(P, theta0)
         out = ops.zeros(P.out_len, dtype=torch.float64, device=device)
@@ -360,6 +385,8 @@
         q.fold = fold
         evaluate = lambda w, b, flag, out, **kw: evaluate_partials(w, b, flag, **kw)
     zkw = {"zc": zc} if zc is not None else {}
+    if zc is not None and ztrial_blocks > 0 and allreduce is None and QN_ZTRIAL == "launch" and q.ztrial_supported():
+        zkw["zt"] = q.enable_ztrial(ztrial_blocks)
     poll = _comm_poll(allreduce)
     flag = q.flags[F_DONE: F_DONE + 1]
     host_flag = ops.zeros(2, dtype=torch.int32, pin_memory=True)
diff --git a/spark_rapids_ml_nai_amd/ops/__init__.py b/spark_rapids_ml_nai_amd/ops/__init__.py
--- a/spark_rapids_ml_nai_amd/ops/__init__.py
+++ b/spark_rapids_ml_nai_amd/ops/__init__.py
@@ -314,6 +314,14 @@
     m, n = X.shape
     ptr, ld = (X.data_ptr(), X.stride(0)) if X.is_contiguous() else (0, n)
     return bool(int(native.lib().srml_logreg_zcache_ok(m, n, ld, ptr)))
+
+
+def logreg_trial_blocks(X: Any) -> int:
+    if not logreg_zcache_ok(X):
+        return 0
+    m, n = X.shape
+    ptr, ld = (X.data_ptr(), X.stride(0)) if X.is_contiguous() else (0, n)
+    return int(native.lib().srml_logreg_trial_blocks(m, n, ld, ptr))
 
 
 def nearest_centroid(X: torch.Tensor, C: torch.Tensor, xnorm: Optional[torch.Tensor] = None,
@@ -3532,8 +3540,11 @@
 
 def logistic_loss_grad(X, y32: torch.Tensor, w: torch.Tensor, b: torch.Tensor, K: int, out: torch.Tensor,
                        flag: Optional[torch.Tensor] = None, ws: Optional[torch.Tensor] = None,
-                       leave_partials: bool = False, zcache: Optional[tuple] = None) -> torch.Tensor:
+                       leave_partials: bool = False, zcache: Optional[tuple] = None,
+                       ztrial: Optional[tuple] = None) -> torch.Tensor:
     path = logistic_path(X, K)
+    if ztrial is not None and (zcache is None or path != "fused_binary_f32"):
+        raise ValueError("ztrial needs the binary margin cache (zcache) on the fused binary evaluation")
     if _is_csr(X):
         m, n = X.shape
         dev = X.data.device
@@ -3601,9 +3612,14 @@
         dgemm(R, X, ta=True, beta=1.0, out=out[: K * n].view(K, n))
     elif path == "fused_binary_f32":
         zc = [t.data_ptr() for t in zcache] if zcache is not None else [None, None, None]
-        native.call("srml_logreg_binary_f32", X.data_ptr(), m, n, X.stride(0), y32.data_ptr(), w.data_ptr(), 0.0,
-                    b.data_ptr(), fp, out.data_ptr(), ws.data_ptr() if ws is not None else None,
-                    int(bool(leave_partials and ws is not None)), *zc, st)
+        if ztrial is not None:
+            native.call("srml_logreg_binary_trial_f32", X.data_ptr(), m, n, X.stride(0), y32.data_ptr(), w.data_ptr(),
+                        0.0, b.data_ptr(), fp, out.data_ptr(), ws.data_ptr() if ws is not None else None,
+                        int(bool(leave_partials and ws is not None)), *zc, ztrial[0].data_ptr(), int(ztrial[1]), st)
+        else:
+            native.call("srml_logreg_binary_f32", X.data_ptr(), m, n, X.stride(0), y32.data_ptr(), w.data_ptr(), 0.0,
+                        b.data_ptr(), fp, out.data_ptr(), ws.data_ptr() if ws is not None else None,
+                        int(bool(leave_partials and ws is not None)), *zc, st)
     elif path.startswith("lds_binary"):
         native.call("srml_logreg_binary_lds_" + path[-3:], X.data_ptr(), m, n, X.stride(0), y32.data_ptr(),
                     w.data_ptr(), 0.0, b.data_ptr(), fp, out.data_ptr(), st)
diff --git a/spark_rapids_ml_nai_amd/ops/csrc/glm.hip b/spark_rapids_ml_nai_amd/ops/csrc/glm.hip
--- a/spark_rapids_ml_nai_amd/ops/csrc/glm.hip
+++ b/spark_rapids_ml_nai_amd/ops/csrc/glm.hip
@@ -1,4 +1,5 @@
 #include "common.h"
+#include "qn.h"
 #include <stdlib.h>
 
 template <int K>
@@ -461,11 +462,12 @@
 }
 
 
-constexpr int LR_F_ZMODE = 9, LR_F_ZSEL = 10, LR_SC_BETA = 6;
+constexpr int LR_F_ZMODE = F_ZMODE, LR_F_ZSEL = F_ZSEL, LR_SC_BETA = SC_BETA;
 
 __device__ __forceinline__ void lr_margin_only(long m, int n, const float* __restrict__ y, double* __restrict__ out,
                                                float* __restrict__ ws, const double* __restrict__ zb,
-                                               const double* __restrict__ zsc, int zsel, long q0, long rows) {
+                                               const double* __restrict__ zsc, int zsel, long q0, long rows,
+                                               const QnTrial* __restrict__ zt) {
   __shared__ double mred[2][4];
   const int lane = threadIdx.x & 63, wid = threadIdx.x >> 6;
   const double beta = zsc[LR_SC_BETA];
@@ -489,6 +491,10 @@
   __syncthreads();
   gbc = (mred[0][0] + mred[0][1]) + (mred[0][2] + mred[0][3]);
   lossc = (mred[1][0] + mred[1][1]) + (mred[1][2] + mred[1][3]);
+  if (zt) {
+    qn_margin_trial(zt, gbc, lossc);
+    return;
+  }
   if (ws == nullptr) {
     if (threadIdx.x == 0) {
       if (gbc != 0.0) atomicAdd(&out[n], gbc);
@@ -520,7 +526,8 @@
                                                                   double* __restrict__ out, long rows_per_block,
                                                                   float* __restrict__ ws, const int* __restrict__ zfl,
                                                                   double* __restrict__ zb,
-                                                                  const double* __restrict__ zsc) {
+                                                                  const double* __restrict__ zsc,
+                                                                  const QnTrial* __restrict__ zt) {
   constexpr int R = LR_PF_R, D = LR_PF_D;
   if (flag && *flag) return;
   const double b = bptr ? *bptr : b_in;
@@ -530,9 +537,10 @@
   const int zmode = (LOSS == GLM_LOGISTIC && zfl) ? zfl[LR_F_ZMODE] : 0;
   const int zsel = (LOSS == GLM_LOGISTIC && zfl) ? zfl[LR_F_ZSEL] : 0;
   if (zmode == 1) {
-    lr_margin_only(m, n, y, out, ws, zb, zsc, zsel, (long)blockIdx.x * rows_per_block, rows_per_block);
+    lr_margin_only(m, n, y, out, ws, zb, zsc, zsel, (long)blockIdx.x * rows_per_block, rows_per_block, zt);
     return;
   }
+  if (zt && blockIdx.x == 0 && threadIdx.x == 0) zt->A.fl[F_STEPPED] = 0;
   double* zw = (LOSS == GLM_LOGISTIC && zfl) ? zb + (long)(1 - zsel) * m : nullptr;
   const int cbase = wid * 256 * V;
   double wreg[V][4];
@@ -649,14 +657,16 @@
                                                                    double* __restrict__ out, long rows_per_block,
                                                                    const int* __restrict__ zfl,
                                                                    double* __restrict__ zb,
-                                                                   const double* __restrict__ zsc) {
+                                                                   const double* __restrict__ zsc,
+                                                                   const QnTrial* __restrict__ zt) {
   if (flag && *flag) return;
   const int zmode = (LOSS == GLM_LOGISTIC && zfl) ? zfl[LR_F_ZMODE] : 0;
   const int zsel = (LOSS == GLM_LOGISTIC && zfl) ? zfl[LR_F_ZSEL] : 0;
   if (zmode == 1) {
-    lr_margin_only(m, n, y, out, nullptr, zb, zsc, zsel, (long)blockIdx.x * rows_per_block, rows_per_block);
+    lr_margin_only(m, n, y, out, nullptr, zb, zsc, zsel, (long)blockIdx.x * rows_per_block, rows_per_block, zt);
     return;
   }
+  if (zt && blockIdx.x == 0 && threadIdx.x == 0) zt->A.fl[F_STEPPED] = 0;
   double* zw = (LOSS == GLM_LOGISTIC && zfl) ? zb + (long)(1 - zsel) * m : nullptr;
   __shared__ float gsum[4][64 * G];
   __shared__ double red[2][4];
@@ -851,28 +861,44 @@
   return m > 0 && (logreg_narrow_eligible(n, ld, X) || logreg_pf_eligible(n, ld, X)) ? 1 : 0;
 }
 
+static long logreg_narrow_rpb(long m) {
+  long nb = m / 256;
+  if (nb > 4096) nb = 4096;
+  if (nb < 1) nb = 1;
+  const long rpb = (m + nb - 1) / nb;
+  return (rpb + 15) / 16 * 16;
+}
+
+SRML_API long srml_logreg_trial_blocks(long m, int n, long ld, const void* X) {
+  if (m <= 0) return 0;
+  if (logreg_narrow_eligible(n, ld, X)) {
+    const long rpb = logreg_narrow_rpb(m);
+    return (m + rpb - 1) / rpb;
+  }
+  return logreg_pf_eligible(n, ld, X) ? logreg_grid(m) : 0;
+}
+static long logreg_trial_blocks(long m, int n, long ld, const void* X) { return srml_logreg_trial_blocks(m, n, ld, X); }
+
 template <int LOSS>
 static int logreg_binary_launch(const float* X, long m, int n, long ld, const float* y, const double* w, double b,
                                 const double* bptr, const int* flag, double* out, float* fold_ws, int leave,
-                                const int* zfl, double* zb, const double* zsc, hipStream_t stream) {
+                                const int* zfl, double* zb, const double* zsc, const QnTrial* zt, int ztcap,
+                                hipStream_t stream) {
   if (m <= 0) return 0;
+  if (zt && (!zfl || logreg_trial_blocks(m, n, ld, X) > ztcap)) return (int)hipErrorInvalidValue;
   if (LOSS != GLM_LOGISTIC && zfl) return -2;
   if (zfl && !logreg_pf_eligible(n, ld, X) && !logreg_narrow_eligible(n, ld, X)) return -2;
   if (logreg_narrow_eligible(n, ld, X)) {
-    long nb = m / 256;
-    if (nb > 4096) nb = 4096;
-    if (nb < 1) nb = 1;
-    long rpb = (m + nb - 1) / nb;
-    rpb = (rpb + 15) / 16 * 16;
+    const long rpb = logreg_narrow_rpb(m);
     const long blocks = (m + rpb - 1) / rpb;
     const int G = (n + 63) / 64;
 #define SRML_LR_NARROW(GG, DD)                                                                                       \
   hipLaunchKernelGGL((logreg_binary_narrow_kernel<GG, DD, LOSS>), dim3((unsigned)blocks), dim3(256), 0, stream, X, m, n, ld, \
-                     y, w, b, bptr, flag, out, rpb, zfl, zb, zsc)
+                     y, w, b, bptr, flag, out, rpb, zfl, zb, zsc, zt)
     if constexpr (LOSS != GLM_LOGISTIC) {
       if (G > 2 && G <= 4) {
         hipLaunchKernelGGL((logreg_binary_narrow_kernel<4, 1, LOSS, 4>), dim3((unsigned)blocks), dim3(256), 0, stream,
-                           X, m, n, ld, y, w, b, bptr, flag, out, rpb, zfl, zb, zsc);
+                           X, m, n, ld, y, w, b, bptr, flag, out, rpb, zfl, zb, zsc, zt);
         return srml_status();
       }
     }
@@ -893,7 +919,7 @@
     float* fws = logreg_fold_enabled() ? fold_ws : nullptr;
 #define SRML_LR_PF(VV)                                                                                       \
   hipLaunchKernelGGL((logreg_binary_pf_kernel<VV, LOSS>), grid, blk, 0, stream, X, m, n, ld, y, w, b, bptr, flag, out, \
-                     rpb, fws, zfl, zb, zsc)
+                     rpb, fws, zfl, zb, zsc, zt)
     if (VS == 2) SRML_LR_PF(2);
     else if (VS == 3) SRML_LR_PF(3);
     else SRML_LR_PF(4);
@@ -922,7 +948,16 @@
 SRML_API int srml_logreg_binary_f32(const float* X, long m, int n, long ld, const float* y, const double* w, double b,
                                     const double* bptr, const int* flag, double* out, float* fold_ws, int leave,
                                     const int* zfl, double* zb, const double* zsc, hipStream_t stream) {
-  return logreg_binary_launch<GLM_LOGISTIC>(X, m, n, ld, y, w, b, bptr, flag, out, fold_ws, leave, zfl, zb, zsc, stream);
+  return logreg_binary_launch<GLM_LOGISTIC>(X, m, n, ld, y, w, b, bptr, flag, out, fold_ws, leave, zfl, zb, zsc, nullptr,
+                                            0, stream);
+}
+
+SRML_API int srml_logreg_binary_trial_f32(const float* X, long m, int n, long ld, const float* y, const double* w,
+                                          double b, const double* bptr, const int* flag, double* out, float* fold_ws,
+                                          int leave, const int* zfl, double* zb, const double* zsc, const QnTrial* zt,
+                                          int ztcap, hipStream_t stream) {
+  return logreg_binary_launch<GLM_LOGISTIC>(X, m, n, ld, y, w, b, bptr, flag, out, fold_ws, leave, zfl, zb, zsc, zt,
+                                            ztcap, stream);
 }
 
 SRML_API int srml_svc_loss_grad_f32(const float* X, long m, int n, long ld, const float* y, const double* w, double b,
@@ -930,9 +965,9 @@
                                     int loss, hipStream_t stream) {
   if (loss == 0)
     return logreg_binary_launch<GLM_HINGE>(X, m, n, ld, y, w, b, bptr, flag, out, fold_ws, leave, nullptr, nullptr,
-                                           nullptr, stream);
+                                           nullptr, nullptr, 0, stream);
   if (loss == 1)
     return logreg_binary_launch<GLM_SQ_HINGE>(X, m, n, ld, y, w, b, bptr, flag, out, fold_ws, leave, nullptr, nullptr,
-                                              nullptr, stream);
+                                              nullptr, nullptr, 0, stream);
   return -2;
 }
diff --git a/spark_rapids_ml_nai_amd/ops/csrc/qn.h b/spark_rapids_ml_nai_amd/ops/csrc/qn.h
--- /dev/null
+++ b/spark_rapids_ml_nai_amd/ops/csrc/qn.h
@@ -0,0 +1,373 @@
+#pragma once
+#include "common.h"
+
+namespace {
+
+constexpr int QN_MMAX = 12;
+
+enum { F_DONE = 0, F_STATUS, F_ITER, F_NEVAL, F_LS, F_COUNT, F_HEAD, F_STARTED, F_BRACKET, F_ZMODE, F_ZSEL,
+       F_NCHEAP, F_ZC, F_SKIPX, F_STEPPED, F_TICKET };
+enum { ST_RUNNING = 0, ST_CONV_GRAD = 1, ST_CONV_F = 2, ST_MAXITER = 3, ST_LS_FAIL = 4 };
+enum { SC_F = 0, SC_ALPHA, SC_DGINIT, SC_GAMMA, SC_GINF, SC_ALPHA1, SC_BETA };
+
+}
+
+struct QnArgs {
+  long N;
+  long Kn;
+  int n, K, M, past, max_iter, max_ls, l1, wolfe;
+  double tol, delta, inv_m, c1, c2;
+  double *x, *g, *pg, *d, *xt, *gt;
+  double *S, *Y;
+  double *SY, *YY;
+  double *fh;
+  double *sc;
+  const double *l2, *l1c;
+  const double *isg;
+  int *fl;
+  double *wb;
+  double *out;
+  long long *probe;
+};
+
+struct QnTrial {
+  QnArgs A;
+  double* scr;
+  double* tab;
+  int elems;
+  int pad;
+};
+
+template <int NW, int NV>
+__device__ __forceinline__ void qn_block_sum(const double (&v)[NV], double* red, double* tot) {
+  const int lane = threadIdx.x & 63, wid = threadIdx.x >> 6;
+#pragma unroll
+  for (int i = 0; i < NV; ++i) {
+    const double t = wave_sum(v[i]);
+    if (lane == 0) red[i * NW + wid] = t;
+    __builtin_amdgcn_sched_barrier(0);
+  }
+  __syncthreads();
+  if (threadIdx.x < NV) {
+    double s = 0.0;
+#pragma unroll
+    for (int w = 0; w < NW; ++w) s += red[threadIdx.x * NW + w];
+    tot[threadIdx.x] = s;
+  }
+  __syncthreads();
+}
+
+__device__ __forceinline__ double qn_trial_value(double xv, double dv, double pv, double cv, double alpha) {
+  double t = xv + alpha * dv;
+  if (cv > 0.0) {
+    const double orth = xv != 0.0 ? (xv > 0.0 ? 1.0 : -1.0) : (pv < 0.0 ? 1.0 : (pv > 0.0 ? -1.0 : 0.0));
+    if (t * orth <= 0.0) t = 0.0;
+  }
+  return t;
+}
+
+__device__ __forceinline__ double qn_p0_terms(const QnArgs& A, double ov, double isg, double l2v, double l1v,
+                                              double xv, double dv, double pv, double xo, double (&t)[4]) {
+  const double gi = ov * A.inv_m * isg + l2v * xv;
+  t[0] = l2v * xv * xv;
+  t[1] = l1v * fabs(xv);
+  t[2] = gi * dv;
+  t[3] = pv * (xv - xo);
+  return gi;
+}
+
+__device__ __forceinline__ double qn_objective(const QnArgs& A, double loss, const double* p0) {
+  return loss * A.inv_m + 0.5 * p0[0] + p0[1];
+}
+
+struct QnLs {
+  bool accept;
+  double width;
+};
+
+__device__ __forceinline__ QnLs qn_ls_decide(const QnArgs& A, double ft, double f, double alpha, double dginit,
+                                             double p02, double p03, bool bracket, bool zc, int zmode) {
+  bool accept = true;
+  double width = 1.0;
+  if (zc && zmode == 2 && isfinite(ft)) {
+  } else if (!isfinite(ft)) {
+    accept = false;
+    width = 0.5;
+  } else {
+    const double dgtest = A.l1 ? p03 : alpha * dginit;
+    if (ft > f + A.c1 * dgtest) {
+      accept = false;
+      const double den = 2.0 * (ft - f - dgtest);
+      width = den > 0.0 ? -dgtest / den : 0.5;
+      width = isfinite(width) ? fmin(0.5, fmax(0.1, width)) : 0.5;
+    } else if (A.wolfe && !A.l1 && !bracket && p02 < A.c2 * dginit) {
+      accept = false;
+      width = 2.1;
+    }
+  }
+  return {accept, width};
+}
+
+__device__ __forceinline__ void qn_commit_done(int* fl, int status) {
+  fl[F_STATUS] = status;
+  fl[F_DONE] = 1;
+  fl[F_SKIPX] = 1;
+}
+
+__device__ __forceinline__ void qn_commit_zmode(int* fl, int zmode) {
+  fl[F_ZMODE] = zmode;
+  fl[F_SKIPX] = zmode == 1 ? 1 : 0;
+}
+
+__device__ __forceinline__ void qn_commit_reject(const QnArgs& A, int ls, int neval, double width, double alpha_tried,
+                                                 double alpha, double ft, bool zc, int zmode, double alpha1) {
+  int* fl = A.fl;
+  fl[F_LS] = ls;
+  fl[F_NEVAL] = neval;
+  if (ls >= A.max_ls) {
+    qn_commit_done(fl, ST_LS_FAIL);
+    return;
+  }
+  if (width < 1.0) fl[F_BRACKET] = 1;
+  A.sc[SC_ALPHA] = alpha;
+  if (zc && isfinite(ft)) {
+    const double a1 = zmode == 0 ? alpha_tried : alpha1;
+    A.sc[SC_ALPHA1] = a1;
+    A.sc[SC_BETA] = alpha / a1;
+    qn_commit_zmode(fl, 1);
+  } else if (zc) {
+    qn_commit_zmode(fl, 0);
+  }
+}
+
+__device__ __forceinline__ void qn_commit_margins_accept(int* fl, int neval) {
+  fl[F_NEVAL] = neval;
+  qn_commit_zmode(fl, 2);
+}
+
+__device__ __forceinline__ void qn_commit_margins_point(int* fl) {
+  fl[F_ZSEL] ^= 1;
+  qn_commit_zmode(fl, 0);
+}
+
+namespace {
+
+constexpr int MB_T = 256;
+constexpr int MB_NW = MB_T / 64;
+constexpr int MB_GMAX = 64;
+constexpr int MBF_E = 32;
+constexpr int MB_GAMAX = 512;
+constexpr int QT_GROUP = 64;
+constexpr int QT_LINE = 32;
+constexpr int MB_PW = 6 + 5 * QN_MMAX + 1;
+enum {
+  S_STARTED = 0, S_ITER, S_COUNT, S_HEAD, S_LS, S_NEVAL, S_BRACKET, S_F, S_ALPHA, S_DGINIT, S_GAMMA, S_FHN, S_LOSS,
+  S_ZMODE, S_ZC, S_ALPHA1,
+  S_PHASE = 16, S_STATUS, S_NEWP, S_CNT, S_HD, S_GAM, S_FT, S_GINF, S_ITERN, S_FN,
+  S_CF = 32,
+  S_SL = S_CF + 2 * QN_MMAX,
+  S_SY = S_SL + QN_MMAX,
+  S_PA = S_SY + 2 * QN_MMAX * QN_MMAX,
+  S_PB = S_PA + 4 * MB_GAMAX,
+  S_PC = S_PB + MB_PW * MB_GMAX,
+  S_END = S_PC + 2 * MB_GMAX
+};
+
+__device__ __forceinline__ void mb_grid_sum(const double* part, int G, int width, double* tot, bool max_last) {
+  __shared__ double gs[MB_T];
+  const int t = threadIdx.x, S = MB_T / width;
+  const int j = t % width, sl = t / width;
+  const bool mx = max_last && j == width - 1;
+  double a[8] = {0.0, 0.0, 0.0, 0.0, 0.0, 0.0, 0.0, 0.0};
+  if (sl < S) {
+    int b = sl;
+    for (; b + 7 * S < G; b += 8 * S) {
+      double v[8];
+#pragma unroll
+      for (int k = 0; k < 8; ++k) v[k] = part[(long)(b + k * S) * width + j];
+#pragma unroll
+      for (int k = 0; k < 8; ++k) a[k] = mx ? fmax(a[k], v[k]) : a[k] + v[k];
+    }
+    for (; b < G; b += S) {
+      const double v = part[(long)b * width + j];
+      a[0] = mx ? fmax(a[0], v) : a[0] + v;
+    }
+  }
+  gs[t] = mx ? fmax(fmax(fmax(a[0], a[1]), fmax(a[2], a[3])), fmax(fmax(a[4], a[5]), fmax(a[6], a[7])))
+             : ((a[0] + a[1]) + (a[2] + a[3])) + ((a[4] + a[5]) + (a[6] + a[7]));
+  __syncthreads();
+  if (t < width) {
+    double x = gs[t];
+    for (int q = 1; q < S; ++q) x = mx ? fmax(x, gs[q * width + t]) : x + gs[q * width + t];
+    tot[t] = x;
+  }
+  __syncthreads();
+}
+
+}
+
+struct MbSnap {
+  int started, iter, count, head, ls, neval, bracket, zmode, zc;
+  double f, alpha, dginit, gamma, alpha1;
+};
+
+__device__ __forceinline__ MbSnap mb_snap_load(const QnArgs& A) {
+  const int* fl = A.fl;
+  MbSnap q;
+  q.started = fl[F_STARTED];
+  q.iter = fl[F_ITER];
+  q.count = fl[F_COUNT];
+  q.head = fl[F_HEAD];
+  q.ls = fl[F_LS];
+  q.neval = fl[F_NEVAL];
+  q.bracket = fl[F_BRACKET];
+  q.f = A.sc[SC_F];
+  q.alpha = A.sc[SC_ALPHA];
+  q.dginit = A.sc[SC_DGINIT];
+  q.gamma = A.sc[SC_GAMMA];
+  q.zc = fl[F_ZC];
+  q.zmode = q.zc ? fl[F_ZMODE] : 0;
+  q.alpha1 = A.sc[SC_ALPHA1];
+  return q;
+}
+
+struct MbP0In {
+  double xv, l2v, l1v, dv, pgv, xo, isg;
+};
+
+__device__ __forceinline__ MbP0In mb_p0_load(const QnArgs& A, long i, bool own) {
+  MbP0In e{0.0, 0.0, 0.0, 0.0, 0.0, 0.0, 1.0};
+  if (own) {
+    e.xv = A.xt[i];
+    e.l2v = A.l2[i];
+    e.l1v = A.l1c[i];
+    e.dv = A.d[i];
+    e.pgv = A.pg[i];
+    e.xo = A.x[i];
+    if (i < A.Kn) e.isg = A.isg[i % A.n];
+  }
+  return e;
+}
+
+__device__ __forceinline__ void mb_trial(const QnArgs& A, long i, double xv, double dv, double pv, double cv,
+                                         double isg, double alpha) {
+  const double t = qn_trial_value(xv, dv, pv, A.l1 ? cv : 0.0, alpha);
+  A.xt[i] = t;
+  A.wb[i] = t * isg;
+}
+
+__device__ __forceinline__ void mb_pair_thread_sum(const double* pairs, long stride, int parts, double& gb,
+                                                   double& ls) {
+  gb = 0.0;
+  ls = 0.0;
+  for (int p = threadIdx.x; p < parts; p += 4 * MB_T) {
+    double t0[4], t1[4];
+#pragma unroll
+    for (int k = 0; k < 4; ++k) {
+      const int pk = p + k * MB_T;
+      const double* pd = pairs + (long)(pk < parts ? pk : 0) * stride;
+      t0[k] = pk < parts ? pd[0] : 0.0;
+      t1[k] = pk < parts ? pd[1] : 0.0;
+    }
+#pragma unroll
+    for (int k = 0; k < 4; ++k) {
+      gb += t0[k];
+      ls += t1[k];
+    }
+  }
+}
+
+__device__ __forceinline__ void mb_pair_block_sum(double gb, double ls, double* red, double (&tot)[2]) {
+  const double sums[2] = {gb, ls};
+  const int lane = threadIdx.x & 63, wid = threadIdx.x >> 6;
+  for (int k = 0; k < 2; ++k) {
+    const double t = wave_sum(sums[k]);
+    if (lane == 0) red[k * MB_NW + wid] = t;
+  }
+  __syncthreads();
+  tot[0] = (red[0] + red[1]) + (red[2] + red[3]);
+  tot[1] = (red[MB_NW] + red[MB_NW + 1]) + (red[MB_NW + 2] + red[MB_NW + 3]);
+}
+
+__device__ __forceinline__ void qn_margin_trial(const QnTrial* __restrict__ zt, double gbc, double lossc) {
+  __shared__ double red[4 * MB_NW], tot[4];
+  __shared__ int s_last;
+  const int tid = threadIdx.x;
+  const unsigned G = gridDim.x;
+  const QnArgs A = zt->A;
+  double* scr = zt->scr;
+  double* tab = zt->tab;
+  const int E = zt->elems;
+  const int ga = (int)((A.N + E - 1) / E);
+  int* fl = A.fl;
+  for (int vb = blockIdx.x; vb < ga; vb += G) {
+    const long i = (long)vb * E + tid;
+    const bool own = tid < E && i < A.N;
+    double p0[4] = {0.0, 0.0, 0.0, 0.0};
+    if (own) qn_p0_terms(A, 0.0, 1.0, A.l2[i], A.l1c[i], A.xt[i], 0.0, 0.0, 0.0, p0);
+    qn_block_sum<MB_NW>(p0, red, tot);
+    if (tid < 4)
+      __hip_atomic_store(&scr[S_PA + vb * 4 + tid], tot[tid], __ATOMIC_RELAXED, __HIP_MEMORY_SCOPE_AGENT);
+  }
+  if (tid == 0) {
+    __hip_atomic_store(&tab[2 * (long)blockIdx.x], gbc, __ATOMIC_RELAXED, __HIP_MEMORY_SCOPE_AGENT);
+    __hip_atomic_store(&tab[2 * (long)blockIdx.x + 1], lossc, __ATOMIC_RELAXED, __HIP_MEMORY_SCOPE_AGENT);
+  }
+  asm volatile("s_waitcnt vmcnt(0)" ::: "memory");
+  __syncthreads();
+  if (tid == 0) {
+    const int grp = blockIdx.x / QT_GROUP, ngrp = ((int)G + QT_GROUP - 1) / QT_GROUP;
+    const int gsize = min(QT_GROUP, (int)G - grp * QT_GROUP);
+    int* gcnt = reinterpret_cast<int*>(tab + 2 * (long)G) + (long)grp * QT_LINE;
+    int last = 0;
+    if (__hip_atomic_fetch_add(gcnt, 1, __ATOMIC_RELAXED, __HIP_MEMORY_SCOPE_AGENT) == gsize - 1) {
+      __hip_atomic_store(gcnt, 0, __ATOMIC_RELAXED, __HIP_MEMORY_SCOPE_AGENT);
+      last = __hip_atomic_fetch_add(&fl[F_TICKET], 1, __ATOMIC_RELAXED, __HIP_MEMORY_SCOPE_AGENT) == ngrp - 1;
+    }
+    if (last) {
+      __hip_atomic_store(&fl[F_TICKET], 0, __ATOMIC_RELAXED, __HIP_MEMORY_SCOPE_AGENT);
+      __builtin_amdgcn_fence(__ATOMIC_ACQUIRE, "agent");
+      asm volatile("s_waitcnt vmcnt(0)" ::: "memory");
+    }
+    s_last = last;
+  }
+  __syncthreads();
+  if (!s_last) return;
+  const MbSnap q = mb_snap_load(A);
+  double gb, ls;
+  mb_pair_thread_sum(tab, 2, (int)G, gb, ls);
+  double pt[2];
+  mb_pair_block_sum(gb, ls, red, pt);
+  __syncthreads();
+  mb_grid_sum(scr + S_PA, ga, 4, tot, false);
+  const double ft = qn_objective(A, pt[1], tot);
+  if (tid == 0) fl[F_NCHEAP] += 1;
+  const QnLs d = qn_ls_decide(A, ft, q.f, q.alpha, q.dginit, tot[2], tot[3], q.bracket != 0, true, 1);
+  if (!d.accept) {
+    const int ls_n = q.ls + 1;
+    const double alpha = q.alpha * d.width;
+    if (ls_n < A.max_ls) {
+      constexpr int U = 4;
+      for (long i0 = tid; i0 < A.N; i0 += (long)MB_T * U) {
+        double xv[U], dv[U], sg[U];
+#pragma unroll
+        for (int u = 0; u < U; ++u) {
+          const long i = i0 + (long)u * MB_T;
+          const bool ok = i < A.N;
+          xv[u] = ok ? A.x[i] : 0.0;
+          dv[u] = ok ? A.d[i] : 0.0;
+          sg[u] = (ok && i < A.Kn) ? A.isg[i % A.n] : 1.0;
+        }
+#pragma unroll
+        for (int u = 0; u < U; ++u) {
+          const long i = i0 + (long)u * MB_T;
+          if (i < A.N) mb_trial(A, i, xv[u], dv[u], 0.0, 0.0, sg[u], alpha);
+        }
+      }
+    }
+    if (tid == 0) qn_commit_reject(A, ls_n, q.neval + 1, d.width, q.alpha, alpha, ft, true, 1, q.alpha1);
+  } else if (tid == 0) {
+    qn_commit_margins_accept(fl, q.neval + 1);
+  }
+  if (tid == 0) fl[F_STEPPED] = 1;
+}
diff --git a/spark_rapids_ml_nai_amd/ops/csrc/qn.hip b/spark_rapids_ml_nai_amd/ops/csrc/qn.hip
--- a/spark_rapids_ml_nai_amd/ops/csrc/qn.hip
+++ b/spark_rapids_ml_nai_amd/ops/csrc/qn.hip
@@ -1,56 +1,13 @@
-#include "common.h"
+#include "qn.h"
 
 namespace {
 
 constexpr int QN_T = 512;
 constexpr int QN_NW = QN_T / 64;
-constexpr int QN_MMAX = 12;
 constexpr int QN_NV = 6 + 5 * QN_MMAX;
 
-enum { F_DONE = 0, F_STATUS, F_ITER, F_NEVAL, F_LS, F_COUNT, F_HEAD, F_STARTED, F_BRACKET, F_ZMODE, F_ZSEL,
-       F_NCHEAP, F_ZC, F_SKIPX };
-enum { ST_RUNNING = 0, ST_CONV_GRAD = 1, ST_CONV_F = 2, ST_MAXITER = 3, ST_LS_FAIL = 4 };
-enum { SC_F = 0, SC_ALPHA, SC_DGINIT, SC_GAMMA, SC_GINF, SC_ALPHA1, SC_BETA };
-
-}
-
-struct QnArgs {
-  long N;
-  long Kn;
-  int n, K, M, past, max_iter, max_ls, l1, wolfe;
-  double tol, delta, inv_m, c1, c2;
-  double *x, *g, *pg, *d, *xt, *gt;
-  double *S, *Y;
-  double *SY, *YY;
-  double *fh;
-  double *sc;
-  const double *l2, *l1c;
-  const double *isg;
-  int *fl;
-  double *wb;
-  double *out;
-  long long *probe;
-};
-
-
-template <int NW, int NV>
-__device__ __forceinline__ void qn_block_sum(const double (&v)[NV], double* red, double* tot) {
-  const int lane = threadIdx.x & 63, wid = threadIdx.x >> 6;
-#pragma unroll
-  for (int i = 0; i < NV; ++i) {
-    const double t = wave_sum(v[i]);
-    if (lane == 0) red[i * NW + wid] = t;
-    __builtin_amdgcn_sched_barrier(0);
-  }
-  __syncthreads();
-  if (threadIdx.x < NV) {
-    double s = 0.0;
-#pragma unroll
-    for (int w = 0; w < NW; ++w) s += red[threadIdx.x * NW + w];
-    tot[threadIdx.x] = s;
-  }
-  __syncthreads();
-}
+}
+
 
 __device__ __forceinline__ double pseudo_grad(double x, double g, double c) {
   if (c <= 0.0) return g;
@@ -59,25 +16,6 @@
   if (g + c < 0.0) return g + c;
   if (g - c > 0.0) return g - c;
   return 0.0;
-}
-
-__device__ __forceinline__ double qn_trial_value(double xv, double dv, double pv, double cv, double alpha) {
-  double t = xv + alpha * dv;
-  if (cv > 0.0) {
-    const double orth = xv != 0.0 ? (xv > 0.0 ? 1.0 : -1.0) : (pv < 0.0 ? 1.0 : (pv > 0.0 ? -1.0 : 0.0));
-    if (t * orth <= 0.0) t = 0.0;
-  }
-  return t;
-}
-
-__device__ __forceinline__ double qn_p0_terms(const QnArgs& A, double ov, double isg, double l2v, double l1v,
-                                              double xv, double dv, double pv, double xo, double (&t)[4]) {
-  const double gi = ov * A.inv_m * isg + l2v * xv;
-  t[0] = l2v * xv * xv;
-  t[1] = l1v * fabs(xv);
-  t[2] = gi * dv;
-  t[3] = pv * (xv - xo);
-  return gi;
 }
 
 struct QnPair {
@@ -105,76 +43,6 @@
   t[2] = yx * Yj;
   t[3] = Sj * pgi;
   t[4] = Yj * pgi;
-}
-
-struct QnLs {
-  bool accept;
-  double width;
-};
-
-__device__ __forceinline__ QnLs qn_ls_decide(const QnArgs& A, double ft, double f, double alpha, double dginit,
-                                             double p02, double p03, bool bracket, bool zc, int zmode) {
-  bool accept = true;
-  double width = 1.0;
-  if (zc && zmode == 2 && isfinite(ft)) {
-  } else if (!isfinite(ft)) {
-    accept = false;
-    width = 0.5;
-  } else {
-    const double dgtest = A.l1 ? p03 : alpha * dginit;
-    if (ft > f + A.c1 * dgtest) {
-      accept = false;
-      const double den = 2.0 * (ft - f - dgtest);
-      width = den > 0.0 ? -dgtest / den : 0.5;
-      width = isfinite(width) ? fmin(0.5, fmax(0.1, width)) : 0.5;
-    } else if (A.wolfe && !A.l1 && !bracket && p02 < A.c2 * dginit) {
-      accept = false;
-      width = 2.1;
-    }
-  }
-  return {accept, width};
-}
-
-__device__ __forceinline__ void qn_commit_done(int* fl, int status) {
-  fl[F_STATUS] = status;
-  fl[F_DONE] = 1;
-  fl[F_SKIPX] = 1;
-}
-
-__device__ __forceinline__ void qn_commit_zmode(int* fl, int zmode) {
-  fl[F_ZMODE] = zmode;
-  fl[F_SKIPX] = zmode == 1 ? 1 : 0;
-}
-
-__device__ __forceinline__ void qn_commit_reject(const QnArgs& A, int ls, int neval, double width, double alpha_tried,
-                                                 double alpha, double ft, bool zc, int zmode, double alpha1) {
-  int* fl = A.fl;
-  fl[F_LS] = ls;
-  fl[F_NEVAL] = neval;
-  if (ls >= A.max_ls) {
-    qn_commit_done(fl, ST_LS_FAIL);
-    return;
-  }
-  if (width < 1.0) fl[F_BRACKET] = 1;
-  A.sc[SC_ALPHA] = alpha;
-  if (zc && isfinite(ft)) {
-    const double a1 = zmode == 0 ? alpha_tried : alpha1;
-    A.sc[SC_ALPHA1] = a1;
-    A.sc[SC_BETA] = alpha / a1;
-    qn_commit_zmode(fl, 1);
-  } else if (zc) {
-    qn_commit_zmode(fl, 0);
-  }
-}
-
-__device__ __forceinline__ void qn_commit_margins_accept(int* fl, int neval) {
-  fl[F_NEVAL] = neval;
-  qn_commit_zmode(fl, 2);
-}
-
-__device__ __forceinline__ void qn_commit_margins_point(int* fl) {
-  fl[F_ZSEL] ^= 1;
-  qn_commit_zmode(fl, 0);
 }
 
 struct QnHist {
@@ -644,85 +512,6 @@
 SRML_API int srml_qn_max_history() { return QN_MMAX; }
 SRML_API long srml_qn_args_size() { return (long)sizeof(QnArgs); }
 
-namespace {
-
-constexpr int MB_T = 256;
-constexpr int MB_NW = MB_T / 64;
-constexpr int MB_GMAX = 64;
-constexpr int MBF_E = 32;
-constexpr int MB_GAMAX = 512;
-constexpr int MB_PW = 6 + 5 * QN_MMAX + 1;
-enum {
-  S_STARTED = 0, S_ITER, S_COUNT, S_HEAD, S_LS, S_NEVAL, S_BRACKET, S_F, S_ALPHA, S_DGINIT, S_GAMMA, S_FHN, S_LOSS,
-  S_ZMODE, S_ZC, S_ALPHA1,
-  S_PHASE = 16, S_STATUS, S_NEWP, S_CNT, S_HD, S_GAM, S_FT, S_GINF, S_ITERN, S_FN,
-  S_CF = 32,
-  S_SL = S_CF + 2 * QN_MMAX,
-  S_SY = S_SL + QN_MMAX,
-  S_PA = S_SY + 2 * QN_MMAX * QN_MMAX,
-  S_PB = S_PA + 4 * MB_GAMAX,
-  S_PC = S_PB + MB_PW * MB_GMAX,
-  S_END = S_PC + 2 * MB_GMAX
-};
-
-__device__ __forceinline__ void mb_grid_sum(const double* part, int G, int width, double* tot, bool max_last) {
-  __shared__ double gs[MB_T];
-  const int t = threadIdx.x, S = MB_T / width;
-  const int j = t % width, sl = t / width;
-  const bool mx = max_last && j == width - 1;
-  double a[8] = {0.0, 0.0, 0.0, 0.0, 0.0, 0.0, 0.0, 0.0};
-  if (sl < S) {
-    int b = sl;
-    for (; b + 7 * S < G; b += 8 * S) {
-      double v[8];
-#pragma unroll
-      for (int k = 0; k < 8; ++k) v[k] = part[(long)(b + k * S) * width + j];
-#pragma unroll
-      for (int k = 0; k < 8; ++k) a[k] = mx ? fmax(a[k], v[k]) : a[k] + v[k];
-    }
-    for (; b < G; b += S) {
-      const double v = part[(long)b * width + j];
-      a[0] = mx ? fmax(a[0], v) : a[0] + v;
-    }
-  }
-  gs[t] = mx ? fmax(fmax(fmax(a[0], a[1]), fmax(a[2], a[3])), fmax(fmax(a[4], a[5]), fmax(a[6], a[7])))
-             : ((a[0] + a[1]) + (a[2] + a[3])) + ((a[4] + a[5]) + (a[6] + a[7]));
-  __syncthreads();
-  if (t < width) {
-    double x = gs[t];
-    for (int q = 1; q < S; ++q) x = mx ? fmax(x, gs[q * width + t]) : x + gs[q * width + t];
-    tot[t] = x;
-  }
-  __syncthreads();
-}
-
-}
-
-
-struct MbSnap {
-  int started, iter, count, head, ls, neval, bracket, zmode, zc;
-  double f, alpha, dginit, gamma, alpha1;
-};
-
-__device__ __forceinline__ MbSnap mb_snap_load(const QnArgs& A) {
-  const int* fl = A.fl;
-  MbSnap q;
-  q.started = fl[F_STARTED];
-  q.iter = fl[F_ITER];
-  q.count = fl[F_COUNT];
-  q.head = fl[F_HEAD];
-  q.ls = fl[F_LS];
-  q.neval = fl[F_NEVAL];
-  q.bracket = fl[F_BRACKET];
-  q.f = A.sc[SC_F];
-  q.alpha = A.sc[SC_ALPHA];
-  q.dginit = A.sc[SC_DGINIT];
-  q.gamma = A.sc[SC_GAMMA];
-  q.zc = fl[F_ZC];
-  q.zmode = q.zc ? fl[F_ZMODE] : 0;
-  q.alpha1 = A.sc[SC_ALPHA1];
-  return q;
-}
 
 __device__ __forceinline__ void mb_snap_store(const QnArgs& A, const MbSnap& q, double* scr) {
   scr[S_STARTED] = q.started ? 1.0 : 0.0;
@@ -743,29 +532,12 @@
   scr[S_PHASE] = 0.0;
 }
 
-struct MbP0In {
-  double xv, l2v, l1v, dv, pgv, xo, isg;
-};
-
-__device__ __forceinline__ MbP0In mb_p0_load(const QnArgs& A, long i, bool own) {
-  MbP0In e{0.0, 0.0, 0.0, 0.0, 0.0, 0.0, 1.0};
-  if (own) {
-    e.xv = A.xt[i];
-    e.l2v = A.l2[i];
-    e.l1v = A.l1c[i];
-    e.dv = A.d[i];
-    e.pgv = A.pg[i];
-    e.xo = A.x[i];
-    if (i < A.Kn) e.isg = A.isg[i % A.n];
-  }
-  return e;
-}
-
 __device__ __forceinline__ void mb_p0(const QnArgs& A, long i, bool own, const MbP0In& e, double ov, double (&p0)[4]) {
   if (own) A.gt[i] = qn_p0_terms(A, ov, e.isg, e.l2v, e.l1v, e.xv, e.dv, e.pgv, e.xo, p0);
 }
 
 __global__ __launch_bounds__(MB_T) void qn_mb1_kernel(QnArgs A, double* __restrict__ scr) {
+  if (A.fl[F_STEPPED]) return;
   __shared__ double red[4 * MB_NW], tot[4];
   const bool first = blockIdx.x == 0 && threadIdx.x == 0;
   const long i = (long)blockIdx.x * MB_T + threadIdx.x;
@@ -794,14 +566,8 @@
   if (threadIdx.x < 4) scr[S_PA + blockIdx.x * 4 + threadIdx.x] = tot[threadIdx.x];
 }
 
-__device__ __forceinline__ void mb_trial(const QnArgs& A, long i, double xv, double dv, double pv, double cv,
-                                         double isg, double alpha) {
-  const double t = qn_trial_value(xv, dv, pv, A.l1 ? cv : 0.0, alpha);
-  A.xt[i] = t;
-  A.wb[i] = t * isg;
-}
-
 __global__ __launch_bounds__(MB_T) void qn_mb2_kernel(QnArgs A, double* __restrict__ scr, int ga) {
+  if (A.fl[F_STEPPED]) return;
   __shared__ double red[MB_PW * MB_NW], p0[4];
   int* fl = A.fl;
   const int M = A.M;
@@ -837,7 +603,7 @@
   if (done) return;
   mb_grid_sum(scr + S_PA, ga, 4, p0, false);
   double alpha = alpha0;
-  const double ft = loss * A.inv_m + 0.5 * p0[0] + p0[1];
+  const double ft = qn_objective(A, loss, p0);
   if (first)
     for (long j = N; j < A.Kn + A.K + 1; ++j) A.out[j] = 0.0;
   if (first && zc && zmode == 1) fl[F_NCHEAP] += 1;
@@ -903,6 +669,7 @@
 }
 
 __global__ __launch_bounds__(MB_T) void qn_mb3_kernel(QnArgs A, double* __restrict__ scr) {
+  if (A.fl[F_STEPPED]) return;
   __shared__ double tot[MB_PW], red[2 * MB_NW], t2[2];
   __shared__ QnHist H;
   __shared__ QnUpd s_u;
@@ -991,6 +758,7 @@
 }
 
 __global__ __launch_bounds__(MB_T) void qn_mb4_kernel(QnArgs A, double* __restrict__ scr) {
+  if (A.fl[F_STEPPED]) return;
   __shared__ double p2[2], pbt[MB_PW];
   const int G = gridDim.x, M = A.M, tid = threadIdx.x;
   const bool first = blockIdx.x == 0 && tid == 0;
@@ -1087,21 +855,7 @@
   const bool has_loss = blockIdx.x == G - 1;
   double gb = 0.0, ls = 0.0;
   if (has_bias || has_loss)
-    for (int p = tid; p < parts; p += 4 * MB_T) {
-      double t0[4], t1[4];
-#pragma unroll
-      for (int k = 0; k < 4; ++k) {
-        const int pk = p + k * MB_T;
-        const double* pd = reinterpret_cast<const double*>(fws + (long)(pk < parts ? pk : 0) * wst + wst - 4);
-        t0[k] = pk < parts ? pd[0] : 0.0;
-        t1[k] = pk < parts ? pd[1] : 0.0;
-      }
-#pragma unroll
-      for (int k = 0; k < 4; ++k) {
-        gb += t0[k];
-        ls += t1[k];
-      }
-    }
+    mb_pair_thread_sum(reinterpret_cast<const double*>(fws + wst - 4), wst / 2, parts, gb, ls);
   double a0 = 0.0, a1 = 0.0, a2 = 0.0, a3 = 0.0;
   if (c < A.Kn) {
     int p = rg;
@@ -1122,18 +876,8 @@
   fold[rg][4 * q + 1] = a1;
   fold[rg][4 * q + 2] = a2;
   fold[rg][4 * q + 3] = a3;
-  const double sums[2] = {has_bias ? gb : 0.0, has_loss ? ls : 0.0};
   double tv2[2];
-  {
-    const int lane = tid & 63, wid = tid >> 6;
-    for (int k = 0; k < 2; ++k) {
-      const double t = wave_sum(sums[k]);
-      if (lane == 0) red[k * MB_NW + wid] = t;
-    }
-  }
-  __syncthreads();
-  tv2[0] = (red[0] + red[1]) + (red[2] + red[3]);
-  tv2[1] = (red[MB_NW] + red[MB_NW + 1]) + (red[MB_NW + 2] + red[MB_NW + 3]);
+  mb_pair_block_sum(has_bias ? gb : 0.0, has_loss ? ls : 0.0, red, tv2);
   if (own) {
     if (i < A.Kn) {
       double s = 0.0;
@@ -1150,6 +894,7 @@
 
 __global__ __launch_bounds__(MB_T) void qn_mb1f_kernel(QnArgs A, double* __restrict__ scr,
                                                        const float* __restrict__ fws, int parts, long wst) {
+  if (A.fl[F_STEPPED]) return;
   __shared__ double red[4 * MB_NW], tot[4], fold[32][33];
   const bool first = blockIdx.x == 0 && threadIdx.x == 0;
   const unsigned G = gridDim.x;
@@ -1186,3 +931,18 @@
   hipLaunchKernelGGL(qn_mb4_kernel, grid, blk, 0, stream, *a, scratch);
   return srml_status();
 }
+
+SRML_API long srml_qn_trial_size() { return (long)sizeof(QnTrial); }
+
+SRML_API long srml_qn_trial_tab(long blocks) {
+  return 2 * blocks + (blocks + QT_GROUP - 1) / QT_GROUP * (QT_LINE * (long)sizeof(int) / (long)sizeof(double));
+}
+
+SRML_API int srml_qn_trial_check(const QnTrial* t) {
+  if (!t || !t->scr || !t->tab || !t->A.fl) return (int)hipErrorInvalidValue;
+  if (t->elems != MBF_E && t->elems != MB_T) return (int)hipErrorInvalidValue;
+  const QnArgs& a = t->A;
+  if (a.K != 1 || a.l1 || a.wolfe || a.N <= 0) return (int)hipErrorInvalidValue;
+  if ((a.N + MB_T - 1) / MB_T > MB_GMAX || (a.N + t->elems - 1) / t->elems > MB_GAMAX) return (int)hipErrorInvalidValue;
+  return 0;
+}
diff --git a/spark_rapids_ml_nai_amd/ops/native.py b/spark_rapids_ml_nai_amd/ops/native.py
--- a/spark_rapids_ml_nai_amd/ops/native.py
+++ b/spark_rapids_ml_nai_amd/ops/native.py
@@ -16,6 +16,7 @@
 _F = ctypes.c_float
 
 _LONG_RESULT = ("srml_rf_bootstrap_ws", "srml_logreg_fold_ws", "srml_qn_mb_scratch",
+                "srml_qn_trial_size", "srml_qn_trial_tab", "srml_logreg_trial_blocks",
                 "srml_logreg_fold_parts", "srml_qn_args_size", "srml_logit_residual_ws", "srml_xtv_mfma_ws",
                 "srml_rf_partition_ws", "srml_dbscan_labels_ws", "srml_umap_categorical_ws",
                 "srml_umap_epoch_sync_ws",
@@ -36,6 +37,8 @@
     "srml_xtv_f32": (_P, _L, _I, _L, _P, _I, _L, _P, _P),
     "srml_row_sqnorm_f32": (_P, _L, _I, _L, _P, _P),
     "srml_logreg_binary_f32": (_P, _L, _I, _L, _P, _P, _D, _P, _P, _P, _P, _I, _P, _P, _P, _P),
+    "srml_logreg_binary_trial_f32": (_P, _L, _I, _L, _P, _P, _D, _P, _P, _P, _P, _I, _P, _P, _P, _P, _I, _P),
+    "srml_logreg_trial_blocks": (_L, _I, _L, _P),
     "srml_logreg_fold_parts": (_L,),
     "srml_logreg_fold_ws": (_L, _I, _L, _P),
     "srml_logreg_zcache_ok": (_L, _I, _L, _P),
@@ -76,6 +79,9 @@
     "srml_kmeanspp_gram": (_P, _I, _L, _P, _I, _I, ctypes.c_ulonglong, _P, _P),
     "srml_qn_max_history": (),
     "srml_qn_args_size": (),
+    "srml_qn_trial_size": (),
+    "srml_qn_trial_tab": (_L,),
+    "srml_qn_trial_check": (_P,),
     "srml_nearest_centroid_f32": (_P, _L, _I, _L, _P, _I, _L, _P, _P, _P),
     "srml_nn_finalize": (_P, _L, _P, _P, _P, _P),
     "srml_split_bf16x3": (_P, _L, _I, _L, _I, _L, _P, _P),
```

New measurement: 3491. Within noise of the previous version (-0.5%).
